# QZ1-boy/CDFO

Measured on AMD Instinct MI355X. Metric: x4 SR frames/sec, 7-frame 270x480->1080p, higher is better.
Workload: dtype fp16 MFMA, fp32 accumulate (1 pass inside Block_, 2 passes = fp16 hi+lo activations elsewhere, split-bf16 for the returned feature cache; 2-4e-4 max-abs vs the fp32 reference, bound 1e-3); 1 GPU; JCT-VC ClassB-shape synthetic clips: 8 clips/GPU x 7x1x270x480 luma (padded to 272x480) + MV/residual/partition/unfiltered priors -> 1080x1920, fresh path (pre_L1_fea=None), precision=fp16x2, Gumbel noise drawn per forward inside the mask kernel (the reference's default behaviour); clips_per_gpu=8, parallelism=batch-shard x1, weights=random init (seed 0), launch=eager

## Files before the change

cdfo_amd/_lib.py:

```python
from __future__ import annotations

import ctypes as C
import os

import torch

from . import switches

_HERE = os.path.dirname(os.path.abspath(__file__))
LIB_PATH = switches.get("CDFO_LIB_PATH") or os.path.join(_HERE, "lib", "libcdfo_hip.so")

_lib = None


class CdfoError(RuntimeError):
    pass


class ConvArgs(C.Structure):
    _fields_ = [
        ("src", C.c_void_p * 8), ("ld", C.c_int * 8), ("cs", C.c_int * 8), ("nsrc", C.c_int),
        ("B", C.c_int), ("H", C.c_int), ("W", C.c_int), ("Ho", C.c_int), ("Wo", C.c_int),
        ("ks", C.c_int), ("stride", C.c_int), ("pad", C.c_int),
        ("Cin", C.c_int), ("Cout", C.c_int), ("CoutP", C.c_int),
        ("w", C.c_void_p), ("w_bstride", C.c_longlong), ("bias", C.c_void_p),
        ("act", C.c_int),
        ("res1", C.c_void_p), ("ldr1", C.c_int),
        ("res2", C.c_void_p), ("ldr2", C.c_int),
        ("out", C.c_void_p), ("ldo", C.c_int), ("store_mode", C.c_int),
        ("prec", C.c_int),
        ("ln_gamma", C.c_void_p), ("ln_beta", C.c_void_p),
        ("tap_mask", C.c_void_p),
        ("src_f16", C.c_int), ("out_f16", C.c_int),
        ("out2_cp16", C.c_void_p),
        ("src_plane_wrap", C.c_int),
        ("res_up2", C.c_void_p), ("ldru", C.c_int),
        ("out2_lo", C.c_int),
        ("mask_out", C.c_void_p), ("flow", C.c_void_p), ("flow_bstride", C.c_longlong), ("off_mag", C.c_float),
        ("off_accumulate", C.c_int),
        ("res2_pixscale", C.c_void_p),
        ("src_halfsplit", C.c_int),
    ]


def lib() -> C.CDLL:
    global _lib
    if _lib is None:
        if not os.path.exists(LIB_PATH):
            raise CdfoError(
                f"{LIB_PATH} is missing: the HIP extension has not been built "
                "(run `python -m cdfo_amd.build`).  There is no CPU fallback for the product path.")
        switches.check_hip_environment()
        _lib = C.CDLL(LIB_PATH)
        for name, (restype, argtypes) in header_prototypes().items():
            fn = getattr(_lib, name)
            fn.restype = restype
            fn.argtypes = argtypes
    return _lib


HEADER_PATH = os.path.join(os.path.dirname(_HERE), "include", "cdfo_hip.h")


def header_prototypes(path: str = HEADER_PATH):
    import re
    text = open(path).read()
    text = re.sub(r"/\*.*?\*/", " ", text, flags=re.S)
    protos = {}
    for m in re.finditer(r"(const char\*|long long|int)\s+(cdfo_[a-z0-9_]+)\s*\(([^)]*)\)\s*;", text):
        ret, name, args = m.group(1), m.group(2), m.group(3).strip()
        at = []
        if args and args != "void":
            for a in args.split(","):
                a = " ".join(a.split())
                if "*" in a:
                    at.append(C.c_void_p)
                elif a.startswith("long long"):
                    at.append(C.c_longlong)
                elif a.startswith("float"):
                    at.append(C.c_float)
                elif a.startswith("int"):
                    at.append(C.c_int)
                else:
                    raise CdfoError(f"cannot map C type in prototype of {name}: {a!r}")
        protos[name] = (C.c_char_p if ret.startswith("const char") else C.c_longlong if ret == "long long" else C.c_int, at)
    return protos


def check(status: int, what: str) -> None:
    if status != 0:
        kind = {-1: "invalid argument", -2: "misaligned pointer/pitch"}.get(status, f"hipError_t {status}")
        raise CdfoError(f"{what} failed: {kind}")
```

cdfo_amd/csrc/conv1x1_bf16x3.hip:

```cpp
#include "common.h"

namespace {

constexpr int PXT = 128;
constexpr int PIXB = 80;
constexpr int A_CHUNK = PXT * PIXB;
constexpr int A_BYTES = 4 * A_CHUNK;
constexpr int W_HALF = 4 * 2 * 64 * 16;
constexpr int W_BYTES = 2 * W_HALF;
constexpr int EPI_RS = 68;
constexpr int EPI_BYTES = 4 * 32 * EPI_RS * 4;
constexpr int MAXCB = 4;

typedef __bf16 bf16x8_t __attribute__((ext_vector_type(8)));
typedef unsigned int u32x2 __attribute__((ext_vector_type(2)));

__device__ __forceinline__ unsigned pack_bf16(float a, float b) {
  const __bf16 ha = (__bf16)a, hb = (__bf16)b;
  return (unsigned)__builtin_bit_cast(unsigned short, ha) | ((unsigned)__builtin_bit_cast(unsigned short, hb) << 16);
}
__device__ __forceinline__ float bf16_round(float a) { return (float)(__bf16)a; }
__device__ __forceinline__ void split_store(unsigned char* dst_hi, int lo_delta, const f32x4 v) {
  u32x2 hi, lo;
  hi[0] = pack_bf16(v[0], v[1]);
// ... 86 lines not shown
        const bf16x8_t ah = *reinterpret_cast<const bf16x8_t*>(sA + c * A_CHUNK + a_off);
        const bf16x8_t al = *reinterpret_cast<const bf16x8_t*>(sA + c * A_CHUNK + a_off + 32);
#pragma unroll
        for (int ni = 0; ni < 2; ++ni) {
          const bf16x8_t bh = *reinterpret_cast<const bf16x8_t*>(sW + (c * 2 * 64 + ni * 32) * 16 + b_off);
          const bf16x8_t bl = *reinterpret_cast<const bf16x8_t*>(sW + W_HALF + (c * 2 * 64 + ni * 32) * 16 + b_off);
          acc[cb][ni] = __builtin_amdgcn_mfma_f32_32x32x16_bf16(al, bh, acc[cb][ni], 0, 0, 0);
          acc[cb][ni] = __builtin_amdgcn_mfma_f32_32x32x16_bf16(ah, bl, acc[cb][ni], 0, 0, 0);
          acc[cb][ni] = __builtin_amdgcn_mfma_f32_32x32x16_bf16(ah, bh, acc[cb][ni], 0, 0, 0);
        }
      }
    }
  }

  __syncthreads();
  float* wl = reinterpret_cast<float*>(smem) + wave * 32 * EPI_RS;
  const float slope = a.act == CDFO_ACT_NONE ? 1.f : (a.act == CDFO_ACT_LRELU ? 0.1f : 0.f);
  const int c4 = lane & 15, pr = lane >> 4;
  const bool plain = a.store_mode == CDFO_STORE_PLAIN;
  const int cq = a.Cout >> 2;
  typedef _Float16 c1_f16x8 __attribute__((ext_vector_type(8)));
  c1_f16x8 twh[TAPS ? 4 : 1], twl[TAPS ? 4 : 1];
  if (TAPS) {
#pragma unroll
    for (int s4 = 0; s4 < 4; ++s4)
#pragma unroll
      for (int j = 0; j < 8; ++j) {
        const float wv = r < 9 ? a.res2[(16 * s4 + 8 * h + j) * 9 + r] : 0.f;
        twh[s4][j] = (_Float16)wv;
        twl[s4][j] = (_Float16)(wv - (float)twh[s4][j]);
      }
  }
#pragma unroll
  for (int cb = 0; cb < NCB; ++cb) {
#pragma unroll
    for (int ni = 0; ni < 2; ++ni)
#pragma unroll
      for (int e = 0; e < 16; ++e) wl[((e & 3) + 8 * (e >> 2) + 4 * h) * EPI_RS + ni * 32 + r] = acc[cb][ni][e];
    __builtin_amdgcn_fence(__ATOMIC_RELEASE, "wavefront");
    __builtin_amdgcn_wave_barrier();
    __builtin_amdgcn_fence(__ATOMIC_ACQUIRE, "wavefront");
    if (TAPS) {
      f32x4 y[4][2];
      float amax = 0.f;
#pragma unroll
      for (int s4 = 0; s4 < 4; ++s4)
#pragma unroll
        for (int q = 0; q < 2; ++q) {
          const int ch = 16 * s4 + 8 * h + 4 * q;
          f32x4 t = *reinterpret_cast<const f32x4*>(wl + r * EPI_RS + ch);
          if (a.bias) t += *reinterpret_cast<const f32x4*>(a.bias + cb * 64 + ch);
#pragma unroll
          for (int k = 0; k < 4; ++k) {
            t[k] = fmaxf(t[k], 0.f) + slope * fminf(t[k], 0.f);
            amax = fmaxf(amax, fabsf(t[k]));
          }
          y[s4][q] = t;
        }
      amax = fmaxf(amax, __shfl_xor(amax, 32, 64));
      int ex = 0;
      if (amax > 0.f && amax < INFINITY) frexpf(amax, &ex);
      ex = ex < -100 ? -100 : (ex > 100 ? 100 : ex);
      const float sc = ldexpf(1.f, 14 - ex), inv = ldexpf(1.f, ex - 14);
      f32x16 tacc;
#pragma unroll
      for (int e = 0; e < 16; ++e) tacc[e] = 0.f;
#pragma unroll
      for (int s4 = 0; s4 < 4; ++s4) {
        c1_f16x8 yh, yl;
#pragma unroll
        for (int j = 0; j < 8; ++j) {
          const float v = y[s4][j >> 2][j & 3] * sc;
          yh[j] = (_Float16)v;
          yl[j] = (_Float16)(v - (float)yh[j]);
        }
        tacc = __builtin_amdgcn_mfma_f32_32x32x16_f16(twl[s4], yh, tacc, 0, 0, 0);
        tacc = __builtin_amdgcn_mfma_f32_32x32x16_f16(twh[s4], yl, tacc, 0, 0, 0);
        tacc = __builtin_amdgcn_mfma_f32_32x32x16_f16(twh[s4], yh, tacc, 0, 0, 0);
      }
      const long long pin = p0 + wave * 32 + r;
      if (pin < P) {
        const int oy = (int)(pin / a.W), ox = (int)(pin - (long long)oy * a.W);
        const long long opix = ((long long)b * 2 * a.H + 2 * oy + (cb >> 1)) * (2 * a.W) + 2 * ox + (cb & 1);
        float* op = a.out + opix * a.ldo;
        const f32x4 t4 = {tacc[0] * inv, tacc[1] * inv, tacc[2] * inv, tacc[3] * inv};
        if ((a.ldo & 3) == 0) *reinterpret_cast<f32x4*>(op + 4 * h) = t4;
        else { op[4 * h] = t4[0]; op[4 * h + 1] = t4[1]; op[4 * h + 2] = t4[2]; op[4 * h + 3] = t4[3]; }
        if (h == 0) op[8] = tacc[4] * inv;
      }
      __builtin_amdgcn_fence(__ATOMIC_RELEASE, "wavefront");
      __builtin_amdgcn_wave_barrier();
      continue;
    }
    const int n = cb * 64 + c4 * 4;
    const bool nok = n < a.Cout;
    f32x4 bias = {0.f, 0.f, 0.f, 0.f};
    if (a.bias && nok) bias = *reinterpret_cast<const f32x4*>(a.bias + n);
#pragma unroll
    for (int it = 0; it < 8; ++it) {
      const int i = it * 4 + pr;
      f32x4 t = *reinterpret_cast<const f32x4*>(wl + i * EPI_RS + c4 * 4) + bias;
#pragma unroll
      for (int k = 0; k < 4; ++k) t[k] = fmaxf(t[k], 0.f) + slope * fminf(t[k], 0.f);
      const long long pin = p0 + wave * 32 + i;
      if (!nok || pin >= P) continue;
      const long long pix = (long long)b * P + pin;
      if (plain) {
        if (a.res1) t += *reinterpret_cast<const f32x4*>(a.res1 + pix * a.ldr1 + n);
        if (a.res2) t += *reinterpret_cast<const f32x4*>(a.res2 + pix * a.ldr2 + n);
        *reinterpret_cast<f32x4*>(a.out + pix * a.ldo + n) = t;
      } else {
        const int sub = n / cq, cc = n - sub * cq;
        const int oy = (int)(pin / a.W), ox = (int)(pin - (long long)oy * a.W);
        const long long opix = ((long long)b * 2 * a.H + 2 * oy + (sub >> 1)) * (2 * a.W) + 2 * ox + (sub & 1);
        *reinterpret_cast<f32x4*>(a.out + opix * a.ldo + cc) = t;
      }
    }
    __builtin_amdgcn_fence(__ATOMIC_RELEASE, "wavefront");
    __builtin_amdgcn_wave_barrier();
  }
}

}

int cdfo_conv1x1_stream_try(const cdfo_conv_args& a, hipStream_t st);
extern "C" int cdfo_layernorm64_cp16hl(const float* in, int ldi, const float* gamma, const float* beta, int B, long long P,
                                       void* out, void* stream);

extern "C" int cdfo_conv1x1_bf16x3(const cdfo_conv_args* pa, void* stream) {
  const cdfo_conv_args& a = *pa;
  hipStream_t st = static_cast<hipStream_t>(stream);
  if (a.nsrc < 1 || a.nsrc > CDFO_MAXSRC || a.B <= 0 || a.ks != 1 || a.stride != 1 || a.pad != 0) return CDFO_EINVAL;
  if (a.act == CDFO_ACT_SIGMOID || a.tap_mask || a.src_f16 || a.out_f16 || a.res_up2 || a.src_plane_wrap) return CDFO_EINVAL;
  const bool ln_out = a.out2_cp16 != nullptr;
  const bool copy_out = ln_out && !a.ln_gamma && !a.ln_beta;
  if (ln_out && (a.Cout != 64 || a.CoutP != 64 || a.store_mode != CDFO_STORE_PLAIN || a.ldo < 64 || !aligned16(a.out2_cp16))) return CDFO_EINVAL;
  if (ln_out && !copy_out && (!a.ln_gamma || !a.ln_beta || !aligned16(a.ln_gamma) || !aligned16(a.ln_beta))) return CDFO_EINVAL;
  int csum = 0;
  for (int s = 0; s < a.nsrc; ++s) {
    if (a.cs[s] <= 0 || a.cs[s] % 64 || a.ld[s] % 4 || a.ld[s] < a.cs[s]) return CDFO_EINVAL;
    if (!aligned16(a.src[s])) return CDFO_EALIGN;
    csum += a.cs[s];
  }
  if (csum != a.Cin || a.CoutP % 64 || a.CoutP > 64 * MAXCB || a.CoutP < a.Cout || a.Cout <= 0 || a.Cout % 4) return CDFO_EINVAL;
  if (a.Ho != a.H || a.Wo != a.W) return CDFO_EINVAL;
  if (a.store_mode == CDFO_STORE_S2D || (a.store_mode == CDFO_STORE_SHUFFLE2 && (a.Cout % 16 || a.res1 || a.res2))) return CDFO_EINVAL;
  if (a.store_mode == CDFO_STORE_TAPS9 && (a.Cout != 256 || a.CoutP != 256 || a.res1 || !a.res2 || a.ldo < 9 || a.w_bstride)) return CDFO_EINVAL;
  const bool taps = a.store_mode == CDFO_STORE_TAPS9;
  if (!aligned16(a.w) || a.w_bstride % 4 || (!taps && a.ldo % 4) || !aligned16(a.out) || (a.bias && !aligned16(a.bias))) return CDFO_EALIGN;
  if ((a.res1 && (a.ldr1 % 4 || !aligned16(a.res1))) || (!taps && a.res2 && (a.ldr2 % 4 || !aligned16(a.res2)))) return CDFO_EALIGN;
  if (!ln_out && a.ln_gamma && !(a.nsrc == 1 && a.cs[0] == 64 && a.ln_beta && aligned16(a.ln_gamma) && aligned16(a.ln_beta))) return CDFO_EINVAL;
  const long long P = (long long)a.H * a.W;
  if (a.res2_pixscale && (!a.res2 || taps)) return CDFO_EINVAL;
  if (ln_out) {
    const int r = cdfo_conv1x1_stream_try(a, st);
    if (r == 1) return 0;
    if (r != 0) return r;
    if (a.res2_pixscale) return CDFO_EINVAL;
    cdfo_conv_args plain = a;
    plain.out2_cp16 = nullptr; plain.ln_gamma = nullptr; plain.ln_beta = nullptr;
    const int rc = cdfo_conv1x1_bf16x3(&plain, stream);
    if (rc) return rc;
    if (copy_out) return cdfo_to_cp16(a.out, a.ldo, a.B, P, 64, a.out2_cp16, stream);
    return cdfo_layernorm64_cp16hl(a.out, a.ldo, a.ln_gamma, a.ln_beta, a.B, P, a.out2_cp16, stream);
  }
  {
    static const bool use_stream = cdfo_switch("CDFO_CONV1X1_STREAM", 1) != 0;
    static const bool taps_stream = cdfo_switch("CDFO_TAPS_STREAM", 1) != 0;
    if (use_stream && (!taps || taps_stream)) {
      const int r = cdfo_conv1x1_stream_try(a, st);
      if (r == 1) return 0;
      if (r != 0) return r;
    }
  }
  if (a.res2_pixscale) return CDFO_EINVAL;
  dim3 grid((unsigned)((P + PXT - 1) / PXT), a.B);
  const double px = (double)a.B * P;
  CdfoProfScope prof(st, KID_CONV1, 2.0 * px * a.Cout * a.Cin, 4.0 * (px * a.Cout + px * a.Cin + (double)a.Cin * a.Cout));
  if (taps) {
    hipLaunchKernelGGL((conv1x1_bf16x3_kernel<4, true>), grid, dim3(256), 0, st, a);
    CDFO_LAUNCH_CHECK();
    return 0;
  }
  switch (a.CoutP / 64) {
    case 1: hipLaunchKernelGGL(conv1x1_bf16x3_kernel<1>, grid, dim3(256), 0, st, a); break;
    case 2: hipLaunchKernelGGL(conv1x1_bf16x3_kernel<2>, grid, dim3(256), 0, st, a); break;
    case 3: hipLaunchKernelGGL(conv1x1_bf16x3_kernel<3>, grid, dim3(256), 0, st, a); break;
    default: hipLaunchKernelGGL(conv1x1_bf16x3_kernel<4>, grid, dim3(256), 0, st, a); break;
  }
  CDFO_LAUNCH_CHECK();
  return 0;
}
```

cdfo_amd/csrc/conv1x1_stream.hip:

```cpp
#include "common.h"

namespace {

constexpr int ST_THREADS = 256;
constexpr int ST_STAGE = 8192;
constexpr int ST_MAXNS = 4;

typedef __bf16 bf16x8_t __attribute__((ext_vector_type(8)));
typedef int i32x4 __attribute__((ext_vector_type(4)));
typedef unsigned int u32x2 __attribute__((ext_vector_type(2)));

struct st_item { const float* base; int ld; int ch0; };

struct st_args {
  st_item act[CDFO_MAXSRC * 4];
  int nkb;
  st_item res[2];
  const float* res_scale;
  const float* w; long long w_bstride; const float* bias;
  int Cin, Cout, CoutP, act_fn;
  float* out; int ldo;
  int B; long long P;
  int tiles_per_image; long long tiles;
  int ns;
  _Float16* ln_hl; const float* ln_g; const float* ln_b;
  const float* w_last;
  int W;
};

__device__ __forceinline__ unsigned st_pack_bf16(float a, float b) {
  const __bf16 ha = (__bf16)a, hb = (__bf16)b;
  return (unsigned)__builtin_bit_cast(unsigned short, ha) | ((unsigned)__builtin_bit_cast(unsigned short, hb) << 16);
}
__device__ __forceinline__ float st_bf16_round(float a) { return (float)(__bf16)a; }

__device__ __forceinline__ void st_dma8(const unsigned (&voff)[8], i32x4 rsrc, unsigned lds) {
  unsigned keep;
  asm volatile(
      "s_nop 4\n\t"
      "s_mov_b32 %0, m0\n\t"
      "s_mov_b32 m0, %10\n\ts_nop 0\n\t"
      "buffer_load_dwordx4 %1, %9, 0 offen lds\n\t"
      "s_add_u32 m0, m0, 0x400\n\ts_nop 0\n\t"
      "buffer_load_dwordx4 %2, %9, 0 offen lds\n\t"
      "s_add_u32 m0, m0, 0x400\n\ts_nop 0\n\t"
      "buffer_load_dwordx4 %3, %9, 0 offen lds\n\t"
      "s_add_u32 m0, m0, 0x400\n\ts_nop 0\n\t"
      "buffer_load_dwordx4 %4, %9, 0 offen lds\n\t"
      "s_add_u32 m0, m0, 0x400\n\ts_nop 0\n\t"
      "buffer_load_dwordx4 %5, %9, 0 offen lds\n\t"
      "s_add_u32 m0, m0, 0x400\n\ts_nop 0\n\t"
      "buffer_load_dwordx4 %6, %9, 0 offen lds\n\t"
      "s_add_u32 m0, m0, 0x400\n\ts_nop 0\n\t"
      "buffer_load_dwordx4 %7, %9, 0 offen lds\n\t"
      "s_add_u32 m0, m0, 0x400\n\ts_nop 0\n\t"
      "buffer_load_dwordx4 %8, %9, 0 offen lds\n\t"
      "s_mov_b32 m0, %0"
      : "=&s"(keep)
      : "v"(voff[0]), "v"(voff[1]), "v"(voff[2]), "v"(voff[3]), "v"(voff[4]), "v"(voff[5]), "v"(voff[6]), "v"(voff[7]),
        "s"(rsrc), "s"(lds)
      : "memory", "scc");
}

__device__ __forceinline__ void st_dma1(unsigned voff, i32x4 rsrc, unsigned lds) {
  unsigned keep;
  asm volatile(
      "s_nop 4\n\t"
      "s_mov_b32 %0, m0\n\t"
      "s_mov_b32 m0, %3\n\ts_nop 0\n\t"
      "buffer_load_dword %1, %2, 0 offen lds\n\t"
      "s_mov_b32 m0, %0"
      : "=&s"(keep)
      : "v"(voff), "s"(rsrc), "s"(lds)
      : "memory", "scc");
}

__device__ __forceinline__ void st_split_pair_f16(float x, float y, unsigned& hi, unsigned& lo) {
  typedef _Float16 h2 __attribute__((ext_vector_type(2)));
  const h2 hv = {(_Float16)x, (_Float16)y};
  hi = __builtin_bit_cast(unsigned, hv);
  float rx, ry;
  asm("v_fma_mix_f32 %0, %1, 1.0, -%2 op_sel_hi:[0,0,1]" : "=v"(rx) : "v"(x), "v"(hi));
  asm("v_fma_mix_f32 %0, %1, 1.0, -%2 op_sel:[0,0,1] op_sel_hi:[0,0,1]" : "=v"(ry) : "v"(y), "v"(hi));
  const h2 lv = {(_Float16)rx, (_Float16)ry};
  lo = __builtin_bit_cast(unsigned, lv);
}

template <int NCB, bool TAPS = false>
__global__ __launch_bounds__(ST_THREADS) void conv1x1_stream_kernel(st_args a) {
  extern __shared__ __attribute__((aligned(16))) unsigned char smem[];
  const int tid = threadIdx.x, lane = tid & 63, h = lane >> 5, r = lane & 31;
  const int wave = __builtin_amdgcn_readfirstlane(tid >> 6);
  const int nkb = a.nkb, NS = a.ns;
  const int w_half = nkb * 4 * 2 * NCB * 64 * 16;
  unsigned char* sWh = smem;
  unsigned char* sWl = smem + w_half;
  float* sBias = reinterpret_cast<float*>(smem + 2 * w_half);
  const int ring_off = 2 * w_half + NCB * 64 * 4;
  unsigned char* ring = smem + ring_off + wave * NS * ST_STAGE;
  const unsigned ring_lds = (unsigned)(unsigned long long)(smem) + ring_off + wave * NS * ST_STAGE;
  const unsigned char* scale_slots = smem + ring_off + 4 * NS * ST_STAGE + wave * 512;
  const unsigned scale_lds = (unsigned)(unsigned long long)(smem) + ring_off + 4 * NS * ST_STAGE + wave * 512;

  auto chan_of_row = [](int n) { const int m = n & 31; return (n & ~31) + ((m >> 4) & 1) * 16 + ((m >> 2) & 1) * 8 + ((m >> 3) & 1) * 4 + (m & 3); };

  const long long t_lo = a.tiles * blockIdx.x / gridDim.x, t_hi = a.tiles * (blockIdx.x + 1) / gridDim.x;
  if (t_lo >= t_hi) return;
  const int nres = (a.res[0].base ? 1 : 0) + (a.res[1].base ? 1 : 0);
  const int items_per_tile = nkb + nres * NCB;
  const float slope = a.act_fn == CDFO_ACT_NONE ? 1.f : (a.act_fn == CDFO_ACT_LRELU ? 0.1f : 0.f);

  int d_px[8], d_part[8];
#pragma unroll
  for (int k = 0; k < 8; ++k) {
    const int s = 64 * k + lane, p = s >> 4;
    d_px[k] = p;
    d_part[k] = (s & 15) ^ (p & 15);
  }
  auto part_off = [&](int q) { return r * 256 + ((q ^ (r & 15)) << 4); };

  typedef _Float16 st_h8 __attribute__((ext_vector_type(8)));
  typedef unsigned st_u4 __attribute__((ext_vector_type(4)));
  st_h8 twh[TAPS ? 4 : 1], twl[TAPS ? 4 : 1];
  if (TAPS) {
#pragma unroll
    for (int s4 = 0; s4 < 4; ++s4)
#pragma unroll
      for (int j = 0; j < 8; ++j) {
        const float wv = r < 9 ? a.w_last[(16 * s4 + 8 * h + j) * 9 + r] : 0.f;
        twh[s4][j] = (_Float16)wv;
        twl[s4][j] = (_Float16)(wv - (float)twh[s4][j]);
      }
  }

  for (long long img_t0 = t_lo; img_t0 < t_hi;) {
    const int b = (int)(img_t0 / a.tiles_per_image);
    const long long img_end = (long long)(b + 1) * a.tiles_per_image;
    const long long seg_hi = img_end < t_hi ? img_end : t_hi;
    __syncthreads();
    {
      const float* wb = a.w + (long long)b * a.w_bstride;
      const int ngrp = (a.Cin >> 2) * NCB * 64;
      for (int i = tid; i < ngrp; i += ST_THREADS) {
        const int rowpos = i % (NCB * 64), kg = i / (NCB * 64);
        const int n = chan_of_row(rowpos);
        f32x4 wv = {0.f, 0.f, 0.f, 0.f};
        if (n < a.CoutP) wv = *reinterpret_cast<const f32x4*>(wb + ((long long)kg * a.CoutP + n) * 4);
        const int c = kg >> 2, hh = (kg >> 1) & 1, j0 = (kg & 1) * 4;
        u32x2 hi, lo;
        hi[0] = st_pack_bf16(wv[0], wv[1]); hi[1] = st_pack_bf16(wv[2], wv[3]);
        lo[0] = st_pack_bf16(wv[0] - st_bf16_round(wv[0]), wv[1] - st_bf16_round(wv[1]));
        lo[1] = st_pack_bf16(wv[2] - st_bf16_round(wv[2]), wv[3] - st_bf16_round(wv[3]));
        const int off = ((c * 2 + hh) * (NCB * 64) + rowpos) * 16 + j0 * 2;
        *reinterpret_cast<u32x2*>(sWh + off) = hi;
        *reinterpret_cast<u32x2*>(sWl + off) = lo;
      }
      for (int i = tid; i < NCB * 64; i += ST_THREADS) sBias[i] = (a.bias && i < a.Cout) ? a.bias[i] : 0.f;
    }
    __syncthreads();

    const long long n_items = (seg_hi - img_t0) * items_per_tile;
    long long issued = 0;
    auto issue = [&](long long it) {
      const long long tile = img_t0 + it / items_per_tile;
      const int k = (int)(it % items_per_tile);
      const long long p0 = (tile - (long long)b * a.tiles_per_image) * 128 + wave * 32;
      if (a.res_scale && k == 0) {
        const long long rows = a.P - p0;
        const unsigned long long pb = reinterpret_cast<unsigned long long>(a.res_scale + (long long)b * a.P + (rows > 0 ? p0 : 0));
        i32x4 rs;
        rs[0] = __builtin_amdgcn_readfirstlane((int)(unsigned)pb);
        rs[1] = __builtin_amdgcn_readfirstlane((int)(unsigned)(pb >> 32));
        rs[2] = __builtin_amdgcn_readfirstlane((int)(rows > 0 ? (rows < 32 ? rows : 32) * 4 : 0));
        rs[3] = 0x00020000;
        st_dma1((unsigned)r * 4, rs, __builtin_amdgcn_readfirstlane(scale_lds + (unsigned)(tile & 1) * 256));
      }
      st_item src;
      int chan0;
      if (k < nkb) { src = a.act[k]; chan0 = src.ch0; }
      else {
        const int j = k - nkb;
        src = a.res[j / NCB];
        chan0 = (j % NCB) * 64;
      }
      const long long rows_left = a.P - p0;
      const float* base = src.base + ((long long)b * a.P + (rows_left > 0 ? p0 : 0)) * src.ld + chan0;
      const unsigned long long pb = reinterpret_cast<unsigned long long>(base);
      i32x4 rsrc;
      rsrc[0] = __builtin_amdgcn_readfirstlane((int)(unsigned)pb);
      rsrc[1] = __builtin_amdgcn_readfirstlane((int)(unsigned)(pb >> 32));
      const long long bytes = rows_left > 0 ? (rows_left < 32 ? rows_left : 32) * (long long)src.ld * 4 : 0;
      rsrc[2] = __builtin_amdgcn_readfirstlane((int)bytes);
      rsrc[3] = 0x00020000;
      unsigned voff[8];
#pragma unroll
      for (int q = 0; q < 8; ++q) voff[q] = (unsigned)(d_px[q] * src.ld * 4 + d_part[q] * 16);
      st_dma8(voff, rsrc, __builtin_amdgcn_readfirstlane(ring_lds + (unsigned)(it % NS) * ST_STAGE));
    };
    for (; issued < NS - 1 && issued < n_items; ++issued) issue(issued);

    f32x16 acc[NCB][2];
    for (long long it = 0; it < n_items; ++it) {
      const int k = (int)(it % items_per_tile);
      const long long younger = TAPS ? 0 : issued - it - 1;
      if (younger >= 2) asm volatile("s_waitcnt vmcnt(16)" ::: "memory");
      else if (younger == 1) asm volatile("s_waitcnt vmcnt(8)" ::: "memory");
      else asm volatile("s_waitcnt vmcnt(0)" ::: "memory");
      const unsigned char* st = ring + (it % NS) * ST_STAGE;
      if (TAPS) {
        if (issued < n_items) { asm volatile("s_waitcnt lgkmcnt(0)" ::: "memory"); issue(issued); ++issued; }
      }
      if (k == 0) {
#pragma unroll
        for (int cb = 0; cb < NCB; ++cb)
#pragma unroll
          for (int ni = 0; ni < 2; ++ni)
#pragma unroll
            for (int e = 0; e < 16; ++e) acc[cb][ni][e] = 0.f;
      }
      if (k < nkb) {
#pragma unroll
        for (int c = 0; c < 4; ++c) {
          const f32x4 v0 = *reinterpret_cast<const f32x4*>(st + part_off(c * 4 + h * 2));
          const f32x4 v1 = *reinterpret_cast<const f32x4*>(st + part_off(c * 4 + h * 2 + 1));
          union { unsigned u[4]; bf16x8_t v; } ph, pl;
          ph.u[0] = st_pack_bf16(v0[0], v0[1]); ph.u[1] = st_pack_bf16(v0[2], v0[3]);
          ph.u[2] = st_pack_bf16(v1[0], v1[1]); ph.u[3] = st_pack_bf16(v1[2], v1[3]);
          pl.u[0] = st_pack_bf16(v0[0] - st_bf16_round(v0[0]), v0[1] - st_bf16_round(v0[1]));
          pl.u[1] = st_pack_bf16(v0[2] - st_bf16_round(v0[2]), v0[3] - st_bf16_round(v0[3]));
          pl.u[2] = st_pack_bf16(v1[0] - st_bf16_round(v1[0]), v1[1] - st_bf16_round(v1[1]));
          pl.u[3] = st_pack_bf16(v1[2] - st_bf16_round(v1[2]), v1[3] - st_bf16_round(v1[3]));
          const int wrow = ((k * 4 + c) * 2 + h) * (NCB * 64) + r;
#pragma unroll
          for (int cb = 0; cb < NCB; ++cb)
#pragma unroll
            for (int ni = 0; ni < 2; ++ni) {
              const bf16x8_t wh = *reinterpret_cast<const bf16x8_t*>(sWh + (wrow + cb * 64 + ni * 32) * 16);
              const bf16x8_t wl = *reinterpret_cast<const bf16x8_t*>(sWl + (wrow + cb * 64 + ni * 32) * 16);
              acc[cb][ni] = __builtin_amdgcn_mfma_f32_32x32x16_bf16(wh, pl.v, acc[cb][ni], 0, 0, 0);
              acc[cb][ni] = __builtin_amdgcn_mfma_f32_32x32x16_bf16(wl, ph.v, acc[cb][ni], 0, 0, 0);
              acc[cb][ni] = __builtin_amdgcn_mfma_f32_32x32x16_bf16(wh, ph.v, acc[cb][ni], 0, 0, 0);
            }
        }
        if (k == nkb - 1) {
#pragma unroll
          for (int cb = 0; cb < NCB; ++cb)
#pragma unroll
            for (int ni = 0; ni < 2; ++ni)
#pragma unroll
              for (int e = 0; e < 16; ++e) {
                const float t = acc[cb][ni][e] + sBias[cb * 64 + ni * 32 + (e >> 3) * 16 + h * 8 + (e & 7)];
                acc[cb][ni][e] = fmaxf(t, 0.f) + slope * fminf(t, 0.f);
              }
        }
      } else {
        const int cb = (k - nkb) % NCB;
        float sc = 1.f;
        if (a.res_scale && (k - nkb) / NCB == nres - 1)
          sc = *reinterpret_cast<const float*>(scale_slots + ((img_t0 + it / items_per_tile) & 1) * 256 + lane * 4);
#pragma unroll
        for (int cc = 0; cc < NCB; ++cc) {
          if (cc != cb) continue;
#pragma unroll
          for (int ni = 0; ni < 2; ++ni)
#pragma unroll
            for (int jj = 0; jj < 2; ++jj) {
              const int q = (ni * 32 + jj * 16 + h * 8) >> 2;
              const f32x4 r0 = *reinterpret_cast<const f32x4*>(st + part_off(q));
              const f32x4 r1 = *reinterpret_cast<const f32x4*>(st + part_off(q + 1));
#pragma unroll
              for (int e = 0; e < 4; ++e) { acc[cc][ni][8 * jj + e] = fmaf(sc, r0[e], acc[cc][ni][8 * jj + e]); acc[cc][ni][8 * jj + 4 + e] = fmaf(sc, r1[e], acc[cc][ni][8 * jj + 4 + e]); }
            }
        }
      }
      if (!TAPS && issued < n_items) { asm volatile("s_waitcnt lgkmcnt(0)" ::: "memory"); issue(issued); ++issued; }
      if (k == items_per_tile - 1) {
        const long long tile = img_t0 + it / items_per_tile;
        const long long pin = (tile - (long long)b * a.tiles_per_image) * 128 + wave * 32 + r;
        if (NCB == 1 && a.ln_hl && !a.ln_g) {
          typedef _Float16 st_f16x8 __attribute__((ext_vector_type(8)));
          if (pin < a.P) {
#pragma unroll
            for (int ni = 0; ni < 2; ++ni)
#pragma unroll
              for (int jj = 0; jj < 2; ++jj) {
                const int n = ni * 32 + jj * 16 + h * 8;
                st_f16x8 hv;
#pragma unroll
                for (int e = 0; e < 8; ++e) hv[e] = (_Float16)acc[0][ni][8 * jj + e];
                *reinterpret_cast<st_f16x8*>(a.ln_hl + (((long long)b * 4 + (n >> 4)) * a.P + pin) * 16 + h * 8) = hv;
              }
          }
        } else if (NCB == 1 && a.ln_hl) {
          typedef _Float16 st_f16x8 __attribute__((ext_vector_type(8)));
          float sm = 0.f;
#pragma unroll
          for (int ni = 0; ni < 2; ++ni)
#pragma unroll
            for (int e = 0; e < 16; ++e) sm += acc[0][ni][e];
          sm += __shfl_xor(sm, 32, 64);
          const float mu = sm * (1.f / 64.f);
          float sq = 0.f;
#pragma unroll
          for (int ni = 0; ni < 2; ++ni)
#pragma unroll
            for (int e = 0; e < 16; ++e) { const float d = acc[0][ni][e] - mu; sq = fmaf(d, d, sq); }
          sq += __shfl_xor(sq, 32, 64);
          const float rstd = 1.f / sqrtf(sq * (1.f / 64.f) + 1e-5f);
          if (pin < a.P) {
#pragma unroll
            for (int ni = 0; ni < 2; ++ni)
#pragma unroll
              for (int jj = 0; jj < 2; ++jj) {
                const int n = ni * 32 + jj * 16 + h * 8;
                const f32x4 g0 = *reinterpret_cast<const f32x4*>(a.ln_g + n), g1 = *reinterpret_cast<const f32x4*>(a.ln_g + n + 4);
                const f32x4 b0 = *reinterpret_cast<const f32x4*>(a.ln_b + n), b1 = *reinterpret_cast<const f32x4*>(a.ln_b + n + 4);
                st_f16x8 hi, lo;
#pragma unroll
                for (int e = 0; e < 8; ++e) {
                  const float y = (acc[0][ni][8 * jj + e] - mu) * rstd * (e < 4 ? g0[e & 3] : g1[e & 3]) + (e < 4 ? b0[e & 3] : b1[e & 3]);
                  hi[e] = (_Float16)y;
                  lo[e] = (_Float16)(y - (float)hi[e]);
                }
                _Float16* o16 = a.ln_hl + (((long long)b * 8 + (n >> 4)) * a.P + pin) * 16 + h * 8;
                *reinterpret_cast<st_f16x8*>(o16) = hi;
                *reinterpret_cast<st_f16x8*>(o16 + 4 * a.P * 16) = lo;
              }
          }
        }
        if (TAPS) {
          const int oy = (int)(pin / a.W), ox = (int)(pin - (long long)oy * a.W);
#pragma unroll
          for (int cb = 0; cb < NCB; ++cb) {
            float amax = 0.f;
#pragma unroll
            for (int ni = 0; ni < 2; ++ni)
#pragma unroll
              for (int e = 0; e < 16; ++e) amax = fmaxf(amax, fabsf(acc[cb][ni][e]));
            amax = fmaxf(amax, __shfl_xor(amax, 32, 64));
            int ex = 0;
            if (amax > 0.f && amax < INFINITY) frexpf(amax, &ex);
            ex = ex < -100 ? -100 : (ex > 100 ? 100 : ex);
            const float sc = ldexpf(1.f, 14 - ex), inv = ldexpf(1.f, ex - 14);
            f32x16 tacc;
#pragma unroll
            for (int e = 0; e < 16; ++e) tacc[e] = 0.f;
#pragma unroll
            for (int s4 = 0; s4 < 4; ++s4) {
              unsigned hh[4], ll[4];
#pragma unroll
              for (int j = 0; j < 4; ++j)
                st_split_pair_f16(acc[cb][s4 >> 1][8 * (s4 & 1) + 2 * j] * sc, acc[cb][s4 >> 1][8 * (s4 & 1) + 2 * j + 1] * sc, hh[j], ll[j]);
              const st_u4 hu = {hh[0], hh[1], hh[2], hh[3]}, lu = {ll[0], ll[1], ll[2], ll[3]};
              const st_h8 yh = __builtin_bit_cast(st_h8, hu), yl = __builtin_bit_cast(st_h8, lu);
              tacc = __builtin_amdgcn_mfma_f32_32x32x16_f16(twl[s4], yh, tacc, 0, 0, 0);
              tacc = __builtin_amdgcn_mfma_f32_32x32x16_f16(twh[s4], yl, tacc, 0, 0, 0);
              tacc = __builtin_amdgcn_mfma_f32_32x32x16_f16(twh[s4], yh, tacc, 0, 0, 0);
            }
            if (pin < a.P) {
              const long long opix = ((long long)b * 2 * (a.P / a.W) + 2 * oy + (cb >> 1)) * (2 * a.W) + 2 * ox + (cb & 1);
              float* op = a.out + opix * a.ldo;
              const f32x4 t4 = {tacc[0] * inv, tacc[1] * inv, tacc[2] * inv, tacc[3] * inv};
              *reinterpret_cast<f32x4*>(op + 4 * h) = t4;
              if (h == 0) op[8] = tacc[4] * inv;
            }
          }
        } else if (pin < a.P) {
          float* op = a.out + ((long long)b * a.P + pin) * a.ldo;
#pragma unroll
          for (int cb = 0; cb < NCB; ++cb)
#pragma unroll
            for (int ni = 0; ni < 2; ++ni)
#pragma unroll
              for (int jj = 0; jj < 2; ++jj) {
                const int n = cb * 64 + ni * 32 + jj * 16 + h * 8;
                if (n < a.Cout) {
                  f32x4 v0, v1;
#pragma unroll
                  for (int e = 0; e < 4; ++e) { v0[e] = acc[cb][ni][8 * jj + e]; v1[e] = acc[cb][ni][8 * jj + 4 + e]; }
                  *reinterpret_cast<f32x4*>(op + n) = v0;
                  *reinterpret_cast<f32x4*>(op + n + 4) = v1;
                }
              }
        }
      }
    }
    img_t0 = seg_hi;
  }
}

}

int cdfo_conv1x1_stream_try(const cdfo_conv_args& a, hipStream_t st) {
  const bool ln_out = a.out2_cp16 != nullptr;
  const bool taps = a.store_mode == CDFO_STORE_TAPS9;
  if (taps) {
    if (a.Cin != 64 || a.nsrc != 1 || a.ldo % 4 || a.ldo < 12 || a.ln_gamma || ln_out || (long long)a.ld[0] * 4 * 32 >= (1ll << 31)) return 0;
    st_args s{};
    s.act[0].base = a.src[0]; s.act[0].ld = a.ld[0]; s.act[0].ch0 = 0;
    s.nkb = 1;
    s.w = a.w; s.w_bstride = a.w_bstride; s.bias = a.bias;
    s.Cin = 64; s.Cout = 256; s.CoutP = 256; s.act_fn = a.act;
    s.out = a.out; s.ldo = a.ldo; s.B = a.B; s.P = (long long)a.H * a.W;
    s.w_last = a.res2; s.W = a.W;
    s.tiles_per_image = (int)((s.P + 127) / 128);
    s.tiles = (long long)a.B * s.tiles_per_image;
    s.ns = 2;
    const int w_bytes = 2 * 1 * 4 * 2 * 4 * 64 * 16 + 4 * 64 * 4;
    const int lds = w_bytes + 4 * s.ns * ST_STAGE;
    const int cus = cdfo_num_cus();
    if (cus <= 0) return CDFO_EINVAL;
    const int grid = (int)(s.tiles < cus ? s.tiles : cus);
    const double px = (double)a.B * s.P;
    CdfoProfScope prof(st, KID_CONV1, 2.0 * px * 256 * 64 + 2.0 * px * 4 * 9 * 64, 4.0 * (px * 64 + px * 4 * a.ldo + 64.0 * 256));
    static CdfoAttrOnce once;
    const hipError_t e = cdfo_set_max_lds(once, reinterpret_cast<const void*>(conv1x1_stream_kernel<4, true>), 160 * 1024 - 256);
    if (e != hipSuccess) return (int)e;
    hipLaunchKernelGGL((conv1x1_stream_kernel<4, true>), dim3(grid), dim3(ST_THREADS), lds, st, s);
    const hipError_t e2 = hipGetLastError();
    return e2 == hipSuccess ? 1 : (int)e2;
  }
  if (a.store_mode != CDFO_STORE_PLAIN || (a.ln_gamma && !ln_out) || a.CoutP % 64 || a.CoutP > 128 || a.Cout % 8) return 0;
  if (ln_out && (a.CoutP != 64 || a.Cout != 64)) return 0;
  const int ncb = a.CoutP / 64, nkb = a.Cin / 64;
  if (nkb < 1 || nkb > CDFO_MAXSRC * 4) return 0;
  const int w_bytes = 2 * nkb * 4 * 2 * ncb * 64 * 16 + ncb * 64 * 4;
  const int scale_bytes = (a.res2 && a.res2_pixscale) ? 4 * 512 : 0;
  int ns = (160 * 1024 - 256 - scale_bytes - w_bytes) / (4 * ST_STAGE);
  if (ns > ST_MAXNS) ns = ST_MAXNS;
  if (scale_bytes) {
    const int items_per_tile = nkb + ((a.res1 ? 1 : 0) + 1) * ncb;
    if (ns > items_per_tile + 2) ns = items_per_tile + 2;
  }
  if (ns < 3) return 0;
  const long long P = (long long)a.H * a.W;
  st_args s{};
  int k = 0;
  for (int i = 0; i < a.nsrc; ++i) {
    if ((long long)a.ld[i] * 4 * 32 >= (1ll << 31)) return 0;
    for (int c = 0; c < a.cs[i]; c += 64) { s.act[k].base = a.src[i]; s.act[k].ld = a.ld[i]; s.act[k].ch0 = c; ++k; }
  }
  if (k != nkb) return 0;
  s.nkb = nkb;
  int nr = 0;
  if (a.res1) { if (a.ldr1 < a.CoutP) return 0; s.res[nr].base = a.res1; s.res[nr].ld = a.ldr1; ++nr; }
  if (a.res2) { if (a.ldr2 < a.CoutP) return 0; s.res[nr].base = a.res2; s.res[nr].ld = a.ldr2; ++nr; }
  s.res_scale = a.res2 ? a.res2_pixscale : nullptr;
  s.w = a.w; s.w_bstride = a.w_bstride; s.bias = a.bias;
  s.Cin = a.Cin; s.Cout = a.Cout; s.CoutP = a.CoutP; s.act_fn = a.act;
  s.out = a.out; s.ldo = a.ldo; s.B = a.B; s.P = P;
  s.ln_hl = ln_out ? static_cast<_Float16*>(a.out2_cp16) : nullptr; s.ln_g = a.ln_gamma; s.ln_b = a.ln_beta;
  s.tiles_per_image = (int)((P + 127) / 128);
  s.tiles = (long long)a.B * s.tiles_per_image;
  s.ns = ns;
  const int cus = cdfo_num_cus();
  if (cus <= 0) return CDFO_EINVAL;
  const int grid = (int)(s.tiles < cus ? s.tiles : cus);
  const int lds = w_bytes + 4 * ns * ST_STAGE + scale_bytes;
  const double px = (double)a.B * P;
  CdfoProfScope prof(st, KID_CONV1, 2.0 * px * a.Cout * a.Cin, 4.0 * (px * a.Cout * (1 + nr) + px * a.Cin + (double)a.Cin * a.Cout));
  if (ncb == 1) {
    static CdfoAttrOnce once;
    const hipError_t e = cdfo_set_max_lds(once, reinterpret_cast<const void*>(conv1x1_stream_kernel<1>), 160 * 1024 - 256);
    if (e != hipSuccess) return (int)e;
    hipLaunchKernelGGL(conv1x1_stream_kernel<1>, dim3(grid), dim3(ST_THREADS), lds, st, s);
  } else {
    static CdfoAttrOnce once;
    const hipError_t e = cdfo_set_max_lds(once, reinterpret_cast<const void*>(conv1x1_stream_kernel<2>), 160 * 1024 - 256);
    if (e != hipSuccess) return (int)e;
    hipLaunchKernelGGL(conv1x1_stream_kernel<2>, dim3(grid), dim3(ST_THREADS), lds, st, s);
  }
  hipError_t e = hipGetLastError();
  return e == hipSuccess ? 1 : (int)e;
}
```

cdfo_amd/csrc/conv3x3_bf16.hip:

```cpp
#include "common.h"
#include "conv_epilogue.h"

constexpr int PIXB_F32SRC = 80;

namespace {

constexpr int TH = 8, TW = 32, IW = 34, NPIX = 34 * 10;
constexpr int W_HALF = 9 * 2 * 64 * 16;

enum { M_BF16X3 = CDFO_PREC_BF16X3, M_BF16 = CDFO_PREC_BF16, M_FP16X2 = CDFO_PREC_FP16X2, M_FP16IN = CDFO_PREC_FP16,
       M_FP16X1 = CDFO_PREC_FP16X1 };

typedef __bf16 bf16x8_t __attribute__((ext_vector_type(8)));
typedef _Float16 f16x8_t __attribute__((ext_vector_type(8)));
typedef unsigned int u32x2 __attribute__((ext_vector_type(2)));
typedef unsigned int u32x4 __attribute__((ext_vector_type(4)));

template <int MODE> struct Fmt;
template <> struct Fmt<M_BF16X3> { using frag = bf16x8_t; static constexpr bool ALO = true, WLO = true; };
template <> struct Fmt<M_BF16> { using frag = bf16x8_t; static constexpr bool ALO = false, WLO = false; };
template <> struct Fmt<M_FP16X2> { using frag = f16x8_t; static constexpr bool ALO = true, WLO = false; };
template <> struct Fmt<M_FP16IN> { using frag = f16x8_t; static constexpr bool ALO = false, WLO = false; };
template <> struct Fmt<M_FP16X1> { using frag = f16x8_t; static constexpr bool ALO = false, WLO = false; };

// ... 186 lines not shown
      hi[0] = pack16<F16>(v[0], v[1]);
      hi[1] = pack16<F16>(v[2], v[3]);
      *reinterpret_cast<u32x2*>(sA + a_lds[s]) = hi;
      if (F::ALO) {
        lo[0] = pack16<F16>(v[0] - round16<F16>(v[0]), v[1] - round16<F16>(v[1]));
        lo[1] = pack16<F16>(v[2] - round16<F16>(v[2]), v[3] - round16<F16>(v[3]));
        *reinterpret_cast<u32x2*>(sA + a_lds[s] + 32) = lo;
      }
    }
#pragma unroll
    for (int s = 0; s < NWS; ++s) {
      const int idx = tid + 256 * s;
      if (idx < NWU) *reinterpret_cast<u32x4*>(sW + idx * 16) = rw[s];
    }
  };

  frag_t fah[2][2], fal[2][2], fbh[2][2], fbl[2][2];
  auto load_frags = [&](int t, int par) {
    const int dy = t / 3, dx = t - dy * 3;
#pragma unroll
    for (int mi = 0; mi < 2; ++mi) {
      fah[par][mi] = *reinterpret_cast<const frag_t*>(sA + a_off[mi] + (dy * IW + dx) * PIXB);
      if (F::ALO) fal[par][mi] = *reinterpret_cast<const frag_t*>(sA + a_off[mi] + (dy * IW + dx) * PIXB + 32);
    }
#pragma unroll
    for (int ni = 0; ni < NT; ++ni) {
      fbh[par][ni] = *reinterpret_cast<const frag_t*>(sW + (t * 2 * 64 + ni * 32) * 16 + b_off);
      if (F::WLO) fbl[par][ni] = *reinterpret_cast<const frag_t*>(sW + W_HALF + (t * 2 * 64 + ni * 32) * 16 + b_off);
    }
  };
  auto mma_tap = [&](int par) {
    if (DBG & 1) {
#pragma unroll
      for (int mi = 0; mi < 2; ++mi)
#pragma unroll
        for (int ni = 0; ni < NT; ++ni) acc[mi][ni][0] += (float)fah[par][mi][0] * (float)fbh[par][ni][0];
      return;
    }
#pragma unroll
    for (int mi = 0; mi < 2; ++mi)
#pragma unroll
      for (int ni = 0; ni < NT; ++ni) {
        if (F::ALO) acc[mi][ni] = mma(fal[par][mi], fbh[par][ni], acc[mi][ni]);
        if (F::WLO) acc[mi][ni] = mma(fah[par][mi], fbl[par][ni], acc[mi][ni]);
        acc[mi][ni] = mma(fah[par][mi], fbh[par][ni], acc[mi][ni]);
      }
  };

  constexpr bool OFFMASK_OK = (MODE == M_BF16X3 || MODE == M_FP16X2 || MODE == M_FP16X1) && NT == 2 && DBG == 0;
  constexpr bool OFFMASK_EARLY = OFFMASK_OK && MODE == M_FP16X1;
  const bool offmask = OFFMASK_OK && a.store_mode == CDFO_STORE_OFFMASK;
  OffmaskLane<NT> om;

  issue_loads(0);
  write_lds();
  __syncthreads();
  const int nmain = (OFFMASK_EARLY && offmask) ? nchunks - 1 : nchunks;
  for (int c = 0; c < nmain; ++c) {
    if (WAVES_PER_SIMD <= 2 && c + 1 < nchunks && !(DBG & 2)) issue_loads(c + 1);
    if (a.tap_mask) {
      const unsigned tm = a.tap_mask[c];
#pragma unroll
      for (int t = 0; t < 9; ++t) {
        if (!((tm >> t) & 1u)) continue;
        load_frags(t, 0);
        mma_tap(0);
      }
    } else {
      if (WAVES_PER_SIMD <= 2) {
        load_frags(0, 0);
#pragma unroll
        for (int t = 0; t < 9; ++t) {
          if (t < 8) load_frags(t + 1, (t & 1) ^ 1);
          mma_tap(t & 1);
        }
      } else {
#pragma unroll 1
        for (int t = 0; t < 9; ++t) {
          load_frags(t, 0);
          mma_tap(0);
        }
      }
    }
    if (!(DBG & 16)) __syncthreads();
    if (c + 1 < nchunks) {
      if (WAVES_PER_SIMD > 2) issue_loads(c + 1);
      if (!(DBG & 4)) write_lds();
      if (!(DBG & 16)) __syncthreads();
    }
  }
  if (OFFMASK_EARLY && offmask) {
    offmask_prefetch<NT>(a, om, lane, b, oy0 + wave * 2, ox0, n0);
    load_frags(0, 0);
#pragma unroll
    for (int t = 0; t < 9; ++t) {
      if (t < 8) load_frags(t + 1, (t & 1) ^ 1);
      mma_tap(t & 1);
    }
    __syncthreads();
  }

  if (DBG & 8) {
    float t = 0.f;
#pragma unroll
    for (int mi = 0; mi < 2; ++mi)
#pragma unroll
      for (int ni = 0; ni < NT; ++ni)
#pragma unroll
        for (int e = 0; e < 16; ++e) t += acc[mi][ni][e];
    if (t == 123.456f) a.out[0] = t;
    return;
  }
  if (offmask) {
    if (!OFFMASK_EARLY) offmask_prefetch<NT>(a, om, lane, b, oy0 + wave * 2, ox0, n0);
    offmask_finish<NT>(a, om, acc, lane, oy0 + wave * 2, ox0);
    return;
  }
  float* wl = reinterpret_cast<float*>(smem) + wave * ConvEpi<NT>::WAVE_FLOATS;
#pragma unroll
  for (int mi = 0; mi < 2; ++mi) conv_tile_epilogue_row32<NT>(a, wl, acc[mi], lane, b, oy0 + wave * 2 + mi, ox0, n0);
}

template <bool F16>
__global__ void pack16_kernel(const float* __restrict__ w, unsigned short* __restrict__ p, int Cout, int Cin, int CoutP) {
  const long long half = (long long)(Cin / 16) * 18 * CoutP * 8;
  for (long long i = blockIdx.x * (long long)blockDim.x + threadIdx.x; i < half;
       i += (long long)gridDim.x * blockDim.x) {
    const int j = i & 7;
    long long rest = i >> 3;
    const int n = rest % CoutP; rest /= CoutP;
    const int hh = rest & 1; rest >>= 1;
    const int t = rest % 9;
    const int c = rest / 9;
    const int cin = c * 16 + hh * 8 + j;
    float v = 0.f;
    if (n < Cout) v = w[((long long)n * Cin + cin) * 9 + t];
    if (F16) {
      p[i] = __builtin_bit_cast(unsigned short, (_Float16)v);
    } else {
      const __bf16 hi = (__bf16)v;
      p[i] = __builtin_bit_cast(unsigned short, hi);
      p[half + i] = __builtin_bit_cast(unsigned short, (__bf16)(v - (float)hi));
    }
  }
}

}

extern "C" int cdfo_conv3x3_bf16(const cdfo_conv_args* pa, void* stream) {
  const cdfo_conv_args& a = *pa;
  hipStream_t st = static_cast<hipStream_t>(stream);
  if (a.nsrc < 1 || a.nsrc > CDFO_MAXSRC || a.B <= 0 || a.ks != 3 || a.stride != 1 || a.pad != 1) return CDFO_EINVAL;
  if (a.act == CDFO_ACT_SIGMOID) return CDFO_EINVAL;
  if (a.out2_cp16 || a.res_up2 || a.src_plane_wrap || a.res2_pixscale) return CDFO_EINVAL;
  int csum = 0;
  for (int s = 0; s < a.nsrc; ++s) {
    if (a.cs[s] <= 0 || a.cs[s] % 16 || a.ld[s] % 4 || a.ld[s] < a.cs[s]) return CDFO_EINVAL;
    if (!aligned16(a.src[s])) return CDFO_EALIGN;
    csum += a.cs[s];
  }
  if (csum != a.Cin || a.CoutP % 64 || a.CoutP < a.Cout || a.Cout <= 0 || a.Ho != a.H || a.Wo != a.W) return CDFO_EINVAL;
  const bool offmask = a.store_mode == CDFO_STORE_OFFMASK;
  if (offmask) {
    const int pr = a.prec & 255;
    if ((pr != CDFO_PREC_BF16X3 && pr != CDFO_PREC_FP16X2 && pr != CDFO_PREC_FP16X1) || (a.prec >> 8) || a.Cout % 3 || a.Cout <= 32 || a.Wo % 4 || a.act != CDFO_ACT_NONE ||
        a.res1 || a.res2 || a.out_f16 || a.tap_mask || !a.mask_out || !a.flow || a.flow_bstride % 4 ||
        (long long)a.Ho * a.Wo >= (1ll << 31))
      return CDFO_EINVAL;
    if (!aligned16(a.mask_out) || !aligned16(a.flow)) return CDFO_EALIGN;
  }
  if ((a.store_mode != CDFO_STORE_PLAIN && a.store_mode != CDFO_STORE_S2D && !offmask) || a.w_bstride != 0) return CDFO_EINVAL;
  if (a.store_mode == CDFO_STORE_S2D && ((a.Ho | a.Wo) & 1 || a.res1 || a.res2)) return CDFO_EINVAL;
  if (!aligned16(a.w) || a.Cout % 4 || a.ldo % 4 || !aligned16(a.out) || (a.bias && !aligned16(a.bias))) return CDFO_EALIGN;
  if ((a.res1 && (a.ldr1 % 4 || !aligned16(a.res1))) || (a.res2 && (a.ldr2 % 4 || !aligned16(a.res2)))) return CDFO_EALIGN;
  if ((long long)a.B * a.H * a.W >= (1ll << 31)) return CDFO_EINVAL;
  if (a.src_f16 != ((a.prec & 255) == CDFO_PREC_FP16) || (a.src_f16 && (a.nsrc != 1 || a.ld[0] % 8))) return CDFO_EINVAL;
  if (a.out_f16 && (a.res1 || a.res2 || a.store_mode == CDFO_STORE_SHUFFLE2)) return CDFO_EINVAL;
  dim3 grid(cdiv(cdiv(a.Wo, TW) * cdiv(a.Ho, TH) * a.B, 8) * 8 * (a.CoutP / 64));
  const double px = (double)a.B * a.Ho * a.Wo;
  CdfoProfScope prof(st, KID_CONV3_WIDE, 2.0 * px * a.Cout * a.Cin * 9,
                     4.0 * (px * a.Cout + px * a.Cin + 9.0 * a.Cin * a.Cout));
  const int dbg = a.prec >> 8, prec = a.prec & 255;
  if (dbg) {
#ifdef CDFO_DEV_ABLATIONS
    if (prec != CDFO_PREC_BF16X3) return CDFO_EINVAL;
#define CDFO_DBG_CASE(D) case D: hipLaunchKernelGGL((conv3x3_mma16_kernel<M_BF16X3, 2, D>), grid, dim3(256), 0, st, a); break;
    switch (dbg) {
      CDFO_DBG_CASE(1) CDFO_DBG_CASE(2) CDFO_DBG_CASE(3) CDFO_DBG_CASE(4) CDFO_DBG_CASE(7) CDFO_DBG_CASE(8)
      CDFO_DBG_CASE(15) CDFO_DBG_CASE(16) CDFO_DBG_CASE(31)
      default: return CDFO_EINVAL;
    }
#undef CDFO_DBG_CASE
#else
    return CDFO_EINVAL;
#endif
  } else if (prec == CDFO_PREC_BF16X3 && a.Cout <= 32 && a.CoutP == 64) {
    hipLaunchKernelGGL((conv3x3_mma16_kernel<M_BF16X3, 2, 0, 1>), grid, dim3(256), 0, st, a);
  } else if (prec == CDFO_PREC_FP16X2 && a.Cout <= 32 && a.CoutP == 64) {
    hipLaunchKernelGGL((conv3x3_mma16_kernel<M_FP16X2, 2, 0, 1>), grid, dim3(256), 0, st, a);
  } else if (prec == CDFO_PREC_BF16X3) {
    hipLaunchKernelGGL((conv3x3_mma16_kernel<M_BF16X3, 2, 0>), grid, dim3(256), 0, st, a);
  } else if (prec == CDFO_PREC_BF16) {
    hipLaunchKernelGGL((conv3x3_mma16_kernel<M_BF16, 2, 0>), grid, dim3(256), 0, st, a);
  } else if (prec == CDFO_PREC_FP16X2) {
    hipLaunchKernelGGL((conv3x3_mma16_kernel<M_FP16X2, 2, 0>), grid, dim3(256), 0, st, a);
  } else if (prec == CDFO_PREC_FP16) {
    hipLaunchKernelGGL((conv3x3_mma16_kernel<M_FP16IN, 2, 0>), grid, dim3(256), 0, st, a);
  } else if (prec == CDFO_PREC_FP16X1) {
    hipLaunchKernelGGL((conv3x3_mma16_kernel<M_FP16X1, 2, 0>), grid, dim3(256), 0, st, a);
  } else {
    return CDFO_EINVAL;
  }
  CDFO_LAUNCH_CHECK();
  return 0;
}

static int pack16_launch(const float* w, void* packed, int Cout, int Cin, bool f16, void* stream) {
  if (Cin % 16 || Cout <= 0) return CDFO_EINVAL;
  const int CoutP = (Cout + 63) / 64 * 64;
  const long long half = (long long)(Cin / 16) * 18 * CoutP * 8;
  const int blocks = (int)((half + 255) / 256 < 2048 ? (half + 255) / 256 : 2048);
  CdfoProfScope prof(static_cast<hipStream_t>(stream), KID_PACK, 0, 8.0 * half);
  if (f16)
    hipLaunchKernelGGL(pack16_kernel<true>, dim3(blocks), dim3(256), 0, static_cast<hipStream_t>(stream), w,
                       static_cast<unsigned short*>(packed), Cout, Cin, CoutP);
  else
    hipLaunchKernelGGL(pack16_kernel<false>, dim3(blocks), dim3(256), 0, static_cast<hipStream_t>(stream), w,
                       static_cast<unsigned short*>(packed), Cout, Cin, CoutP);
  CDFO_LAUNCH_CHECK();
  return 0;
}

extern "C" int cdfo_pack_conv3x3_bf16(const float* w_oihw, void* packed, int Cout, int Cin, void* stream) {
  return pack16_launch(w_oihw, packed, Cout, Cin, false, stream);
}
extern "C" int cdfo_pack_conv3x3_f16(const float* w_oihw, void* packed, int Cout, int Cin, void* stream) {
  return pack16_launch(w_oihw, packed, Cout, Cin, true, stream);
}
```

cdfo_amd/csrc/conv3x3_ring.hip:

```cpp
#include "common.h"

namespace {

constexpr int RG_THREADS = 512;
constexpr int RG_TH = 16, RG_IW = 34, RG_NPIX = 18 * 34;
constexpr int RG_ACT = 20 * 1024;
constexpr int RG_ET_ROWS = 10, RG_ET_COLS = 18;
constexpr int RG_ET_PIECES = 48;
template <bool SPARSE> struct RingLds {
  static constexpr int NS = SPARSE ? 3 : 4;
  static constexpr int WGT = (SPARSE ? 8 : 18) * 1024;
  static constexpr int STAGE = RG_ACT + WGT;
  static constexpr int ETILE = NS * STAGE;
  static constexpr int DUMP = ETILE + (SPARSE ? RG_ET_PIECES * 1024 : 0);
  static constexpr int BIAS = DUMP + 1024;
  static constexpr int WINTAB = BIAS + 4096;
  static constexpr int TOTAL = WINTAB + (SPARSE ? 1024 : 0);
};

typedef _Float16 f16x8_t __attribute__((ext_vector_type(8)));
typedef int i32x4 __attribute__((ext_vector_type(4)));

struct ring_extra {
  const void* src;
// ... 931 lines not shown

    if (DBG & 8) {
      float t = 0.f;
#pragma unroll
      for (int ni = 0; ni < 2; ++ni)
#pragma unroll
        for (int mi = 0; mi < CR; ++mi)
#pragma unroll
          for (int q = 0; q < 16; ++q) t += acc[ni][mi][q] + rva[ni & 1][mi & 1][0][q & 3];
      if (t == 123.456f) a.out[0] = t;
      continue;
    }
    auto epilogue_row = [&](int mi, const f32x4 (&rv)[2][2][2]) {
      const int oy = oyw + mi, X = ox0 + r;
      const bool ok = row_ok(mi);
      const long long pix = (long long)(b * H + oy) * W + X;
#pragma unroll
      for (int ni = 0; ni < 2; ++ni)
#pragma unroll
        for (int jj = 0; jj < 2; ++jj) {
          const int n = n0 + ni * 32 + jj * 16 + h * 8;
          const f32x4 b0 = *reinterpret_cast<const f32x4*>(smem + L::BIAS + n * 4);
          const f32x4 b1 = *reinterpret_cast<const f32x4*>(smem + L::BIAS + n * 4 + 16);
          f32x4 v0, v1;
#pragma unroll
          for (int k = 0; k < 4; ++k) {
            const float t0 = acc[ni][mi][8 * jj + k] + b0[k], t1 = acc[ni][mi][8 * jj + 4 + k] + b1[k];
            v0[k] = fmaxf(t0, slope * t0);
            v1[k] = fmaxf(t1, slope * t1);
          }
          v0 += rv[ni][jj][0];
          v1 += rv[ni][jj][1];
          if (!ok || n >= a.Cout) continue;
          if (a.res2 && !(DBG & 16)) {
            const float* p2 = a.res2 + pix * a.ldr2 + n;
            v0 += *reinterpret_cast<const f32x4*>(p2);
            v1 += *reinterpret_cast<const f32x4*>(p2 + 4);
          }
          if (a.res_up2) {
            const float ly = (oy & 1) ? 0.25f : 0.75f, lx = (X & 1) ? 0.25f : 0.75f;
            if (SPARSE) {
              const int li = ((oy + 1) >> 1) - (oy0 >> 1), lj = ((X + 1) >> 1) - (ox0 >> 1);
              const unsigned char* et = smem + L::ETILE;
              const int cq = (ni * 32 + jj * 16 + h * 8) >> 2;
#pragma unroll
              for (int hf = 0; hf < 2; ++hf) {
                auto tap = [&](int i, int j) {
                  const int px = i * RG_ET_COLS + j;
                  return *reinterpret_cast<const f32x4*>(et + px * 256 + (((cq + hf) ^ (px & 15)) << 4));
                };
                (hf ? v1 : v0) += (1.f - ly) * ((1.f - lx) * tap(li, lj) + lx * tap(li, lj + 1)) +
                                  ly * ((1.f - lx) * tap(li + 1, lj) + lx * tap(li + 1, lj + 1));
              }
            } else {
              const int Hd = H >> 1, Wd = W >> 1;
              const int Q = (oy + 1) >> 1, P = (X + 1) >> 1;
              const int ya = Q > 0 ? Q - 1 : 0, yb = Q < Hd ? Q : Hd - 1, xa = P > 0 ? P - 1 : 0, xb = P < Wd ? P : Wd - 1;
              const float* eb = a.res_up2 + (long long)b * Hd * Wd * a.ldru + n;
              const float* paa = eb + ((long long)ya * Wd + xa) * a.ldru;
              const float* pab = eb + ((long long)ya * Wd + xb) * a.ldru;
              const float* pba = eb + ((long long)yb * Wd + xa) * a.ldru;
              const float* pbb = eb + ((long long)yb * Wd + xb) * a.ldru;
#pragma unroll
              for (int hf = 0; hf < 2; ++hf) {
                const f32x4 eaa = *reinterpret_cast<const f32x4*>(paa + 4 * hf), eab = *reinterpret_cast<const f32x4*>(pab + 4 * hf);
                const f32x4 eba = *reinterpret_cast<const f32x4*>(pba + 4 * hf), ebb = *reinterpret_cast<const f32x4*>(pbb + 4 * hf);
                (hf ? v1 : v0) += (1.f - ly) * ((1.f - lx) * eaa + lx * eab) + ly * ((1.f - lx) * eba + lx * ebb);
              }
            }
          }
          f16x8_t hv;
#pragma unroll
          for (int k = 0; k < 4; ++k) { hv[k] = (_Float16)v0[k]; hv[4 + k] = (_Float16)v1[k]; }
          if (a.out_f16) {
            *reinterpret_cast<f16x8_t*>(reinterpret_cast<_Float16*>(a.out) + pix * a.ldo + n) = hv;
          } else {
            *reinterpret_cast<f32x4*>(a.out + pix * a.ldo + n) = v0;
            *reinterpret_cast<f32x4*>(a.out + pix * a.ldo + n + 4) = v1;
          }
          if (a.out2_cp16) {
            const int npl = a.out2_lo ? (a.Cout >> 3) : (a.Cout >> 4);
            _Float16* o2 = static_cast<_Float16*>(a.out2_cp16) + (((long long)b * npl + (n >> 4)) * H * W + (long long)oy * W + X) * 16 + h * 8;
            *reinterpret_cast<f16x8_t*>(o2) = hv;
            if (a.out2_lo) {
              f16x8_t lv;
#pragma unroll
              for (int k = 0; k < 4; ++k) { lv[k] = (_Float16)(v0[k] - (float)hv[k]); lv[4 + k] = (_Float16)(v1[k] - (float)hv[4 + k]); }
              *reinterpret_cast<f16x8_t*>(o2 + (long long)(a.Cout >> 4) * H * W * 16) = lv;
            }
          }
        }
    };
    unsigned long long te0 = 0, te1 = 0;
    if (DBG & 16) asm volatile("s_memtime %0" : "=s"(te0) : : "memory");
    load_res_row(1, rvb);
    epilogue_row(0, rva);
    load_res_row(2, rva);
    epilogue_row(1, rvb);
    load_res_row(3, rvb);
    epilogue_row(2, rva);
    epilogue_row(3, rvb);
    if (DBG & 16) {
      asm volatile("s_memtime %0" : "=s"(te1) : : "memory");
      asm volatile("s_waitcnt lgkmcnt(0)" ::: "memory");
      if (ord == RG_PROBE_UNIT + 1 && lane == 0) {
        unsigned long long* cb = reinterpret_cast<unsigned long long*>(const_cast<float*>(a.res2)) + ((long long)blockIdx.x * 8 + wave) * 40;
        cb[29] = te0;
        cb[39] = te1;
      }
    }
  }
}

int rg_num_cus() { return cdfo_num_cus(); }

bool rg_split() {
  static const bool v = cdfo_switch("CDFO_RING_SPLIT", 1) != 0;
  return v;
}

template <bool SPARSE, int DBG>
int rg_launch(const cdfo_conv_args& a, const ring_extra& e, int grid, hipStream_t st) {
  static CdfoAttrOnce once, once_split;
  if constexpr (SPARSE) {
    if (rg_split() && !(a.res_up2 && e.nc < 8)) {
      static const bool mf16 = cdfo_switch("CDFO_RING_MFMA16", 1) != 0;
      if (mf16 && !(DBG & (4 | 16))) {
        static CdfoAttrOnce once16;
        const hipError_t err = cdfo_set_max_lds(once16, reinterpret_cast<const void*>(conv3x3_ring_split_kernel<SPARSE, DBG, true>), RingLds<SPARSE>::TOTAL);
        if (err != hipSuccess) return (int)err;
        hipLaunchKernelGGL((conv3x3_ring_split_kernel<SPARSE, DBG, true>), dim3(grid), dim3(RG_THREADS), RingLds<SPARSE>::TOTAL, st, a, e);
        return 0;
      }
      const hipError_t err = cdfo_set_max_lds(once_split, reinterpret_cast<const void*>(conv3x3_ring_split_kernel<SPARSE, DBG>), RingLds<SPARSE>::TOTAL);
      if (err != hipSuccess) return (int)err;
      hipLaunchKernelGGL((conv3x3_ring_split_kernel<SPARSE, DBG>), dim3(grid), dim3(RG_THREADS), RingLds<SPARSE>::TOTAL, st, a, e);
      return 0;
    }
  }
  const hipError_t err = cdfo_set_max_lds(once, reinterpret_cast<const void*>(conv3x3_ring_kernel<SPARSE, DBG>), RingLds<SPARSE>::TOTAL);
  if (err != hipSuccess) return (int)err;
  hipLaunchKernelGGL((conv3x3_ring_kernel<SPARSE, DBG>), dim3(grid), dim3(RG_THREADS), RingLds<SPARSE>::TOTAL, st, a, e);
  return 0;
}

}

extern "C" int cdfo_conv3x3_ring(const cdfo_conv_args* pa, void* stream) {
  const cdfo_conv_args& a = *pa;
  hipStream_t st = static_cast<hipStream_t>(stream);
  if (a.nsrc != 1 || a.B <= 0 || a.ks != 3 || a.stride != 1 || a.pad != 1 || !a.src_f16) return CDFO_EINVAL;
  if (a.act == CDFO_ACT_SIGMOID || a.Cin <= 0 || a.Cin % 16 || a.cs[0] != a.Cin || a.ld[0] != 16) return CDFO_EINVAL;
  if (a.CoutP % 64 || a.CoutP > 1024 || a.CoutP < a.Cout || a.Cout <= 0 || a.Ho != a.H || a.Wo != a.W || a.w_bstride != 0) return CDFO_EINVAL;
  if (a.store_mode != CDFO_STORE_PLAIN || a.res2_pixscale) return CDFO_EINVAL;
  if (a.Cout % 8) return CDFO_EINVAL;
  if (a.out2_cp16 && (a.Cout % 16 || !aligned16(a.out2_cp16))) return CDFO_EINVAL;
  if (a.res_up2 && ((a.H | a.W) & 1 || a.ldru % 4 || a.ldru < a.Cout || !aligned16(a.res_up2))) return CDFO_EINVAL;
  if (!aligned16(a.src[0]) || !aligned16(a.w) || a.Cout % 4 || a.ldo % 4 || !aligned16(a.out) ||
      (a.bias && !aligned16(a.bias)))
    return CDFO_EALIGN;
  if ((a.res1 && (a.ldr1 % 4 || !aligned16(a.res1))) || (a.res2 && (a.ldr2 % 4 || !aligned16(a.res2)))) return CDFO_EALIGN;
  const int nc = a.Cin / 16;
  if ((long long)nc * a.H * a.W * 32 >= (1ll << 31) || (long long)a.B * a.H * a.W >= (1ll << 31)) return CDFO_EINVAL;
  const int taps = a.tap_mask ? 4 : 9;
  const long long w_bytes = (long long)nc * taps * 2 * a.CoutP * 16;
  if (w_bytes >= (1ll << 31)) return CDFO_EINVAL;
  const int cus = rg_num_cus();
  if (cus < 8) return CDFO_EINVAL;
  ring_extra e;
  e.src = a.src[0]; e.nc = nc; e.w = a.w; e.CoutP = a.CoutP; e.tap_mask = a.tap_mask; e.w_bytes = (int)w_bytes;
  e.plane_wrap = a.src_plane_wrap;
  e.halfsplit = a.src_halfsplit ? 1 : 0;
  static const int touch = cdfo_switch("CDFO_RING_TOUCH", 0);
  e.touch = (touch && a.res1 && (long long)a.H * a.W * a.ldr1 * 4 < (1ll << 31)) ? 1 : 0;
  e.src_planes = a.src_plane_wrap ? a.src_plane_wrap : nc;
  if (a.src_plane_wrap < 0 || a.src_plane_wrap > nc) return CDFO_EINVAL;
  const int grid = cus / 8 * 8;
  const double px = (double)a.B * a.Ho * a.Wo;
  CdfoProfScope prof(st, a.tap_mask ? KID_CONV3_RING4 : KID_CONV3_RING, 2.0 * px * a.Cout * a.Cin * taps,
                     2.0 * px * a.Cin + (a.out_f16 ? 2.0 : 4.0) * px * a.Cout + 2.0 * taps * a.Cin * a.Cout);
  int rc;
  switch (a.prec >> 8) {
    case 0: rc = a.tap_mask ? rg_launch<true, 0>(a, e, grid, st) : rg_launch<false, 0>(a, e, grid, st); break;
#ifdef CDFO_DEV_ABLATIONS
    case 1: rc = a.tap_mask ? rg_launch<true, 1>(a, e, grid, st) : rg_launch<false, 1>(a, e, grid, st); break;
    case 2: rc = a.tap_mask ? rg_launch<true, 2>(a, e, grid, st) : rg_launch<false, 2>(a, e, grid, st); break;
    case 4: rc = a.tap_mask ? rg_launch<true, 4>(a, e, grid, st) : rg_launch<false, 4>(a, e, grid, st); break;
    case 8: rc = a.tap_mask ? rg_launch<true, 8>(a, e, grid, st) : rg_launch<false, 8>(a, e, grid, st); break;
    case 9: rc = a.tap_mask ? rg_launch<true, 9>(a, e, grid, st) : rg_launch<false, 9>(a, e, grid, st); break;
    case 10: rc = a.tap_mask ? rg_launch<true, 10>(a, e, grid, st) : rg_launch<false, 10>(a, e, grid, st); break;
    case 16: rc = a.tap_mask ? rg_launch<true, 16>(a, e, grid, st) : rg_launch<false, 16>(a, e, grid, st); break;
#endif
    default: return CDFO_EINVAL;
  }
  if (rc) return rc;
  CDFO_LAUNCH_CHECK();
  return 0;
}
```

cdfo_amd/csrc/conv_igemm.hip:

```cpp
#include "common.h"
#include "conv_epilogue.h"

namespace {

constexpr int TW = 16;

template <int KS, int S, int TH, int NT, int KC>
struct Geo {
  static constexpr int AST = KC + 4;
  static constexpr int MT = TH / 8;
  static constexpr int BN = 32 * NT;
  static constexpr int IH = (TH - 1) * S + KS;
  static constexpr int IW = (TW - 1) * S + KS;
  static constexpr int NPIX = IH * IW;
  static constexpr int A_FLOATS = ((NPIX * AST + 3) / 4) * 4;
  static constexpr int W_FLOATS = KS * KS * (KC / 4) * BN * 4;
  static constexpr int MAIN_BYTES = (A_FLOATS + W_FLOATS) * 4;
  static constexpr int LDS_BYTES = MAIN_BYTES > ConvEpi<NT>::BLOCK_BYTES ? MAIN_BYTES : ConvEpi<NT>::BLOCK_BYTES;
};

template <int KS, int S, int TH, int NT, int KC>
__global__ __launch_bounds__(256) void conv_igemm_f32(cdfo_conv_args a) {
  using G = Geo<KS, S, TH, NT, KC>;
  constexpr int MT = G::MT, BN = G::BN, IW = G::IW, NPIX = G::NPIX, T = KS * KS, KG = KC / 4, AST = G::AST;
// ... 19 lines not shown
  for (int mi = 0; mi < MT; ++mi)
#pragma unroll
    for (int ni = 0; ni < NT; ++ni)
#pragma unroll
      for (int e = 0; e < 16; ++e) acc[mi][ni][e] = 0.f;

  int a_off[MT];
#pragma unroll
  for (int mi = 0; mi < MT; ++mi) {
    const int m = wave * MT + mi;
    a_off[mi] = (((2 * m + (r >> 4)) * S) * IW + (r & 15) * S) * AST + 4 * h;
  }
  const int b_off = (h * BN + r) * 4;

  const int nchunks = a.Cin / KC;
  int s_idx = 0, s_base = 0;
  for (int c = 0; c < nchunks; ++c) {
    const int ch0 = c * KC;
    while (ch0 >= s_base + a.cs[s_idx]) { s_base += a.cs[s_idx]; ++s_idx; }
    const float* src = a.src[s_idx];
    const int ld = a.ld[s_idx];
    const int coff = ch0 - s_base;
    __syncthreads();
    if constexpr (KS == 1 && KC == 64) {
      constexpr int NL = NPIX * KG / 256;
      static_assert(NPIX * KG % 256 == 0, "tile must divide evenly");
      f32x4 v[NL];
      bool inside[NL];
#pragma unroll
      for (int s = 0; s < NL; ++s) {
        const int idx = tid + 256 * s;
        const int p = idx / KG, q = idx - p * KG;
        const int iy = p / IW, ix = p - iy * IW;
        const int gy = iy0 + iy, gx = ix0 + ix;
        inside[s] = gy >= 0 && gy < a.H && gx >= 0 && gx < a.W;
        const long long pix = inside[s] ? ((long long)(b * a.H + gy) * a.W + gx) : 0ll;
        v[s] = *reinterpret_cast<const f32x4*>(src + pix * ld + coff + q * 4);
      }
      const bool do_ln = a.ln_gamma != nullptr;
#pragma unroll
      for (int s = 0; s < NL; ++s) {
        const int idx = tid + 256 * s;
        const int p = idx / KG, q = idx - p * KG;
        f32x4 t = v[s];
        if (do_ln) {
          float sm = (t[0] + t[1]) + (t[2] + t[3]);
#pragma unroll
          for (int o = 8; o > 0; o >>= 1) sm += __shfl_xor(sm, o, 64);
          const f32x4 d = t - sm * (1.f / 64.f);
          float sq = (d[0] * d[0] + d[1] * d[1]) + (d[2] * d[2] + d[3] * d[3]);
#pragma unroll
          for (int o = 8; o > 0; o >>= 1) sq += __shfl_xor(sq, o, 64);
          const float rstd = 1.f / sqrtf(sq * (1.f / 64.f) + 1e-5f);
          t = d * rstd * *reinterpret_cast<const f32x4*>(a.ln_gamma + q * 4) +
              *reinterpret_cast<const f32x4*>(a.ln_beta + q * 4);
        }
        if (!inside[s]) t = f32x4{0.f, 0.f, 0.f, 0.f};
        *reinterpret_cast<f32x4*>(sA + p * AST + q * 4) = t;
      }
    } else {
      for (int idx = tid; idx < NPIX * KG; idx += 256) {
        const int p = idx / KG, q = idx - p * KG;
        const int iy = p / IW, ix = p - iy * IW;
        const int gy = iy0 + iy, gx = ix0 + ix;
        f32x4 v = {0.f, 0.f, 0.f, 0.f};
        if (gy >= 0 && gy < a.H && gx >= 0 && gx < a.W)
          v = *reinterpret_cast<const f32x4*>(src + ((long long)(b * a.H + gy) * a.W + gx) * ld + coff + q * 4);
        *reinterpret_cast<f32x4*>(sA + p * AST + q * 4) = v;
      }
    }
    for (int idx = tid; idx < T * KG * BN; idx += 256) {
      const int n = idx % BN, tk = idx / BN;
      const int kg = tk % KG, t = tk / KG;
      const f32x4 v = *reinterpret_cast<const f32x4*>(
          wbase + ((long long)(t * cin4 + (ch0 >> 2) + kg) * a.CoutP + n0 + n) * 4);
      *reinterpret_cast<f32x4*>(sW + idx * 4) = v;
    }
    __syncthreads();
#pragma unroll
    for (int t = 0; t < T; ++t) {
      const int dy = t / KS, dx = t - dy * KS;
#pragma unroll
      for (int j = 0; j < KC / 8; ++j) {
        f32x4 av[MT], bv[NT];
#pragma unroll
        for (int mi = 0; mi < MT; ++mi)
          av[mi] = *reinterpret_cast<const f32x4*>(sA + a_off[mi] + (dy * IW + dx) * AST + 8 * j);
#pragma unroll
        for (int ni = 0; ni < NT; ++ni)
          bv[ni] = *reinterpret_cast<const f32x4*>(sW + ((t * KG + 2 * j) * BN + ni * 32) * 4 + b_off);
#pragma unroll
        for (int e = 0; e < 4; ++e)
#pragma unroll
          for (int mi = 0; mi < MT; ++mi)
#pragma unroll
            for (int ni = 0; ni < NT; ++ni)
              acc[mi][ni] = __builtin_amdgcn_mfma_f32_32x32x2f32(av[mi][e], bv[ni][e], acc[mi][ni], 0, 0, 0);
      }
    }
  }

  __syncthreads();
  float* wl = smem + wave * ConvEpi<NT>::WAVE_FLOATS;
#pragma unroll
  for (int mi = 0; mi < MT; ++mi)
    conv_tile_epilogue<NT>(a, wl, acc[mi], lane, b, oy0 + 2 * (wave * MT + mi), ox0, n0);
}

__global__ void pack_weight_kernel(const float* __restrict__ w, float* __restrict__ p, int Cout, int Cin, int ks,
                                   int CoutP, int shuffle2, int transposed) {
  const int T = ks * ks;
  const long long total = (long long)T * Cin * CoutP;
  for (long long i = blockIdx.x * (long long)blockDim.x + threadIdx.x; i < total;
       i += (long long)gridDim.x * blockDim.x) {
    const int e = i & 3;
    long long rest = i >> 2;
    const int n = rest % CoutP; rest /= CoutP;
    const int c4 = rest % (Cin / 4);
    const int t = rest / (Cin / 4);
    const int cin = c4 * 4 + e;
    float v = 0.f;
    if (n < Cout) {
      int o = n;
      if (shuffle2) { const int cq = Cout / 4; o = (n % cq) * 4 + n / cq; }
      if (!transposed) v = w[((long long)o * Cin + cin) * T + t];
      else v = w[((long long)cin * Cout + o) * T + (T - 1 - t)];
    }
    p[i] = v;
  }
}

template <int KS, int S, int TH, int NT, int KC>
int launch(const cdfo_conv_args& a, hipStream_t st) {
  using G = Geo<KS, S, TH, NT, KC>;
  static CdfoAttrOnce once;
  const hipError_t ea = cdfo_set_max_lds(once, reinterpret_cast<const void*>(&conv_igemm_f32<KS, S, TH, NT, KC>), G::LDS_BYTES);
  if (ea != hipSuccess) return (int)ea;
  dim3 grid(cdiv(cdiv(a.Wo, TW) * cdiv(a.Ho, TH) * a.B, 8) * 8 * (a.CoutP / G::BN));
  const int kid = KS == 1 ? KID_CONV1 : (S == 2 ? KID_CONV3_S2 : (NT == 2 ? KID_CONV3_WIDE : KID_CONV3_NARROW));
  const double px = (double)a.B * a.Ho * a.Wo;
  CdfoProfScope prof(st, kid, 2.0 * px * a.Cout * a.Cin * KS * KS,
                     4.0 * (px * a.Cout + (double)a.B * a.H * a.W * a.Cin + (double)KS * KS * a.Cin * a.Cout));
  hipLaunchKernelGGL((conv_igemm_f32<KS, S, TH, NT, KC>), grid, dim3(256), G::LDS_BYTES, st, a);
  CDFO_LAUNCH_CHECK();
  return 0;
}

}

extern "C" int cdfo_conv_igemm(const cdfo_conv_args* pa, void* stream) {
  const cdfo_conv_args& a = *pa;
  hipStream_t st = static_cast<hipStream_t>(stream);
  if (a.nsrc < 1 || a.nsrc > CDFO_MAXSRC || a.B <= 0 || a.H <= 0 || a.W <= 0) return CDFO_EINVAL;
  if (a.act == CDFO_ACT_SIGMOID || a.out2_cp16 || a.res_up2 || a.src_plane_wrap || a.res2_pixscale) return CDFO_EINVAL;
  int csum = 0;
  for (int s = 0; s < a.nsrc; ++s) {
    if (a.cs[s] <= 0 || a.cs[s] % 16 || a.ld[s] % 4 || a.ld[s] < a.cs[s]) return CDFO_EINVAL;
    if (!aligned16(a.src[s])) return CDFO_EALIGN;
    csum += a.cs[s];
  }
  if (csum != a.Cin || a.CoutP % 32 || a.CoutP < a.Cout || a.Cout <= 0) return CDFO_EINVAL;
  if (!aligned16(a.w) || a.w_bstride % 4) return CDFO_EALIGN;
  if (a.Ho != (a.H + 2 * a.pad - a.ks) / a.stride + 1 || a.Wo != (a.W + 2 * a.pad - a.ks) / a.stride + 1)
    return CDFO_EINVAL;
  if (a.store_mode == CDFO_STORE_SHUFFLE2 && (a.Cout % 16 || a.res1 || a.res2)) return CDFO_EINVAL;
  if (a.Cout % 4 || a.ldo % 4 || !aligned16(a.out) || (a.bias && !aligned16(a.bias))) return CDFO_EALIGN;
  if ((a.res1 && (a.ldr1 % 4 || !aligned16(a.res1))) || (a.res2 && (a.ldr2 % 4 || !aligned16(a.res2)))) return CDFO_EALIGN;
  if (a.prec != CDFO_PREC_F32 || a.tap_mask || a.src_f16 || a.out_f16) return CDFO_EINVAL;
  if (a.store_mode == CDFO_STORE_S2D && ((a.Ho | a.Wo) & 1 || a.res1 || a.res2)) return CDFO_EINVAL;
  const bool wide = (a.CoutP % 64) == 0;
  bool k64 = a.ks == 1 && a.stride == 1 && wide;
  for (int s = 0; s < a.nsrc; ++s) k64 = k64 && (a.cs[s] % 64 == 0);
  if (a.ln_gamma && !(k64 && a.nsrc == 1 && a.cs[0] == 64 && a.ln_beta)) return CDFO_EINVAL;
  if (a.ln_gamma && (!aligned16(a.ln_gamma) || !aligned16(a.ln_beta))) return CDFO_EALIGN;
  if (k64) return launch<1, 1, 8, 2, 64>(a, st);
  if (a.ks == 3 && a.stride == 1) return wide ? launch<3, 1, 16, 2, 16>(a, st) : launch<3, 1, 16, 1, 16>(a, st);
  if (a.ks == 1 && a.stride == 1) return wide ? launch<1, 1, 16, 2, 16>(a, st) : launch<1, 1, 16, 1, 16>(a, st);
  if (a.ks == 3 && a.stride == 2) return wide ? launch<3, 2, 8, 2, 16>(a, st) : launch<3, 2, 8, 1, 16>(a, st);
  return CDFO_EINVAL;
}

extern "C" int cdfo_pack_conv_weight(const float* w, float* packed, int Cout, int Cin, int ks, int shuffle2,
                                     int transposed, void* stream) {
  if (Cin % 4 || Cout <= 0 || ks <= 0) return CDFO_EINVAL;
  const int CoutP = (Cout + 31) / 32 * 32;
  const long long total = (long long)ks * ks * Cin * CoutP;
  const int blocks = (int)((total + 255) / 256 < 2048 ? (total + 255) / 256 : 2048);
  CdfoProfScope prof(static_cast<hipStream_t>(stream), KID_PACK, 0, 8.0 * total);
  hipLaunchKernelGGL(pack_weight_kernel, dim3(blocks), dim3(256), 0, static_cast<hipStream_t>(stream), w, packed, Cout,
                     Cin, ks, CoutP, shuffle2, transposed);
  CDFO_LAUNCH_CHECK();
  return 0;
}
```

cdfo_amd/cvsr_v8.py:

```python
from __future__ import annotations

import threading

import contextlib
import math
from typing import Dict, List, Optional, Sequence

import torch
import torch.nn as nn

from . import kernels as K
from . import switches

NF, NFRAMES = 64, 7


def _param_spec():
    sp = []

    def conv(key, co, ci, kh, kw=None, bias=True, init="default"):
        kw = kw or kh
        sp.append((key + ".weight", (co, ci, kh, kw), ci * kh * kw, init))
        if bias:
            sp.append((key + ".bias", (co,), ci * kh * kw, "zero" if init == "kaiming0.1" else "bias"))

    conv("conv_first", 64, 1, 3)
    conv("conv_second", 64, 1, 3)
    p = "transformer_feature_extraction.path1."
    for n in ("norm1", "norm2"):
        sp.append((p + n + ".body.weight", (64,), None, "ones"))
        sp.append((p + n + ".body.bias", (64,), None, "zero"))
    sp.append((p + "attn.temperature", (8, 1, 1), None, "ones"))
    conv(p + "attn.qkv", 192, 64, 1, bias=False)
    conv(p + "attn.qkv_dwconv", 192, 1, 3, bias=False)
    conv(p + "attn.project_out", 64, 64, 1, bias=False)
    conv(p + "conv", 64, 64, 3)
    u = p + "side_to_feaoneUDSA.body."
    conv(u + "0", 16, 64, 3)
    conv(u + "2", 16, 16, 3)
    conv(u + "4", 16, 16, 3)
    conv(u + "6.spatial", 1, 2, 7)
    conv(u + "7", 16, 16, 3)
    conv(u + "9", 16, 16, 3)
    conv(u + "11", 64, 16, 3)
    conv("conv_expand_fea_r", 64, 128, 3)
    conv("conv_expand_ufs", 64, 1, 3)
    conv("conv_expand_rms", 64, 1, 3)
    conv("tsa_fusion", 64, 448, 1)
    for g in range(7):
        gp = f"recon_trunk.body.{g}."
        conv(gp + "conv", 64, 64, 3)
        for b in range(3):
            bp = gp + f"body.{b}."
            conv(bp + "body.0", 256, 64, 3, init="kaiming0.1")
            conv(bp + "body.2", 64, 256, 3, init="kaiming0.1")
            conv(bp + "down.0", 64, 64, 1, init="kaiming0.1")
            conv(bp + "up.0", 64, 64, 1, init="kaiming0.1")
    conv("upconv1", 256, 64, 1)
    conv("upconv2", 256, 64, 1)
    conv("conv_last", 1, 64, 3)
    a = "MV_deform_align."
    sp.append((a + "temperature", (4, 1, 1), None, "ones"))
    conv(a + "conv_du.0", 4, 64, 1)
    conv(a + "conv_du.2", 64, 4, 1)
    conv(a + "project_out", 64, 64, 1, bias=False)
    conv(a + "fusion_in.0", 64, 128, 1)
    conv(a + "fusion_in.2", 64, 64, 1)
    conv(a + "fusion_out.0", 64, 128, 1, bias=False)
    conv(a + "CALayer.conv_du.0", 64, 64, 1)
    conv(a + "CALayer.conv_du.2", 64, 64, 1)
    for rb in ("ResidualBlock.", "ResidualBlock1."):
        conv(a + rb + "conv1", 64, 64, 3, init="kaiming0.1")
        conv(a + rb + "conv2", 64, 64, 3, init="kaiming0.1")
    r = "RDAB."
    conv(r + "input_conv", 128, 64, 1)
    conv(r + "conv_du_re.0", 64, 64, 1)
    conv(r + "conv_du_re.2", 64, 64, 3)
    conv(r + "conv_du_re2.0", 64, 64, 1)
    conv(r + "fuse", 64, 128, 1)
    conv(r + "directW1_conv", 1, 1, 1, 9)
    conv(r + "directH1_conv", 1, 1, 9, 1)
    return sp


class _Holder(nn.Module):
    """Parameter container: reproduces the reference's module tree names without its Python forward code."""


def _register(root: nn.Module, key: str, param: nn.Parameter):
    parts = key.split(".")
    m = root
    for name in parts[:-1]:
        if name not in m._modules:
            m.add_module(name, _Holder())
        m = m._modules[name]
    m.register_parameter(parts[-1], param)


class CVSR_V8(nn.Module):
    def __init__(self, nf=64, nframes=7, fea_ext_RBs=7, SCGs=4, istraining=False):
        super().__init__()
        if nf != 64 or nframes != 7:
            raise ValueError("the HIP path is specialised for nf=64, nframes=7 (the only configuration the reference runs)")
        self.nf, self.center, self.istraining, self.stride = nf, nframes // 2, istraining, 4
        self.gumbel_uniform: Optional[Sequence[torch.Tensor]] = None
        self._precision = "fp16x2"
        self.neighbour_streams = 0
        self.udsa_n16 = switches.get("CDFO_UDSA_N16")
        self.udsa_side_stream = switches.get("CDFO_UDSA_STREAM")
        self.attn_pv_single = not switches.get("CDFO_ATTN_PV3")
        self.neighbour_group = 0
        self.overlap_new_frame = switches.get("CDFO_OVERLAP_NEW")
        self.new_frame_alone = switches.get("CDFO_NEW_ALONE")
        self.trunk_side_stream = switches.get("CDFO_TRUNK_SIDE")
        self.wino_halfsplit = switches.get("CDFO_WINO_HS")
        self.fe_weight_lo = True
        self.fea_r_single_pass = switches.get("CDFO_FEA_R_1PASS")
        for key, shape, fan_in, init in _param_spec():
            t = torch.empty(shape)
            if init == "default":
                nn.init.kaiming_uniform_(t, a=math.sqrt(5))
            elif init == "kaiming0.1":
                nn.init.kaiming_normal_(t, a=0, mode="fan_in")
                t.mul_(0.1)
            elif init == "bias":
                bound = 1.0 / math.sqrt(fan_in)
                nn.init.uniform_(t, -bound, bound)
            elif init == "ones":
                t.fill_(1.0)
            else:
                t.zero_()
            _register(self, key, nn.Parameter(t))
        self.debug_taps: Optional[dict] = None
        self.capture_noise: Optional[list] = None
        self._noise_seed = 0
        self._noise_key: Optional[torch.Tensor] = None
        self.range_guard = True
        self.last_range: Optional[dict] = None
        self._probe = None
        self._warned_range = False
        self._packed: Optional[dict] = None
        self._packed_sig = None

    def _signature(self):
        return tuple((p.data_ptr(), p._version) for p in self.parameters())

    def _weights(self) -> dict:
        sig = self._signature()
        if self._packed is not None and sig == self._packed_sig:
            return self._packed
        sd = {k: v.detach() for k, v in self.named_parameters()}
        for k, v in sd.items():
            if not v.is_cuda:
                raise NotImplementedError("CVSR_V8 (HIP): parameters must live on the GPU; call .cuda() / .to(device)")
            if v.dtype != torch.float32:
                raise NotImplementedError("CVSR_V8 (HIP): fp32 parameters expected")
        w: Dict[str, object] = {}

        def pc(key, **kw):
            w[key] = K.pack_conv(sd[key + ".weight"], sd.get(key + ".bias"), **kw)

        p = "transformer_feature_extraction.path1."
        for key in (p + "attn.qkv", p + "conv", p + "side_to_feaoneUDSA.body.0", p + "side_to_feaoneUDSA.body.11",
                    "conv_expand_fea_r", "tsa_fusion", "MV_deform_align.fusion_out.0",
                    "MV_deform_align.ResidualBlock.conv1", "MV_deform_align.ResidualBlock.conv2",
                    "MV_deform_align.ResidualBlock1.conv1", "MV_deform_align.ResidualBlock1.conv2",
                    "RDAB.input_conv", "RDAB.conv_du_re.0", "RDAB.conv_du_re.2", "RDAB.fuse"):
            pc(key)
        for g in range(7):
            pc(f"recon_trunk.body.{g}.conv")
            w[f"recon_trunk.body.{g}.conv_hl2"] = K.pack_conv_hilo(sd[f"recon_trunk.body.{g}.conv.weight"],
                                                                   sd[f"recon_trunk.body.{g}.conv.bias"], weight_lo=False)
            for b in range(3):
                for leaf in ("body.0", "body.2", "down.0", "up.0"):
                    pc(f"recon_trunk.body.{g}.body.{b}.{leaf}")
        masks = []
        for ph in range(4):
            pa, pb = ph >> 1, ph & 1
            m = 0
            for dy in range(3):
                for dx in range(3):
                    if 0 <= 2 * dy + pa - 1 <= 3 and 0 <= 2 * dx + pb - 1 <= 3:
                        m |= 1 << (dy * 3 + dx)
            masks += [m] * 16
        tap_mask = torch.tensor(masks, dtype=torch.int32, device=sd["conv_first.weight"].device)
        for g in range(7):
            for b in range(3):
                bp = f"recon_trunk.body.{g}.body.{b}."
                w3, b2 = sd[bp + "body.2.weight"], sd[bp + "body.2.bias"]
                wdn, bdn = sd[bp + "down.0.weight"][:, :, 0, 0], sd[bp + "down.0.bias"]
                w4 = w3.new_zeros(64, 256, 4, 4)
                for pa in range(2):
                    for pb in range(2):
                        w4[:, :, pa:pa + 3, pb:pb + 3] += 0.25 * w3
                wp = w3.new_zeros(64, 4, 256, 3, 3)
                for ph in range(4):
                    pa, pb = ph >> 1, ph & 1
                    for dy in range(3):
                        for dx in range(3):
                            u, v = 2 * dy + pa - 1, 2 * dx + pb - 1
                            if 0 <= u <= 3 and 0 <= v <= 3:
                                wp[:, ph, :, dy, dx] = w4[:, :, u, v]
                wf = torch.einsum("po,ocyx->pcyx", wdn, wp.view(64, 1024, 3, 3)).contiguous()
                fused = K.pack_conv(wf, wdn @ b2 + bdn)
                fused.tap_mask = tap_mask
                w[bp + "down_fused"] = fused
                wup, bup = sd[bp + "up.0.weight"][:, :, 0, 0], sd[bp + "up.0.bias"]
                w[bp + "body.2_up"] = K.pack_conv(torch.einsum("po,ocyx->pcyx", wup, w3).contiguous(), wup @ b2 + bup)
                w[bp + "pro"] = K.pack_block_prologue(sd[bp + "up.0.weight"], sd[bp + "up.0.bias"],
                                                      sd[bp + "down.0.weight"], sd[bp + "down.0.bias"])
        fe = "transformer_feature_extraction.path1."
        wlo = bool(getattr(self, "fe_weight_lo", True))
        w[fe + "conv_hl"] = K.pack_conv_hilo(sd[fe + "conv.weight"], sd[fe + "conv.bias"], wlo)
        w[fe + "side_to_feaoneUDSA.body.11_hl"] = K.pack_conv_hilo(sd[fe + "side_to_feaoneUDSA.body.11.weight"],
                                                                   sd[fe + "side_to_feaoneUDSA.body.11.bias"], wlo)
        w[fe + "qkv_dw"] = K.pack_qkv_dw(sd[fe + "attn.qkv.weight"], sd[fe + "norm1.body.weight"], sd[fe + "norm1.body.bias"])
        w["rms_du0"] = K.compose_stem_1x1(sd["conv_expand_rms.weight"], sd["conv_expand_rms.bias"], sd["RDAB.conv_du_re.0.weight"],
                                          sd["RDAB.conv_du_re.0.bias"])
        w["RDAB.conv_du_re.2_s2d"] = K.pack_conv_s2p2_s2d(sd["RDAB.conv_du_re.2.weight"], sd["RDAB.conv_du_re.2.bias"])
        w[fe + "side_to_feaoneUDSA.body.0_n16"] = K.pack_conv_n16(sd[fe + "side_to_feaoneUDSA.body.0.weight"])
        w["udsa_head"] = K.pack_udsa_head(sd[fe + "side_to_feaoneUDSA.body.0.weight"], sd[fe + "side_to_feaoneUDSA.body.0.bias"],
                                          sd["conv_second.weight"], sd["conv_second.bias"])
        pc("upconv1", shuffle2=True)
        pc("upconv2", shuffle2=True)
        w["raw"] = {k: v.contiguous() for k, v in sd.items()}
        self._packed, self._packed_sig = w, sig
        return w

    PRECISIONS = {"f32": K.PREC_F32, "bf16x3": K.PREC_BF16X3, "bf16": K.PREC_BF16, "fp16x2": K.PREC_FP16X2}

    def _conv(self, *args, exact=False, inner=False, **kw):
        prec = self.PRECISIONS[self.precision]
        if exact and prec == K.PREC_FP16X2:
            prec = K.PREC_BF16X3
        elif inner and prec == K.PREC_FP16X2:
            prec = K.PREC_FP16X1
        return K.conv(*args, prec=prec, **kw)

    def _udsa(self, w, x2, res, head=None):
        raw = w["raw"]
        u = "transformer_feature_extraction.path1.side_to_feaoneUDSA.body."
        if head is not None:
            t = head
        elif self.precision != "f32" and self.udsa_n16:
            t = K.conv3x3_n16(x2, w[u + "0_n16"], raw[u + "0.bias"], K.ACT_LRELU)
        else:
            t = self._conv(x2, w[u + "0"], pad=1, act=K.ACT_LRELU, exact=True)
        t = K.small_conv16(t, raw[u + "2.weight"], raw[u + "2.bias"], 2, 2, act=K.ACT_LRELU)
        t = K.small_conv16(t, raw[u + "4.weight"], raw[u + "4.bias"], 2, 2, act=K.ACT_LRELU)
        t = K.spatial_gate16(t, raw[u + "6.spatial.weight"], raw[u + "6.spatial.bias"])
        t = K.small_conv16(t, raw[u + "7.weight"], raw[u + "7.bias"], 2, 2, 0, True, K.ACT_LRELU)
        if self.precision == "fp16x2":
            t = K.small_conv16(t, raw[u + "9.weight"], raw[u + "9.bias"], 2, 2, 1, True, K.ACT_LRELU, out_hl=True)
            return K.conv_ring(t, w[u + "11_hl"], act=K.ACT_LRELU, res1=res, plane_wrap=2)
        t = K.small_conv16(t, raw[u + "9.weight"], raw[u + "9.bias"], 2, 2, 1, True, K.ACT_LRELU)
        return self._conv(t, w[u + "11"], pad=1, act=K.ACT_LRELU, res1=res, exact=True)

    def _feature_extraction(self, w, x1, prior, P, Bn):
        raw = w["raw"]
        p = "transformer_feature_extraction.path1."
        x2 = None
        main = torch.cuda.current_stream(x1.device)
        side = self._trunk_side(x1.device) if self.udsa_side_stream else None
        for rnd in range(3):
            with (torch.cuda.stream(side) if side is not None else contextlib.nullcontext()):
                if side is not None and rnd == 0:
                    side.wait_stream(main)
                if rnd == 0:
                    x2 = self._udsa(w, None, x1, head=K.udsa_head(prior, P, Bn, self.H, self.W, w["udsa_head"]))
                else:
                    x2 = self._udsa(w, x2, x2)
                if side is not None:
                    x2.record_stream(main)
            if self.precision == "f32":
                qkv = self._conv(x1, w[p + "attn.qkv"], ln=(raw[p + "norm1.body.weight"], raw[p + "norm1.body.bias"]))
                qkv = K.dwconv3x3(qkv, raw[p + "attn.qkv_dwconv.weight"])
            else:
                v, part, n = K.qkv_dw(x1, w[p + "qkv_dw"], raw[p + "attn.qkv_dwconv.weight"], gram=True)
                fold = K.mdta_fold(part, n, raw[p + "attn.temperature"], raw[p + "attn.project_out.weight"])
                if self.precision == "fp16x2":
                    x1, ln = self._conv(v, fold, res1=x1, ln_out=(raw[p + "norm2.body.weight"], raw[p + "norm2.body.bias"]))
                else:
                    x1 = self._conv(v, fold, res1=x1)
            if self.precision == "f32":
                part, n = K.gram_partial(qkv[..., 0:64], qkv[..., 64:128], 8)
                fold = K.mdta_fold(part, n, raw[p + "attn.temperature"], raw[p + "attn.project_out.weight"])
                x1 = self._conv(qkv[..., 128:192], fold, res1=x1)
            if side is not None:
                main.wait_stream(side)
            if self.precision == "fp16x2":
                x1 = K.conv_ring(ln, w[p + "conv_hl"], res1=x1, res2=x2, plane_wrap=8)
            else:
                ln = K.layernorm64(x1, raw[p + "norm2.body.weight"], raw[p + "norm2.body.bias"])
                x1 = self._conv(ln, w[p + "conv"], pad=1, res1=x1, res2=x2, exact=True)
        return x1

    def _rdab(self, w, du0, x, noises):
        raw = w["raw"]
        GB, H, W, _ = x.shape
        G = len(noises)
        B = GB // G
        t = self._conv(du0, w["RDAB.conv_du_re.2_s2d"], pad=1, act=K.ACT_RELU, exact=True)
        part, n = K.chan_sum_partial(t)
        vmax = K.vec_mlp(part, n, t.shape[1] * t.shape[2], raw["RDAB.conv_du_re2.0.weight"],
                         raw["RDAB.conv_du_re2.0.bias"], 64, K.ACT_RELU)
        xq = self._conv(x, w["RDAB.input_conv"])
        sq, vrow, qwin = (K.empty_act(GB, H, W, 64, x.device) for _ in range(3))
        for g, noise in enumerate(noises):
            sl = slice(g * B, (g + 1) * B)
            outs = (sq[sl], vrow[sl], qwin[sl])
            if isinstance(noise, tuple):
                _, seed, draw, capture = noise
                K.rdab_prep_rng(xq[sl], vmax[sl], seed, draw, raw["RDAB.directW1_conv.weight"], raw["RDAB.directW1_conv.bias"],
                                noise_out=capture, outs=outs)
            else:
                K.rdab_prep(xq[sl], vmax[sl], noise, raw["RDAB.directW1_conv.weight"], raw["RDAB.directW1_conv.bias"], outs=outs)
        cat = K.empty_act(GB, H, W, 128, x.device)
        am = 20 if self.precision == "fp16x2" and self.attn_pv_single else 0
        rowo = K.seq_attn(sq, vrow, am)
        qc = K.colconv9(sq, raw["RDAB.directH1_conv.weight"], raw["RDAB.directH1_conv.bias"])
        K.seq_attn(qc, rowo, am + 1, out=cat[..., 0:64])
        K.seq_attn(qwin, xq[..., 64:128], am + 2, out=cat[..., 64:128])
        return self._conv(cat, w["RDAB.fuse"], res1=x)

    def _align(self, w, xc, extra, pred, mvs, mv_bstride, out):
        raw = w["raw"]
        a = "MV_deform_align."
        GB, H, W, _ = xc.shape
        B = GB // len(mvs)
        warped = K.empty_act(GB, H, W, NF, xc.device)
        for g, mv in enumerate(mvs):
            K.flow_warp(extra[g * B:(g + 1) * B], mv, mv_bstride, out=warped[g * B:(g + 1) * B])
        kf = self._conv([warped, pred], w[a + "fusion_out.0"], act=K.ACT_RELU)
        gp, ng = K.gram_partial(xc, kf, 16)
        sw, ns = K.chan_sum_partial(warped)
        sp, _ = K.chan_sum_partial(pred)
        fold = K.align_fold(gp, ng, sw, sp, ns, H * W, raw[a + "temperature"], raw[a + "conv_du.0.weight"],
                            raw[a + "conv_du.0.bias"], raw[a + "conv_du.2.weight"], raw[a + "conv_du.2.bias"],
                            raw[a + "project_out.weight"], raw[a + "fusion_out.0.weight"])
        o = self._conv([warped, pred, xc], fold, act=K.ACT_RELU)
        part, n = K.chan_sum_partial(o)
        gate = K.vec_mlp(part, n, H * W, raw[a + "CALayer.conv_du.0.weight"], raw[a + "CALayer.conv_du.0.bias"], 64,
                         K.ACT_RELU, raw[a + "CALayer.conv_du.2.weight"], raw[a + "CALayer.conv_du.2.bias"], 64,
                         K.ACT_SIGMOID)
        rb = [w[a + n] for n in ("ResidualBlock.conv1", "ResidualBlock.conv2", "ResidualBlock1.conv1", "ResidualBlock1.conv2")]
        fast16 = self.precision == "fp16x2" and H % 2 == 0 and all(c.wh is not None for c in rb)
        if fast16:
            o, o16 = K.scale_channels(o, gate, want_cp16=True)
        else:
            o = K.scale_channels(o, gate)
        if fast16:
            n16 = torch.empty_like(o16)
            o = K.conv3x3_ws_res(K.conv3x3_ws(o16, rb[0], act=K.ACT_RELU), rb[1], res1=o, out2_cp16=n16)
            return K.conv3x3_ws_res(K.conv3x3_ws(n16, rb[2], act=K.ACT_RELU), rb[3], res1=o, res2=xc, out=out)
        r = self._conv(o, rb[0], pad=1, act=K.ACT_RELU)
        o = self._conv(r, rb[1], pad=1, res1=o)
        r = self._conv(o, rb[2], pad=1, act=K.ACT_RELU)
        return self._conv(r, rb[3], pad=1, res1=o, res2=xc, out=out)

    def _block(self, w, p, x, x16=None, want16=False, want_hl=False):
        b0, b2, dn, up = w[p + "body.0"], w[p + "body.2"], w[p + "down.0"], w[p + "up.0"]
        t16 = self.precision == "fp16x2"
        if t16 and x.shape[1] % 4 == 0 and b0.wh is not None:
            c1 = lambda src, **kw: K.conv3x3_body0(src, b0, act=K.ACT_LRELU, **kw)
            up2 = (b0.ww is not None and K.wino_up2_enabled() and x.shape[1] % 2 == 0 and x.shape[2] % 2 == 0
                   and x.shape[1] * x.shape[2] * 8 * b0.Cout < (1 << 31))
            if x16 is None:
                u16, d16, x16 = K.block_prologue(x, w[p + "pro"], want_x16=True, lowres_up=up2)
            else:
                u16, d16 = K.block_prologue(x, w[p + "pro"], lowres_up=up2)
            hs = up2 and self.wino_halfsplit
            c2 = (lambda src: K.conv3x3_wino_up2(src, b0, act=K.ACT_LRELU, halfsplit=hs)) if up2 else (lambda src: c1(src, s2d=True))
            side = self._trunk_side(x.device) if self.trunk_side_stream else None
            if side is not None:
                main = torch.cuda.current_stream(x.device)
                side.wait_stream(main)
                with torch.cuda.stream(side):
                    d = K.conv_ring(c1(d16), w[p + "body.2_up"])
                out = K.conv_ring(c1(x16), b2, res1=x)
                t = c2(u16)
                main.wait_stream(side)
                d.record_stream(main)
            else:
                out = K.conv_ring(c1(x16), b2, res1=x)
                d = K.conv_ring(c1(d16), w[p + "body.2_up"])
                t = c2(u16)
            y16 = torch.empty_like(x16) if want16 else None
            if want_hl:
                y16 = torch.empty((x16.shape[0], 8) + tuple(x16.shape[2:]), dtype=torch.float16, device=x16.device)
            y = K.conv_ring(t, w[p + "down_fused"], res1=out, res_up2=d, out2_cp16=y16, out2_hl=want_hl, src_halfsplit=hs)
            return (y, y16) if (want16 or want_hl) else y
        out = self._conv(self._conv(x, b0, pad=1, act=K.ACT_LRELU, out_f16=t16, inner=True), b2, pad=1, res1=x)
        d = self._conv(K.resample2(x, up=False), dn)
        d = self._conv(self._conv(d, b0, pad=1, act=K.ACT_LRELU, out_f16=t16, inner=True), b2, pad=1)
        K.resample2(self._conv(d, up), up=True, out=out, accumulate=True)
        u = K.resample2(self._conv(x, up), up=True, out_f16=t16)
        t = self._conv(u, b0, pad=1, act=K.ACT_LRELU, s2d=True, out_f16=t16, inner=True)
        y = self._conv(t, w[p + "down_fused"], pad=1, res1=out)
        return (y, None) if want16 else y

    def _trunk_side(self, device):
        cache = self.__dict__.setdefault("_trunk_side_streams", {})
        st = cache.get(device)
        if st is None:
            st = cache[device] = torch.cuda.Stream(device)
        return st

    def _trunk(self, w, fused):
        y = fused
        for g in range(7):
            r, r16 = y, None
            fast = self.precision == "fp16x2" and y.shape[1] % 4 == 0 and w[f"recon_trunk.body.{g}.body.0.body.0"].wh is not None
            for b in range(3):
                if b < 2:
                    r, r16 = self._block(w, f"recon_trunk.body.{g}.body.{b}.", r, r16, want16=True)
                elif fast:
                    r, r16 = self._block(w, f"recon_trunk.body.{g}.body.{b}.", r, r16, want_hl=True)
                else:
                    r, r16 = self._block(w, f"recon_trunk.body.{g}.body.{b}.", r, r16), None
            if fast:
                y = K.conv_ring(r16, w[f"recon_trunk.body.{g}.conv_hl2"], res1=y, res2=fused if g == 6 else None)
            else:
                y = self._conv(r, w[f"recon_trunk.body.{g}.conv"], pad=1, res1=y, res2=fused if g == 6 else None)
        return y

    _tls = threading.local()

    @property
    def precision(self) -> str:
        ov = getattr(CVSR_V8._tls, "override", None)
        if ov is not None and ov[0] is self:
            return ov[1]
        return self._precision

    @precision.setter
    def precision(self, value: str):
        if value not in self.PRECISIONS:
            raise ValueError(f"precision must be one of {sorted(self.PRECISIONS)}, got {value!r}")
        self._precision = value

    def _resolve_noise(self, x, gumbel_uniform):
        noise = gumbel_uniform if gumbel_uniform is not None else self.gumbel_uniform
        if noise is None:
            if torch.cuda.is_current_stream_capturing():
                if self._noise_key is None or self._noise_key.device != x.device:
                    raise RuntimeError("CVSR_V8 (HIP): call model.refresh_noise_key(device) before capturing a forward "
                                       "that draws its own Gumbel noise")
                self._noise_seed = self._noise_key
            else:
                self._noise_seed = K.next_noise_seed(x.device)
        return noise

    def forward(self, x, mvs0, mvs1, pms, rms, ufs, pre_L1_fea=None, gumbel_uniform=None):
        if not x.is_cuda:
            raise NotImplementedError("CVSR_V8 (HIP): CPU tensors are not supported; there is no CPU fallback")
        with K.on_device(x):
            training = torch.is_grad_enabled() and any(p.requires_grad for p in self.parameters())
            if training and torch.cuda.is_current_stream_capturing():
                raise RuntimeError("CVSR_V8 (HIP): the autograd path cannot be captured into a HIP graph (its mask kernel takes the "
                                   "Philox key as a launch argument); capture inference forwards under torch.no_grad()")
            noise = self._resolve_noise(x, gumbel_uniform)
            if training:
                if pre_L1_fea is not None:
                    raise NotImplementedError("CVSR_V8 (HIP): the cached-feature path is an inference path; training uses fresh clips")
                for prm in self.parameters():
                    if not prm.is_cuda or prm.dtype != torch.float32:
                        raise NotImplementedError("CVSR_V8 (HIP): fp32 parameters on the GPU expected")
                from .cvsr_v8_train import forward_train
                return forward_train(self, x, mvs0, mvs1, pms, rms, ufs, noise)
            guard = self.precision == "fp16x2" and self.range_guard
            if not guard:
                return self._forward(x, mvs0, mvs1, pms, rms, ufs, pre_L1_fea, noise)
            capturing = torch.cuda.is_current_stream_capturing()
            if capturing:
                probe = self.__dict__.get("_graph_probe")
                if probe is None:
                    raise RuntimeError("CVSR_V8 (HIP): the fp16 range guard reads probes back and cannot be captured by hand; use "
                                       "model.capture(), whose graph carries the two probes and whose replay() reads them back")
                probe.zero_()
            else:
                probe = torch.zeros(4, dtype=torch.int32, device=x.device)
            self._probe = probe
            try:
                res = self._forward(x, mvs0, mvs1, pms, rms, ufs, pre_L1_fea, noise)
            finally:
                self._probe = None
            if capturing:
                return res
            pinned = self.__dict__.setdefault("_guard_pinned", {})
            if x.device not in pinned:
                pinned[x.device] = torch.zeros(4, dtype=torch.int32).pin_memory()
            host = pinned[x.device]
            host.copy_(probe, non_blocking=True)
            ev = torch.cuda.Event()
# ... 220 lines not shown
```

cdfo_amd/kernels.py:

```python
from __future__ import annotations

import contextlib
import ctypes as C
from dataclasses import dataclass
from typing import Optional, Sequence

import torch

from . import _lib, switches
from ._lib import CdfoError, ConvArgs, check

ACT_NONE, ACT_LRELU, ACT_RELU, ACT_SIGMOID = 0, 1, 2, 3
PREC_F32, PREC_BF16X3, PREC_BF16, PREC_FP16X2, PREC_FP16, PREC_FP16X1 = 0, 1, 2, 3, 4, 5


def _stream() -> C.c_void_p:
    return C.c_void_p(torch.cuda.current_stream().cuda_stream)


def on_device(t: torch.Tensor):
    if not t.is_cuda:
        raise NotImplementedError("the HIP path needs device tensors (there is no CPU fallback)")
    return torch.cuda.device(t.device)


def _p(t: Optional[torch.Tensor]) -> Optional[int]:
    return None if t is None else t.data_ptr()


def _chk_act(t: torch.Tensor, name: str = "tensor", dtype=torch.float32):
    if not t.is_cuda:
        raise NotImplementedError(f"{name}: the HIP path needs device tensors (no CPU fallback)")
    if t.device.index != torch.cuda.current_device():
        raise CdfoError(f"{name} lives on {t.device} but the current device is cuda:{torch.cuda.current_device()}: "
                        "enter kernels.on_device(tensor) (the module forwards do) before calling the wrappers")
    if t.dtype != dtype or t.dim() != 4 or t.stride(3) != 1:
        raise ValueError(f"{name}: expected fp32 [B,H,W,C] with contiguous channels, got {t.dtype} {tuple(t.shape)} "
                         f"strides {t.stride()}")
    B, H, W, Cc = t.shape
    ld = t.stride(2)
    if (W > 1 and t.stride(1) != W * ld) or (B > 1 and t.stride(0) != H * W * ld):
        raise ValueError(f"{name}: rows/images must be densely packed at pitch ld={ld}, strides {t.stride()}")
    return B, H, W, Cc, ld


def empty_act(B: int, H: int, W: int, Cc: int, device) -> torch.Tensor:
    return torch.empty((B, H, W, Cc), dtype=torch.float32, device=device)


def nchw_to_nhwc(x: torch.Tensor, out: Optional[torch.Tensor] = None) -> torch.Tensor:
    B, Cc, H, W = x.shape
    x = x.contiguous()
    if out is None:
        out = empty_act(B, H, W, Cc, x.device)
    _, _, _, _, ldo = _chk_act(out, "out")
    check(_lib.lib().cdfo_nchw_to_nhwc(C.c_void_p(x.data_ptr()), C.c_void_p(out.data_ptr()), B, Cc, H, W, ldo,
                                       _stream()), "cdfo_nchw_to_nhwc")
    return out


def nhwc_to_nchw(x: torch.Tensor) -> torch.Tensor:
    B, H, W, Cc, ld = _chk_act(x, "x")
    out = torch.empty((B, Cc, H, W), dtype=torch.float32, device=x.device)
    check(_lib.lib().cdfo_nhwc_to_nchw(C.c_void_p(x.data_ptr()), ld, C.c_void_p(out.data_ptr()), B, Cc, H, W,
                                       _stream()), "cdfo_nhwc_to_nchw")
    return out


def range_probe(x: torch.Tensor, slots: torch.Tensor) -> None:
    if not x.is_contiguous() or x.dtype != torch.float32 or x.numel() % 4:
        raise ValueError("range_probe: dense fp32 tensor with a multiple of 4 elements expected")
    check(_lib.lib().cdfo_range_probe(C.c_void_p(x.data_ptr()), C.c_longlong(x.numel()), C.c_void_p(slots.data_ptr()),
                                      _stream()), "cdfo_range_probe")


@dataclass
class PackedConv:
    w: torch.Tensor
    bias: Optional[torch.Tensor]
    Cout: int
    Cin: int
    ks: int
    CoutP: int
    shuffle2: bool = False
    w_bstride: int = 0
    wq: Optional[torch.Tensor] = None
    tap_mask: Optional[torch.Tensor] = None
    wh: Optional[torch.Tensor] = None
    CoutP16: int = 0
    wh_sparse: Optional[torch.Tensor] = None
    ww: Optional[torch.Tensor] = None


def pack_conv(weight: torch.Tensor, bias: Optional[torch.Tensor], shuffle2: bool = False,
              transposed: bool = False) -> PackedConv:
    w = weight.detach().contiguous().float()
    if transposed:
        Cin, Cout, ks, _ = w.shape
    else:
        Cout, Cin, ks, _ = w.shape
    CoutP = (Cout + 31) // 32 * 32
    packed = torch.empty(ks * ks * Cin * CoutP, dtype=torch.float32, device=w.device)
    check(_lib.lib().cdfo_pack_conv_weight(C.c_void_p(w.data_ptr()), C.c_void_p(packed.data_ptr()), Cout, Cin, ks,
                                           int(shuffle2), int(transposed), _stream()), "cdfo_pack_conv_weight")
    b = None
    if bias is not None:
        b = bias.detach().contiguous().float()
        if shuffle2:
            cq = Cout // 4
            b = b.view(cq, 4).t().contiguous().view(-1)
    pc = PackedConv(packed, b, Cout, Cin, ks, CoutP, shuffle2)
    if ks == 3 and not transposed and not shuffle2 and Cout % 4 == 0 and Cin % 16 == 0:
        cp16 = (Cout + 63) // 64 * 64
        pc.CoutP16 = cp16
        wq = torch.empty(2 * (Cin // 16) * 18 * cp16 * 8, dtype=torch.bfloat16, device=w.device)
        check(_lib.lib().cdfo_pack_conv3x3_bf16(C.c_void_p(w.data_ptr()), C.c_void_p(wq.data_ptr()), Cout, Cin,
                                                _stream()), "cdfo_pack_conv3x3_bf16")
        pc.wq = wq
        wh = torch.empty((Cin // 16) * 18 * cp16 * 8, dtype=torch.float16, device=w.device)
        check(_lib.lib().cdfo_pack_conv3x3_f16(C.c_void_p(w.data_ptr()), C.c_void_p(wh.data_ptr()), Cout, Cin, _stream()),
              "cdfo_pack_conv3x3_f16")
        pc.wh = wh
        if Cin == 64 and Cout % 128 == 0:
            ww = torch.empty(Cout * 64 * 12, dtype=torch.float16, device=w.device)
            check(_lib.lib().cdfo_pack_conv3x3_wino(C.c_void_p(w.data_ptr()), C.c_void_p(ww.data_ptr()), Cout, _stream()),
                  "cdfo_pack_conv3x3_wino")
            pc.ww = ww
    return pc


def conv(srcs: Sequence[torch.Tensor], pc: PackedConv, *, stride: int = 1, pad: int = 0, act: int = ACT_NONE,
         res1: Optional[torch.Tensor] = None, res2: Optional[torch.Tensor] = None,
         out: Optional[torch.Tensor] = None, prec: int = PREC_F32,
         ln: Optional[tuple] = None, s2d: bool = False, out_f16: bool = False, ln_out: Optional[tuple] = None,
         res2_scale: Optional[torch.Tensor] = None, cp16_out: bool = False):
    if isinstance(srcs, torch.Tensor):
        srcs = [srcs]
    a = ConvArgs()
    B = H = W = None
    cin = 0
    src_f16 = srcs[0].dtype == torch.float16
    if src_f16:
        prec = PREC_FP16
    elif prec == PREC_FP16:
        raise ValueError("PREC_FP16 needs an fp16 source tensor")
    odt = torch.float16 if out_f16 else torch.float32
    for i, s in enumerate(srcs):
        b_, h_, w_, c_, ld_ = _chk_act(s, f"src{i}", torch.float16 if src_f16 else torch.float32)
        if B is None:
            B, H, W = b_, h_, w_
        elif (B, H, W) != (b_, h_, w_):
            raise ValueError("conv sources disagree on B/H/W")
        a.src[i] = s.data_ptr()
        a.ld[i] = ld_
        a.cs[i] = c_
        cin += c_
    if cin != pc.Cin:
        raise ValueError(f"conv: sources have {cin} channels, weight expects {pc.Cin}")
    a.nsrc = len(srcs)
    Ho = (H + 2 * pad - pc.ks) // stride + 1
    Wo = (W + 2 * pad - pc.ks) // stride + 1
    a.B, a.H, a.W, a.Ho, a.Wo = B, H, W, Ho, Wo
    a.ks, a.stride, a.pad = pc.ks, stride, pad
    a.Cin, a.Cout, a.CoutP = pc.Cin, pc.Cout, pc.CoutP
    a.w = pc.w.data_ptr()
    a.w_bstride = pc.w_bstride
    a.bias = _p(pc.bias)
    a.act = act
    if pc.shuffle2:
        if out is None:
            out = empty_act(B, 2 * Ho, 2 * Wo, pc.Cout // 4, srcs[0].device)
        a.store_mode = 1
    elif s2d:
        if out is None:
            out = torch.empty((B, Ho // 2, Wo // 2, 4 * pc.Cout), dtype=odt, device=srcs[0].device)
        a.store_mode = 2
    else:
        if out is None:
            out = torch.empty((B, Ho, Wo, pc.Cout), dtype=odt, device=srcs[0].device)
        a.store_mode = 0
    _, _, _, _, a.ldo = _chk_act(out, "out", odt)
    a.src_f16, a.out_f16 = int(src_f16), int(out_f16)
    a.out = out.data_ptr()
    for nm, r in (("res1", res1), ("res2", res2)):
        if r is not None:
            rb, rh, rw, rc, rld = _chk_act(r, nm)
            if (rb, rh, rw) != (B, Ho, Wo) or rc < pc.Cout:
                raise ValueError(f"{nm} shape {tuple(r.shape)} does not match the conv output")
            setattr(a, nm, r.data_ptr())
            setattr(a, "ldr" + nm[-1], rld)
    if res2_scale is not None:
        if res2 is None or tuple(res2_scale.shape) != (B, Ho, Wo) or not res2_scale.is_contiguous() or res2_scale.dtype != torch.float32:
            raise ValueError("conv: res2_scale must be a contiguous fp32 [B,H,W] plane next to res2")
        a.res2_pixscale = res2_scale.data_ptr()
    if (prec != PREC_F32 and pc.wq is not None and stride == 1 and pad == 1 and pc.w_bstride == 0):
        a.prec = prec
        a.CoutP = pc.CoutP16
        a.w = (pc.wh if prec in (PREC_FP16X2, PREC_FP16, PREC_FP16X1) else pc.wq).data_ptr()
        a.tap_mask = _p(pc.tap_mask)
        check(_lib.lib().cdfo_conv3x3_bf16(C.byref(a), _stream()), "cdfo_conv3x3_bf16")
        return out
    if src_f16 or out_f16:
        raise ValueError("fp16 tensors are only supported by the 16-bit MFMA 3x3 kernel")
    a.prec = 0
    if ln is not None:
        a.ln_gamma, a.ln_beta = ln[0].data_ptr(), ln[1].data_ptr()
    if (prec != PREC_F32 and pc.ks == 1 and stride == 1 and pad == 0 and pc.CoutP % 64 == 0 and pc.CoutP <= 256
            and all(s.shape[3] % 64 == 0 for s in srcs)):
        if cp16_out:
            if ln_out is not None or ln is not None or pc.Cout != 64 or pc.CoutP != 64:
                raise ValueError("conv: cp16_out needs a plain 64-channel 1x1 convolution")
            copy = torch.empty((B, 4, Ho, Wo, 16), dtype=torch.float16, device=out.device)
            a.out2_cp16 = copy.data_ptr()
            check(_lib.lib().cdfo_conv1x1_bf16x3(C.byref(a), _stream()), "cdfo_conv1x1_bf16x3")
            return out, copy
        planes = None
        if ln_out is not None and pc.Cout == 64 and pc.CoutP == 64 and ln is None:
            planes = torch.empty((B, 8, Ho, Wo, 16), dtype=torch.float16, device=out.device)
            a.out2_cp16, a.ln_gamma, a.ln_beta = planes.data_ptr(), ln_out[0].data_ptr(), ln_out[1].data_ptr()
        check(_lib.lib().cdfo_conv1x1_bf16x3(C.byref(a), _stream()), "cdfo_conv1x1_bf16x3")
        if ln_out is not None:
            return out, (planes if planes is not None else layernorm64_hl(out, ln_out[0], ln_out[1]))
        return out
    check(_lib.lib().cdfo_conv_igemm(C.byref(a), _stream()), "cdfo_conv_igemm")
    if ln_out is not None:
        return out, layernorm64_hl(out, ln_out[0], ln_out[1])
    if cp16_out:
        return out, to_cp16(out)
    return out


def _vp(t):
    return C.c_void_p(None if t is None else t.data_ptr())


@contextlib.contextmanager
def cu_limit(n: int):
    prev = _lib.lib().cdfo_set_cu_limit(int(n))
    try:
        yield
    finally:
        _lib.lib().cdfo_set_cu_limit(prev)


def conv_offset_mask(src: torch.Tensor, pc: PackedConv, offset: torch.Tensor, mask: torch.Tensor, flow: torch.Tensor, mag: float,
                     accumulate: bool, prec: int) -> None:
    B, H, W, Cc, ld = _chk_act(src)
    third = pc.Cout // 3
    if (pc.ks != 3 or Cc != pc.Cin or pc.Cout % 3 or pc.wq is None or W % 4 or prec not in (PREC_BF16X3, PREC_FP16X2, PREC_FP16X1)
            or tuple(offset.shape) != (B, 2 * third, H, W) or tuple(mask.shape) != (B, third, H, W) or tuple(flow.shape) != (B, 2, H, W)
            or not (offset.is_contiguous() and mask.is_contiguous() and flow.is_contiguous())
            or any(t.dtype != torch.float32 for t in (offset, mask, flow))):
        raise ValueError("conv_offset_mask: unsupported configuration")
    a = ConvArgs()
    a.src[0], a.ld[0], a.cs[0], a.nsrc = src.data_ptr(), ld, Cc, 1
    a.B, a.H, a.W, a.Ho, a.Wo = B, H, W, H, W
    a.ks, a.stride, a.pad = 3, 1, 1
    a.Cin, a.Cout, a.CoutP = pc.Cin, pc.Cout, pc.CoutP16
    a.w = (pc.wh if prec in (PREC_FP16X2, PREC_FP16X1) else pc.wq).data_ptr()
    a.bias = _p(pc.bias)
    a.act, a.prec, a.store_mode = ACT_NONE, prec, 4
    a.out, a.ldo = offset.data_ptr(), 4
    a.mask_out, a.flow, a.flow_bstride = mask.data_ptr(), flow.data_ptr(), 2 * H * W
    a.off_mag, a.off_accumulate = float(mag), int(accumulate)
    check(_lib.lib().cdfo_conv3x3_bf16(C.byref(a), _stream()), "cdfo_conv3x3_bf16 (offset / mask epilogue)")


def pack_conv_n16(weight: torch.Tensor) -> torch.Tensor:
    if tuple(weight.shape) != (16, 64, 3, 3):
        raise ValueError("pack_conv_n16: a [16, 64, 3, 3] weight expected")
    w = weight.detach().float().permute(2, 3, 1, 0).reshape(9, 2, 4, 8, 16).permute(0, 1, 2, 4, 3).reshape(18, 64, 8)
    hi = w.to(torch.bfloat16)
    lo = (w - hi.float()).to(torch.bfloat16)
    return torch.stack([hi, lo], 1).contiguous()


def conv3x3_n16(x: torch.Tensor, w_packed: torch.Tensor, bias: Optional[torch.Tensor], act: int = ACT_NONE) -> torch.Tensor:
    B, H, W, Cc, ld = _chk_act(x)
    if Cc != 64 or w_packed.dtype != torch.bfloat16 or w_packed.numel() != 18 * 2 * 64 * 8:
        raise ValueError("conv3x3_n16: 64 input channels and a pack_conv_n16 weight image expected")
    out = empty_act(B, H, W, 16, x.device)
    check(_lib.lib().cdfo_conv3x3_c64_n16(_vp(x), ld, B, H, W, _vp(w_packed), _vp(bias), act, _vp(out), 16, _stream()),
          "cdfo_conv3x3_c64_n16")
    return out


def to_cp16(x: torch.Tensor) -> torch.Tensor:
    B, H, W, Cc, ld = _chk_act(x)
    out = torch.empty((B, Cc // 16, H, W, 16), dtype=torch.float16, device=x.device)
    check(_lib.lib().cdfo_to_cp16(_vp(x), ld, B, C.c_longlong(H * W), Cc, _vp(out), _stream()), "cdfo_to_cp16")
    return out


def conv3x3_ws(src: torch.Tensor, pc: PackedConv, *, act: int = ACT_NONE, s2d: bool = False,
               out: Optional[torch.Tensor] = None, dbg: int = 0, clk: Optional[torch.Tensor] = None) -> torch.Tensor:
    if not src.is_cuda:
        raise NotImplementedError("conv3x3_ws: the HIP path needs device tensors (no CPU fallback)")
    if src.dtype != torch.float16 or src.dim() != 5 or src.shape[1] != 4 or src.shape[4] != 16 or not src.is_contiguous():
        raise ValueError(f"conv3x3_ws: expected a contiguous fp16 [B,4,H,W,16] source, got {src.dtype} {tuple(src.shape)}")
    if pc.wh is None or pc.Cin != 64 or pc.ks != 3 or pc.Cout % 64:
        raise ValueError("conv3x3_ws: needs a 3x3 weight with 64 input channels and Cout % 64 == 0")
    B, _, H, W, _ = src.shape
    shape = (B, pc.Cout // 4, H // 2, W // 2, 16) if s2d else (B, pc.Cout // 16, H, W, 16)
    if out is None:
        out = torch.empty(shape, dtype=torch.float16, device=src.device)
    elif out.shape != shape or out.dtype != torch.float16 or not out.is_contiguous():
        raise ValueError(f"conv3x3_ws: out must be a contiguous fp16 tensor of shape {shape}")
    per_img = 4 * H * W * 32
    step = max(1, min(B, ((1 << 31) - 1) // per_img))
    if per_img >= (1 << 31):
        raise ValueError(f"conv3x3_ws: one {H}x{W} image exceeds the 2 GiB source limit of a launch")
    for b0 in range(0, B, step):
        nb = min(step, B - b0)
        check(_lib.lib().cdfo_conv3x3_c64_ws(_vp(src[b0:b0 + nb]), nb, H, W, _vp(pc.wh), pc.CoutP16, _vp(pc.bias), pc.Cout,
                                             act, _vp(out[b0:b0 + nb]), 2 if s2d else 0, dbg, _vp(clk), _stream()),
              "cdfo_conv3x3_c64_ws")
    return out


def wino_enabled() -> bool:
    return switches.get("CDFO_WINO")


def halfsplit_to_rows(t: torch.Tensor) -> torch.Tensor:
    B, P, H, W, _ = t.shape
    return t.reshape(B, P, H, 2, W, 8).permute(0, 1, 2, 4, 3, 5).reshape(B, P, H, W, 16)


def conv3x3_wino(src: torch.Tensor, pc: PackedConv, *, act: int = ACT_NONE, s2d: bool = False,
                 out: Optional[torch.Tensor] = None, dbg: int = 0, halfsplit: bool = False, clk: Optional[torch.Tensor] = None) -> torch.Tensor:
    if not src.is_cuda:
        raise NotImplementedError("conv3x3_wino: the HIP path needs device tensors (no CPU fallback)")
    if src.dtype != torch.float16 or src.dim() != 5 or src.shape[1] != 4 or src.shape[4] != 16 or not src.is_contiguous():
        raise ValueError(f"conv3x3_wino: expected a contiguous fp16 [B,4,H,W,16] source, got {src.dtype} {tuple(src.shape)}")
    if pc.ww is None:
        raise ValueError("conv3x3_wino: needs a 3x3 weight with 64 input channels and Cout % 128 == 0")
    B, _, H, W, _ = src.shape
    shape = (B, pc.Cout // 4, H // 2, W // 2, 16) if s2d else (B, pc.Cout // 16, H, W, 16)
    if out is None:
        out = torch.empty(shape, dtype=torch.float16, device=src.device)
    elif out.shape != shape or out.dtype != torch.float16 or not out.is_contiguous():
        raise ValueError(f"conv3x3_wino: out must be a contiguous fp16 tensor of shape {shape}")
    if halfsplit and not s2d:
        raise ValueError("conv3x3_wino: half-split rows exist for the space-to-depth store only")
    mode = (5 if halfsplit else 2) if s2d else 0
    if dbg:
        check(_lib.lib().cdfo_conv3x3_c64_wino_dbg(_vp(src), B, H, W, _vp(pc.ww), _vp(pc.bias), pc.Cout, act, _vp(out), mode,
                                                   dbg, _vp(clk), _stream()), "cdfo_conv3x3_c64_wino_dbg")
        return out
    check(_lib.lib().cdfo_conv3x3_c64_wino(_vp(src), B, H, W, _vp(pc.ww), _vp(pc.bias), pc.Cout, act, _vp(out), mode,
                                           _stream()), "cdfo_conv3x3_c64_wino")
    return out


def wino_up2_enabled() -> bool:
    return wino_enabled() and switches.get("CDFO_WINO_UP2")


def conv3x3_wino_up2(src_lr: torch.Tensor, pc: PackedConv, *, act: int = ACT_NONE, halfsplit: bool = False) -> torch.Tensor:
    if not src_lr.is_cuda:
        raise NotImplementedError("conv3x3_wino_up2: the HIP path needs device tensors (no CPU fallback)")
    if src_lr.dtype != torch.float16 or src_lr.dim() != 5 or src_lr.shape[1] != 4 or src_lr.shape[4] != 16 or not src_lr.is_contiguous():
        raise ValueError(f"conv3x3_wino_up2: expected a contiguous fp16 [B,4,h,w,16] source, got {src_lr.dtype} {tuple(src_lr.shape)}")
    B, _, h, w, _ = src_lr.shape
    if pc.ww is None or h % 2 or w % 2:
        raise ValueError("conv3x3_wino_up2: needs a Winograd weight image (Cout % 128 == 0) and even low-resolution sizes")
    out = torch.empty((B, pc.Cout // 4, h, w, 16), dtype=torch.float16, device=src_lr.device)
    check(_lib.lib().cdfo_conv3x3_c64_wino_up2(_vp(src_lr), B, 2 * h, 2 * w, _vp(pc.ww), _vp(pc.bias), pc.Cout, act, _vp(out),
                                               5 if halfsplit else 2, _stream()), "cdfo_conv3x3_c64_wino_up2")
    return out


def conv3x3_body0(src: torch.Tensor, pc: PackedConv, *, act: int = ACT_NONE, s2d: bool = False) -> torch.Tensor:
    _, _, H, W, _ = src.shape
    if pc.ww is not None and wino_enabled() and W % 2 == 0 and (not s2d or H % 2 == 0) and H * W * 2 * pc.Cout < (1 << 31):
        return conv3x3_wino(src, pc, act=act, s2d=s2d)
    return conv3x3_ws(src, pc, act=act, s2d=s2d)


def conv_offset_mask_ws_fits(B: int, H: int, W: int, third: int) -> bool:
    return 4 * H * W * 32 * B < (1 << 31) and H * W * 2 * third * 4 < (1 << 31)


def conv_offset_mask_ws(src: torch.Tensor, pc: PackedConv, offset: torch.Tensor, mask: torch.Tensor, flow: torch.Tensor, mag: float,
                        accumulate: bool) -> None:
    if src.dtype != torch.float16 or src.dim() != 5 or src.shape[1] != 4 or src.shape[4] != 16 or not src.is_contiguous():
        raise ValueError(f"conv_offset_mask_ws: expected a contiguous fp16 [B,4,H,W,16] source, got {src.dtype} {tuple(src.shape)}")
    B, _, H, W, _ = src.shape
# ... 317 lines not shown

def scale_channels(x: torch.Tensor, gate: torch.Tensor, want_cp16: bool = False):
    B, H, W, Cc, ld = _chk_act(x)
    out = empty_act(B, H, W, Cc, x.device)
    o16 = torch.empty((B, Cc // 16, H, W, 16), dtype=torch.float16, device=x.device) if want_cp16 else None
    check(_lib.lib().cdfo_scale_channels(_vp(x), ld, _vp(gate), B, C.c_longlong(H * W), Cc, _vp(out), Cc, _vp(o16),
                                         _stream()), "cdfo_scale_channels")
    return (out, o16) if want_cp16 else out


def upconv_last(x: torch.Tensor, pc: PackedConv, w_last: torch.Tensor, b_last: torch.Tensor, xc: torch.Tensor,
                xc_bstride: int) -> torch.Tensor:
    B, H2, W2, Cc, ld = _chk_act(x)
    if not pc.shuffle2 or pc.Cout != 256 or pc.Cin != Cc or pc.ks != 1:
        raise ValueError("upconv_last: needs the pixel-shuffle packing of a 1x1 conv with 256 outputs")
    taps = torch.empty((B, 2 * H2, 2 * W2, 12), dtype=torch.float32, device=x.device)
    a = ConvArgs()
    a.src[0], a.ld[0], a.cs[0], a.nsrc = x.data_ptr(), ld, Cc, 1
    a.B, a.H, a.W, a.Ho, a.Wo = B, H2, W2, H2, W2
    a.ks, a.stride, a.pad = 1, 1, 0
    a.Cin, a.Cout, a.CoutP = pc.Cin, pc.Cout, pc.CoutP
    a.w, a.bias, a.act = pc.w.data_ptr(), _p(pc.bias), ACT_LRELU
    a.res2 = w_last.detach().contiguous().float().data_ptr()
    a.out, a.ldo, a.store_mode = taps.data_ptr(), 12, 3
    check(_lib.lib().cdfo_conv1x1_bf16x3(C.byref(a), _stream()), "cdfo_conv1x1_bf16x3 (tap sums)")
    out = torch.empty((B, 1, 2 * H2, 2 * W2), dtype=torch.float32, device=x.device)
    check(_lib.lib().cdfo_conv_last_taps(_vp(taps), 12, _vp(b_last), _vp(xc), C.c_longlong(xc_bstride), B, 2 * H2, 2 * W2,
                                         _vp(out), _stream()), "cdfo_conv_last_taps")
    return out


def conv_last(x: torch.Tensor, w: torch.Tensor, bias: torch.Tensor, xc: torch.Tensor, xc_bstride: int) -> torch.Tensor:
    B, Hh, Wh, Cc, ld = _chk_act(x)
    assert Cc == 64
    out = torch.empty((B, 1, Hh, Wh), dtype=torch.float32, device=x.device)
    check(_lib.lib().cdfo_conv_last(_vp(x), ld, _vp(w), _vp(bias), _vp(xc), C.c_longlong(xc_bstride), B, Hh, Wh,
                                    _vp(out), _stream()), "cdfo_conv_last")
    return out


def small_conv16(x: torch.Tensor, w: torch.Tensor, bias: torch.Tensor, stride: int, pad: int, out_pad: int = 0,
                 transposed: bool = False, act: int = ACT_NONE, out_hl: bool = False) -> torch.Tensor:
    B, H, W, Cc, ld = _chk_act(x)
    assert Cc == 16
    if transposed:
        Ho, Wo = (H - 1) * stride - 2 * pad + 3 + out_pad, (W - 1) * stride - 2 * pad + 3 + out_pad
    else:
        Ho, Wo = (H + 2 * pad - 3) // stride + 1, (W + 2 * pad - 3) // stride + 1
    if out_hl:
        hl = torch.empty((B, 2, Ho, Wo, 16), dtype=torch.float16, device=x.device)
        check(_lib.lib().cdfo_small_conv16_hl(_vp(x), ld, _vp(w), _vp(bias), B, H, W, stride, pad, out_pad, int(transposed), act,
                                              _vp(hl), _stream()), "cdfo_small_conv16_hl")
        return hl
    out = empty_act(B, Ho, Wo, 16, x.device)
    check(_lib.lib().cdfo_small_conv16(_vp(x), ld, _vp(w), _vp(bias), B, H, W, stride, pad, out_pad, int(transposed),
                                       act, _vp(out), 16, _stream()), "cdfo_small_conv16")
    return out


def spatial_gate16(x: torch.Tensor, w: torch.Tensor, bias: torch.Tensor) -> torch.Tensor:
    B, H, W, Cc, ld = _chk_act(x)
    assert Cc == 16
    out = empty_act(B, H, W, 16, x.device)
    check(_lib.lib().cdfo_spatial_gate16(_vp(x), ld, _vp(w), _vp(bias), B, H, W, _vp(out), 16, _stream()),
          "cdfo_spatial_gate16")
    return out


def chan_pool(x: torch.Tensor) -> torch.Tensor:
    B, H, W, Cc, ld = _chk_act(x)
    out = torch.empty((B, H, W, 2), dtype=torch.float32, device=x.device)
    check(_lib.lib().cdfo_chan_pool(_vp(x), ld, C.c_longlong(B * H * W), Cc, _vp(out), _stream()), "cdfo_chan_pool")
    return out


def gate_map_cumulative(pooled: torch.Tensor, cum: Optional[torch.Tensor], w: torch.Tensor, bias: torch.Tensor) -> torch.Tensor:
    B, H, W, two = pooled.shape
    if two != 2 or not pooled.is_contiguous() or (cum is not None and (tuple(cum.shape) != (B, H, W) or not cum.is_contiguous())):
        raise ValueError("gate_map_cumulative: pooled [B,H,W,2] and cum [B,H,W] expected")
    out = torch.empty((B, H, W), dtype=torch.float32, device=pooled.device)
    check(_lib.lib().cdfo_gate_map_cumulative(_vp(pooled), _vp(cum), _vp(w), _vp(bias), B, H, W, int(w.shape[-1]), _vp(out), _stream()),
          "cdfo_gate_map_cumulative")
    return out


def spatial_gate(x: torch.Tensor, w: torch.Tensor, bias: torch.Tensor) -> torch.Tensor:
    B, H, W, Cc, ld = _chk_act(x)
    out = empty_act(B, H, W, Cc, x.device)
    gate = torch.empty((B, H, W), dtype=torch.float32, device=x.device)
    check(_lib.lib().cdfo_spatial_gate(_vp(x), ld, _vp(chan_pool(x)), _vp(w), _vp(bias), B, H, W, Cc, int(w.shape[-1]),
                                       _vp(gate), _vp(out), Cc, _stream()), "cdfo_spatial_gate")
    return out


def rdab_mix(xf: torch.Tensor, xc: torch.Tensor, w3: torch.Tensor, b3: torch.Tensor, vmax: torch.Tensor,
             noise: torch.Tensor) -> torch.Tensor:
    B, H, W, Cc, ld = _chk_act(xf)
    if tuple(noise.shape) != (B, 64, H, W) or not noise.is_contiguous() or noise.dtype != torch.float32:
        raise ValueError(f"rdab_mix: noise must be a contiguous fp32 [B,64,H,W] tensor, got {tuple(noise.shape)}")
    if tuple(vmax.shape) != (B, 64) or tuple(w3.shape) != (1, 2, 3, 3):
        raise ValueError("rdab_mix: vmax must be [B,64] and the spatial weight [1,2,3,3]")
    out = empty_act(B, H, W, 64, xf.device)
    check(_lib.lib().cdfo_rdab_mix(_vp(xf), ld, _vp(chan_pool(xc)), _vp(w3), _vp(b3), _vp(vmax), _vp(noise), B, H, W,
                                   _vp(out), 64, _stream()), "cdfo_rdab_mix")
    return out


def shrink_planes(t: torch.Tensor, level: int) -> torch.Tensor:
    B, Cc, H, W = t.shape
    if t.stride(3) != 1 or t.stride(2) != W or t.stride(1) != H * W:
        t = t.contiguous()
    out = torch.empty((B, Cc, H >> level, W >> level), dtype=torch.float32, device=t.device)
    check(_lib.lib().cdfo_shrink_planes(_vp(t), C.c_longlong(t.stride(0)), Cc, B, H, W, level, _vp(out), _stream()),
          "cdfo_shrink_planes")
    return out


def lincomb(a: torch.Tensor, ca: float, b: Optional[torch.Tensor] = None, cb: float = 0.0,
            c: Optional[torch.Tensor] = None, cc: float = 0.0, out: Optional[torch.Tensor] = None) -> torch.Tensor:
    for t in (a, b, c, out):
        if t is not None and (not t.is_contiguous() or t.dtype != torch.float32 or t.shape != a.shape):
            raise ValueError("lincomb: contiguous fp32 tensors of one shape expected")
    if out is None:
        out = torch.empty_like(a)
    check(_lib.lib().cdfo_lincomb(_vp(out), _vp(a), float(ca), _vp(b), float(cb), _vp(c), float(cc),
                                  C.c_longlong(a.numel()), _stream()), "cdfo_lincomb")
    return out


def nchunks_for(P: int) -> int:
    return max(1, min(128, P // 1024))


def chan_sum_partial(x: torch.Tensor):
    B, H, W, Cc, ld = _chk_act(x)
    assert Cc == 64
    n = nchunks_for(H * W)
    part = torch.empty((B, n, 64), dtype=torch.float32, device=x.device)
    check(_lib.lib().cdfo_chan_sum_partial(_vp(x), ld, B, C.c_longlong(H * W), n, _vp(part), _stream()),
          "cdfo_chan_sum_partial")
    return part, n


def gram_partial(q: torch.Tensor, k: torch.Tensor, ch_per_head: int):
    B, H, W, Cc, ldq = _chk_act(q, "q")
    _, _, _, _, ldk = _chk_act(k, "k")
    n = nchunks_for(H * W)
    part = torch.empty((B, n, 64 * (ch_per_head + 2)), dtype=torch.float32, device=q.device)
    check(_lib.lib().cdfo_gram_partial(_vp(q), ldq, _vp(k), ldk, B, C.c_longlong(H * W), ch_per_head, n, _vp(part),
                                       _stream()), "cdfo_gram_partial")
    return part, n


def mdta_fold(part: torch.Tensor, n: int, temperature: torch.Tensor, proj_w: torch.Tensor) -> PackedConv:
    B = part.shape[0]
    wout = torch.empty((B, 4096), dtype=torch.float32, device=part.device)
    check(_lib.lib().cdfo_mdta_fold(_vp(part), n, _vp(temperature), _vp(proj_w), B, _vp(wout), _stream()),
          "cdfo_mdta_fold")
    return PackedConv(wout, None, 64, 64, 1, 64, False, 4096)


_FOLD_CIN = {}


def fold_scale_inputs(fold: PackedConv, gate: torch.Tensor) -> PackedConv:
    if fold.Cin != 64 or fold.Cout != 64 or fold.ks != 1 or fold.w_bstride != 4096 or tuple(gate.shape) != (fold.w.shape[0], 64):
        raise ValueError("fold_scale_inputs: a mdta_fold result and a [B, 64] gate expected")
    cin = _FOLD_CIN.get(gate.device)
    if cin is None:
        i = torch.arange(4096, device=gate.device)
        cin = (i // 1024) * 16 + ((i // 256) % 4) * 4 + i % 4
        if not (gate.is_cuda and torch.cuda.is_current_stream_capturing()):
            _FOLD_CIN[gate.device] = cin
    return PackedConv(fold.w * gate[:, cin], None, 64, 64, 1, 64, False, 4096)


def align_fold(gpart, ng, sw, sp, ns, P, temperature, du0_w, du0_b, du2_w, du2_b, proj_w, fusion_w) -> PackedConv:
    B = gpart.shape[0]
    wout = torch.empty((B, 192 * 64), dtype=torch.float32, device=gpart.device)
    check(_lib.lib().cdfo_align_fold(_vp(gpart), ng, _vp(sw), _vp(sp), ns, C.c_longlong(P), _vp(temperature),
                                     _vp(du0_w), _vp(du0_b), _vp(du2_w), _vp(du2_b), _vp(proj_w), _vp(fusion_w), B,
                                     _vp(wout), _stream()), "cdfo_align_fold")
    return PackedConv(wout, None, 64, 192, 1, 64, False, 192 * 64)


def vec_mlp(part: torch.Tensor, n: int, P: int, w1, b1, c1: int, act1: int, w2=None, b2=None, c2: int = 0,
            act2: int = ACT_NONE) -> torch.Tensor:
    B = part.shape[0]
    out = torch.empty((B, c2 if w2 is not None else c1), dtype=torch.float32, device=part.device)
    check(_lib.lib().cdfo_vec_mlp(_vp(part), n, C.c_longlong(P), _vp(w1), _vp(b1), c1, act1, _vp(w2), _vp(b2), c2, act2,
                                  B, _vp(out), _stream()), "cdfo_vec_mlp")
    return out


def _prep_outs(outs, B, H, W, device):
    if outs is None:
        return empty_act(B, H, W, 64, device), empty_act(B, H, W, 64, device), empty_act(B, H, W, 64, device)
    for t in outs:
        if tuple(t.shape) != (B, H, W, 64) or not t.is_contiguous() or t.dtype != torch.float32:
            raise ValueError("rdab_prep: outs must be three dense fp32 [B,H,W,64] tensors")
    return outs


def rdab_prep(xq: torch.Tensor, vmax: torch.Tensor, noise: torch.Tensor, wW: torch.Tensor, bW: torch.Tensor, outs=None):
    B, H, W, Cc, ld = _chk_act(xq)
    assert Cc == 128 and noise.is_contiguous() and tuple(noise.shape) == (B, 64, H, W)
    sq, vrow, qwin = _prep_outs(outs, B, H, W, xq.device)
    check(_lib.lib().cdfo_rdab_prep(_vp(xq), ld, _vp(vmax), _vp(noise), _vp(wW), _vp(bW), B, C.c_longlong(H * W),
                                    _vp(sq), 64, _vp(vrow), 64, _vp(qwin), 64, _stream()), "cdfo_rdab_prep")
    return sq, vrow, qwin


def rdab_prep_rng(xq: torch.Tensor, vmax: torch.Tensor, seed: int, draw: int, wW: torch.Tensor, bW: torch.Tensor,
                  noise_out: Optional[torch.Tensor] = None, outs=None):
    B, H, W, Cc, ld = _chk_act(xq)
    assert Cc == 128
    if noise_out is not None and (tuple(noise_out.shape) != (B, 64, H, W) or not noise_out.is_contiguous()
                                  or noise_out.dtype != torch.float32):
        raise ValueError("rdab_prep_rng: noise_out must be a contiguous fp32 [B,64,H,W] tensor")
    sq, vrow, qwin = _prep_outs(outs, B, H, W, xq.device)
    if isinstance(seed, torch.Tensor):
        if seed.dtype != torch.int64 or seed.numel() != 1 or seed.device != xq.device:
            raise ValueError("rdab_prep_rng: a device-side key must be an int64[1] tensor on the operands' device")
        check(_lib.lib().cdfo_rdab_prep_rng_dev(_vp(xq), ld, _vp(vmax), _vp(seed), draw, _vp(noise_out), _vp(wW), _vp(bW), B,
                                                C.c_longlong(H * W), _vp(sq), 64, _vp(vrow), 64, _vp(qwin), 64, _stream()),
              "cdfo_rdab_prep_rng_dev")
        return sq, vrow, qwin
    check(_lib.lib().cdfo_rdab_prep_rng(_vp(xq), ld, _vp(vmax), C.c_longlong(seed & 0x7FFFFFFFFFFFFFFF), draw, _vp(noise_out),
                                        _vp(wW), _vp(bW), B, C.c_longlong(H * W), _vp(sq), 64, _vp(vrow), 64, _vp(qwin), 64,
                                        _stream()), "cdfo_rdab_prep_rng")
    return sq, vrow, qwin


_seed_counter = 0


def next_noise_seed(device) -> int:
    global _seed_counter
    if torch.cuda.is_current_stream_capturing():
        base, off = int(torch.initial_seed()), 4 * _seed_counter
        _seed_counter += 1
    else:
        g = torch.cuda.default_generators[device.index if device.index is not None else torch.cuda.current_device()]
        base, off = int(g.initial_seed()), int(g.get_offset())
        g.set_offset(off + 4)
    return (base * 0x9E3779B97F4A7C15 + off * 0xD1B54A32D192ED03 + 0x632BE59BD9B4E019) & 0x7FFFFFFFFFFFFFFF


def colconv9(x: torch.Tensor, wH: torch.Tensor, bH: torch.Tensor) -> torch.Tensor:
    B, H, W, Cc, ld = _chk_act(x)
    out = empty_act(B, H, W, 64, x.device)
    check(_lib.lib().cdfo_colconv9(_vp(x), ld, _vp(wH), _vp(bH), B, H, W, _vp(out), 64, _stream()), "cdfo_colconv9")
    return out


def seq_attn(q: torch.Tensor, v: torch.Tensor, mode: int, out: Optional[torch.Tensor] = None) -> torch.Tensor:
    B, H, W, Cc, ldq = _chk_act(q, "q")
    _, _, _, _, ldv = _chk_act(v, "v")
    if out is None:
        out = empty_act(B, H, W, 64, q.device)
    _, _, _, _, ldo = _chk_act(out, "out")
    check(_lib.lib().cdfo_seq_attn(_vp(q), ldq, _vp(v), ldv, _vp(out), ldo, B, H, W, mode, _stream()), "cdfo_seq_attn")
    return out
```

cdfo_amd/switches.py:

```python
from __future__ import annotations

import functools
import os
from typing import NamedTuple, Optional, Tuple, Union

ONOFF, INT, PATH = "on/off", "int", "path"


class Switch(NamedTuple):
    name: str
    default: Union[int, None]
    kind: str
    layer: str
    meaning: str
    values: Optional[Tuple[int, ...]] = None


TABLE = (
    Switch("CDFO_LIB_PATH", None, PATH, "python", "another build of libcdfo_hip.so (A/B builds, the developer library cdfo_amd/lib/dev/)"),
    Switch("CDFO_DCN_EXACT", 0, ONOFF, "python", "1: the DCN forward always on its exact-fp32 kernel (cdfo_amd.dcn.EXACT_FP32)"),
    Switch("CDFO_TRAIN_EXACT", 0, ONOFF, "python", "1: the training path's convolutions on exact-fp32 MFMA (cdfo_amd.autograd.CONV_PREC = PREC_F32)"),
    Switch("CDFO_WINO", 1, ONOFF, "python", "0: Block_.body[0] stays on the direct weights-stationary kernel instead of the Winograd F(2,3) one"),
    Switch("CDFO_WINO_UP2", 1, ONOFF, "python", "0: Block_'s x2 branch on a materialised double-resolution source instead of the interpolating Winograd form"),
    Switch("CDFO_WINO_HS", 0, ONOFF, "python", "1: the x2 branch's 256-channel intermediate in half-split rows (model.wino_halfsplit; measured: no gain in the forward, 105.2 vs 105.3 ms)"),
    Switch("CDFO_UDSA_N16", 1, ONOFF, "python", "0: the prior U-net's first layer off the 16-channel kernel (model.udsa_n16)"),
    Switch("CDFO_UDSA_STREAM", 1, ONOFF, "python", "0: the prior U-net on the caller's stream instead of a side stream (model.udsa_side_stream)"),
    Switch("CDFO_ATTN_PV3", 0, ONOFF, "python", "1: all three fp16 passes in the attentions' second product instead of one (model.attn_pv_single = False)"),
    Switch("CDFO_OVERLAP_NEW", 1, ONOFF, "python", "0: streaming, frames 0-2 start behind the new frame's feature extraction, not beside it (model.overlap_new_frame)"),
    Switch("CDFO_NEW_ALONE", 1, ONOFF, "python", "0: streaming, the new frame's neighbour pipeline is not a group of its own (model.new_frame_alone)"),
    Switch("CDFO_TRUNK_SIDE", 1, ONOFF, "python", "0: Block_'s half-resolution branch on the caller's stream instead of a side stream (model.trunk_side_stream)"),
    Switch("CDFO_FEA_R_1PASS", 0, ONOFF, "python", "1: conv_expand_fea_r with activations rounded once to fp16 (model.fea_r_single_pass)"),
    Switch("CDFO_V7_FEAR_1PASS", 1, ONOFF, "python", "0: CVSR_V7's conv_expand_fea_r on fp16 hi + lo activations, two passes (model.fea_r_single_pass)"),
    Switch("CDFO_V7_FUSE_ASSEMBLY", 1, ONOFF, "python", "0: MVDualAttAlignment assembles offsets / masks in a kernel of its own (fuse_assembly)"),
    Switch("CDFO_V7_HEAD_1PASS", 1, ONOFF, "python", "0: MVDualAttAlignment's offset head on two-pass activations (head_one_pass)"),
    Switch("CDFO_V7_OFF0_1PASS", 1, ONOFF, "python", "0: MVDualAttAlignment's conv_offset[0] on two-pass activations (off0_one_pass)"),
    Switch("CDFO_V7_WS_HEAD", 1, ONOFF, "python", "0: MVDualAttAlignment's offset head off the weights-stationary kernel (ws_head)"),
    Switch("CDFO_WS_RING", 1, ONOFF, "hip", "0: Block_.body[0] on the private-halo kernel of rounds 1-2 instead of the ring-fed wave-specialised one"),
    Switch("CDFO_WS_MFMA16", 1, ONOFF, "hip", "0: the ring-fed weights-stationary kernel on v_mfma_f32_32x32x16_f16 instead of 16x16x32"),
    Switch("CDFO_WS_WAVES", 12, INT, "hip", "8: two instead of three waves per SIMD in the private-halo weights-stationary kernel", (8, 12)),
    Switch("CDFO_RING_SPLIT", 1, ONOFF, "hip", "0: the four-tap ring convolution on the eight-identical-waves kernel"),
    Switch("CDFO_RING_MFMA16", 1, ONOFF, "hip", "0: the wave-specialised ring kernel's consumers on 32x32x16"),
    Switch("CDFO_RING_TOUCH", 0, ONOFF, "hip", "1: producer-side touches of the tile's residual lines ahead of the epilogue (measured useless, off)"),
    Switch("CDFO_CONV1X1_STREAM", 1, ONOFF, "hip", "0: 1x1 convolutions on the one-tile-per-workgroup kernel instead of the persistent streaming one"),
    Switch("CDFO_TAPS_STREAM", 1, ONOFF, "hip", "0: the CDFO_STORE_TAPS9 1x1 convolution off the persistent streaming kernel"),
    Switch("CDFO_ATTN_NW", 0, INT, "hip", "4 | 8: force the attention workgroup width (0: chosen per shape)", (0, 4, 8)),
    Switch("CDFO_ATTN_XCD", 1, INT, "hip", "0: attention workgroups of one sequence spread over the XCDs as in round 2"),
    Switch("CDFO_DCN_WIN", 1, INT, "hip", "0: the DCN forward on the round-2 gather kernel instead of the window-sampled one"),
    Switch("CDFO_DCN_DBG", 0, INT, "hip", "developer library only (-DCDFO_DEV_ABLATIONS): ablation code of the window-sampled DCN kernel, wrong results"),
)
_ROWS = {s.name: s for s in TABLE}


def _parse(sw: Switch, raw: Optional[str]):
    if sw.kind == PATH:
        return raw or None
    if raw is None:
        return bool(sw.default) if sw.kind == ONOFF else sw.default
    if sw.kind == ONOFF and raw in ("0", "1"):
        return raw == "1"
    if sw.kind == INT and raw.lstrip("-").isdigit() and (sw.values is None or int(raw) in sw.values):
        return int(raw)
    allowed = "0 or 1" if sw.kind == ONOFF else ("one of %s" % (sw.values,) if sw.values else "an integer")
    raise ValueError(f"{sw.name}={raw!r}: expected {allowed} (cdfo_amd/switches.py)")


@functools.lru_cache(maxsize=None)
def get(name: str):
    sw = _ROWS[name]
    if sw.layer != "python":
        raise KeyError(f"{name} is read by the HIP library, not by Python")
    return _parse(sw, os.environ.get(name))


def check_hip_environment() -> None:
    for sw in TABLE:
        if sw.layer == "hip":
            _parse(sw, os.environ.get(sw.name))
```

include/cdfo_hip.h:

```cpp
#ifndef CDFO_HIP_H
#define CDFO_HIP_H

#ifdef __cplusplus
extern "C" {
#endif

#define CDFO_EINVAL (-1)
#define CDFO_EALIGN (-2)
#define CDFO_MAXSRC 8

enum { CDFO_ACT_NONE = 0, CDFO_ACT_LRELU = 1, CDFO_ACT_RELU = 2, CDFO_ACT_SIGMOID = 3 };
enum { CDFO_STORE_PLAIN = 0, CDFO_STORE_SHUFFLE2 = 1, CDFO_STORE_S2D = 2, CDFO_STORE_TAPS9 = 3, CDFO_STORE_OFFMASK = 4,
       CDFO_STORE_S2D_HS = 5  };
enum { CDFO_DTYPE_F32 = 0, CDFO_DTYPE_F16 = 1, CDFO_DTYPE_F64 = 2 };
enum { CDFO_PREC_F32 = 0, CDFO_PREC_BF16X3 = 1, CDFO_PREC_BF16 = 2, CDFO_PREC_FP16X2 = 3, CDFO_PREC_FP16 = 4, CDFO_PREC_FP16X1 = 5 };

int cdfo_abi_version(void);
const char* cdfo_build_info(void);
int cdfo_set_cu_limit(int n);

typedef struct {
  const float* src[CDFO_MAXSRC]; int ld[CDFO_MAXSRC]; int cs[CDFO_MAXSRC]; int nsrc;
  int B, H, W, Ho, Wo;
  int ks, stride, pad;
  int Cin, Cout, CoutP;
  const float* w; long long w_bstride; const float* bias;
  int act;
  const float* res1; int ldr1;
  const float* res2; int ldr2;
  float* out; int ldo; int store_mode;
  int prec;
  const float* ln_gamma; const float* ln_beta;
  const unsigned* tap_mask;
  int src_f16;
  int out_f16;
  void* out2_cp16;
  int src_plane_wrap;
  const float* res_up2; int ldru;
  int out2_lo;
  float* mask_out; const float* flow; long long flow_bstride; float off_mag; int off_accumulate;
  const float* res2_pixscale;
  int src_halfsplit;
} cdfo_conv_args;
int cdfo_sizeof_conv_args(void);
int cdfo_conv_igemm(const cdfo_conv_args* a, void* stream);

int cdfo_pack_conv_weight(const float* w_oihw, float* packed, int Cout, int Cin, int ks, int shuffle2,
                          int transposed, void* stream);

int cdfo_conv3x3_bf16(const cdfo_conv_args* a, void* stream);
int cdfo_pack_conv3x3_bf16(const float* w_oihw, void* packed, int Cout, int Cin, void* stream);
int cdfo_pack_conv3x3_f16(const float* w_oihw, void* packed, int Cout, int Cin, void* stream);

int cdfo_conv3x3_c64_ws(const void* src_cp16, int B, int H, int W, const void* w_f16, int CoutP, const float* bias,
                        int Cout, int act, void* out_cp16, int store_mode, int dbg, void* clk_probe, void* stream);
int cdfo_conv3x3_c64_wino(const void* src_cp16, int B, int H, int W, const void* w_wino, const float* bias, int Cout, int act,
                          void* out_cp16, int store_mode, void* stream);
int cdfo_pack_conv3x3_wino(const float* w_oihw, void* packed, int Cout, void* stream);
int cdfo_conv3x3_c64_wino_up2(const void* src_lr_cp16, int B, int H, int W, const void* w_wino, const float* bias, int Cout, int act,
                              void* out_cp16, int store_mode, void* stream);
int cdfo_conv3x3_c64_wino_dbg(const void* src_cp16, int B, int H, int W, const void* w_wino, const float* bias, int Cout, int act,
                              void* out_cp16, int store_mode, int dbg, void* clk_probe, void* stream);
int cdfo_conv3x3_c64_ws_offmask(const void* src_cp16, int B, int H, int W, const void* w_f16, int CoutP, const float* bias, int Cout,
                                float* offset, float* mask, const float* flow, long long flow_bstride, float mag, int accumulate,
                                void* stream);

int cdfo_conv3x3_c64_ws_res(const void* src_cp16, int B, int H, int W, const void* w_f16, int CoutP, const float* bias,
                            int Cout, int act, float* out, int ldo, const float* res1, int ldr1, const float* res2,
                            int ldr2, void* out2_cp16, void* stream);
int cdfo_conv3x3_ring(const cdfo_conv_args* a, void* stream);
int cdfo_to_cp16(const float* in, int ldi, int B, long long P, int C, void* out_cp16, void* stream);

int cdfo_conv1x1_bf16x3(const cdfo_conv_args* a, void* stream);

int cdfo_conv_last_taps(const float* taps, int ldt, const float* bias, const float* xc, long long xc_bstride, int B, int Hh,
                        int Wh, float* out, void* stream);
int cdfo_nchw_to_nhwc(const float* in, float* out, int B, int C, int H, int W, int ldo, void* stream);
int cdfo_nhwc_to_nchw(const float* in, int ldi, float* out, int B, int C, int H, int W, void* stream);
int cdfo_swap_outer(const float* in, float* out, int B, int N, long long block, void* stream);
int cdfo_range_probe(const float* x, long long n, void* slots2, void* stream);

int cdfo_stem_conv(const float* img, long long img_bstride, const float* w, const float* bias, int B, int H, int W,
                   int act, float* out, int ldo, const float* add, int lda, float* out2, int ldo2, void* stream);
int cdfo_stem_conv2(const float* img, long long img_bstride, const float* wA, const float* bA, const float* add, int lda,
                    float* outA, int ldoA, const float* wB, const float* bB, int actB, float* outB, int ldoB, int s2dB, int B,
                    int H, int W, void* stream);
int cdfo_layernorm64(const float* in, int ldi, const float* gamma, const float* beta, long long npix, float* out,
                     int ldo, void* stream);
int cdfo_layernorm64_cp16hl(const float* in, int ldi, const float* gamma, const float* beta, int B, long long P, void* out,
                            void* stream);
int cdfo_dwconv3x3(const float* in, int ldi, const float* w, int B, int H, int W, int C, float* out, int ldo,
                   void* stream);
int cdfo_flow_warp(const float* in, int ldi, const float* mv, long long mv_bstride, int B, int H, int W, int C,
                   float* out, int ldo, void* stream);
int cdfo_resample2(const float* in, int ldi, int B, int H, int W, int C, float* out, int ldo, int up, int accumulate,
                   int out_f16, void* stream);
int cdfo_scale_channels(const float* in, int ldi, const float* gate, int B, long long P, int C, float* out, int ldo,
                        void* out_cp16, void* stream);
int cdfo_conv_last(const float* in, int ldi, const float* w, const float* bias, const float* xc, long long xc_bstride,
                   int B, int Hh, int Wh, float* out, void* stream);

int cdfo_small_conv16(const float* in, int ldi, const float* w, const float* bias, int B, int H, int W, int stride,
                      int pad, int out_pad, int transposed, int act, float* out, int ldo, void* stream);
int cdfo_small_conv16_hl(const float* in, int ldi, const float* w, const float* bias, int B, int H, int W, int stride,
                         int pad, int out_pad, int transposed, int act, void* out_hl, void* stream);
int cdfo_udsa_head(const float* img, long long img_bstride, const float* wc, const float* bt, const float* b0, int B, int H,
                   int W, float* out, int ldo, void* stream);
int cdfo_spatial_gate16(const float* in, int ldi, const float* w, const float* bias, int B, int H, int W, float* out,
                        int ldo, void* stream);

int cdfo_chan_sum_partial(const float* in, int ldi, int B, long long P, int nchunk, float* partial, void* stream);
int cdfo_gram_partial(const float* q, int ldq, const float* k, int ldk, int B, long long P, int ch_per_head, int nchunk,
                      float* partial, void* stream);
int cdfo_mdta_fold(const float* partial, int nchunk, const float* temperature, const float* proj_w, int B, float* wout,
                   void* stream);
int cdfo_align_fold(const float* gram_partial, int nchunk_g, const float* sum_warp, const float* sum_pred, int nchunk_s,
                    long long P, const float* temperature, const float* du0_w, const float* du0_b, const float* du2_w,
                    const float* du2_b, const float* proj_w, const float* fusion_w, int B, float* wout, void* stream);
int cdfo_vec_mlp(const float* sum_partial, int nchunk, long long P, const float* w1, const float* b1, int c1, int act1,
                 const float* w2, const float* b2, int c2, int act2, int B, float* out, void* stream);

int cdfo_rdab_prep(const float* xq, int ldx, const float* vmax, const float* noise, const float* wW, const float* bW,
                   int B, long long P, float* sq, int lds_, float* vrow, int ldv, float* qwin, int ldw, void* stream);
int cdfo_rdab_prep_rng(const float* xq, int ldx, const float* vmax, long long seed, int draw, float* noise_out,
                       const float* wW, const float* bW, int B, long long P, float* sq, int lds_, float* vrow, int ldv,
                       float* qwin, int ldw, void* stream);
int cdfo_rdab_prep_rng_dev(const float* xq, int ldx, const float* vmax, const void* seed_dev, int draw, float* noise_out,
                           const float* wW, const float* bW, int B, long long P, float* sq, int lds_, float* vrow, int ldv,
                           float* qwin, int ldw, void* stream);
int cdfo_colconv9(const float* in, int ldi, const float* wH, const float* bH, int B, int H, int W, float* out, int ldo,
                  void* stream);
int cdfo_metric_partials(const float* a, const float* b, int N, int H, int W, int crop, float scale, int clamp, int round8,
                         int metric, double* partial, int partial_cap, int* nblocks_out, void* stream);
int cdfo_block_prologue(const float* x, int ldx, int B, int H, int W, const void* w_bf16, const float* bias128, void* u16,
                        void* d16, void* x16, void* stream);
int cdfo_block_prologue2(const float* x, int ldx, int B, int H, int W, const void* w_bf16, const float* bias128, void* u16, void* t16,
                         void* d16, void* x16, void* stream);
int cdfo_qkv_dw_gram_slots(int B, int H, int W);
int cdfo_qkv_dw(const float* x, int ldx, int B, int H, int W, const void* w_bf16, const float* bias, const float* dw_w,
                float eps, float* out, int ldo, float* gram, int gram_slots, void* stream);
int cdfo_seq_attn(const float* q, int ldq, const float* v, int ldv, float* out, int ldo, int B, int H, int W, int mode,
                  void* stream);

long long cdfo_dcn_workspace_bytes(int B, int C, int H, int W, int Co, int kh, int kw, int groups, int deformable_groups);
int cdfo_dcn_forward(const float* in, const float* offset, const float* mask, const float* weight, const float* bias,
                     float* out, int B, int C, int H, int W, int Co, int kh, int kw, int sh, int sw, int ph, int pw,
                     int dh, int dw, int groups, int deformable_groups, void* workspace, long long workspace_bytes,
                     void* stream);

int cdfo_dcn_backward(const float* in, const float* offset, const float* mask, const float* weight,
                      const float* grad_out, float* grad_in, float* grad_offset, float* grad_mask, float* grad_weight,
                      float* grad_bias, int B, int C, int H, int W, int Co, int kh, int kw, int sh, int sw, int ph,
                      int pw, int dh, int dw, int groups, int deformable_groups, float scale, void* stream);
long long cdfo_dcn_backward_workspace_bytes(int B, int C, int H, int W, int Co, int kh, int kw, int sh, int sw, int ph,
                                            int pw, int dh, int dw, int groups, int deformable_groups);
int cdfo_dcn_backward_ws(const float* in, const float* offset, const float* mask, const float* weight,
                         const float* grad_out, float* grad_in, float* grad_offset, float* grad_mask, float* grad_weight,
                         float* grad_bias, int B, int C, int H, int W, int Co, int kh, int kw, int sh, int sw, int ph,
                         int pw, int dh, int dw, int groups, int deformable_groups, float scale, void* workspace,
                         long long workspace_bytes, void* stream);

long long cdfo_dcn_workspace_bytes_dt(int dtype, int backward, int B, int C, int H, int W, int Co, int kh, int kw, int sh,
                                      int sw, int ph, int pw, int dh, int dw, int groups, int deformable_groups);
int cdfo_dcn_forward_dt(int dtype, const void* in, const void* offset, const void* mask, const void* weight,
                        const void* bias, void* out, int B, int C, int H, int W, int Co, int kh, int kw, int sh, int sw,
                        int ph, int pw, int dh, int dw, int groups, int deformable_groups, void* workspace,
                        long long workspace_bytes, void* stream);
int cdfo_dcn_backward_dt(int dtype, const void* in, const void* offset, const void* mask, const void* weight,
                         const void* grad_out, void* grad_in, void* grad_offset, void* grad_mask, void* grad_weight,
                         void* grad_bias, int B, int C, int H, int W, int Co, int kh, int kw, int sh, int sw, int ph, int pw,
                         int dh, int dw, int groups, int deformable_groups, float scale, void* workspace,
                         long long workspace_bytes, void* stream);

long long cdfo_conv_wgrad_slab_floats(int A, int Bc, int ks, int nsplit);
int cdfo_conv_wgrad(const float* S, int lds_, int A, const float* L, int ldl, int Bc, int N, int Hs, int Ws, int Hl, int Wl,
                    int ks, int stride, int pad, int nsplit, float* slab, float* dw, int Btot, int b_off, void* stream);
int cdfo_conv_wgrad_prec(const float* S, int lds_, int A, const float* L, int ldl, int Bc, int N, int Hs, int Ws, int Hl, int Wl,
                         int ks, int stride, int pad, int nsplit, float* slab, float* dw, int Btot, int b_off, int prec,
                         void* stream);
int cdfo_coldot(const float* a, int lda, const float* b, int ldb, int nimg, long long P, int C, int nchunk, float scale,
                float* part, float* out, void* stream);
int cdfo_ew(const float* a, int lda, const float* b, int ldb, long long rows, int C, int mode, int aux, float scale, long long P,
            float* out, int ldo, void* stream);
int cdfo_layernorm64_bwd(const float* x, int ldx, const float* g, int ldg, const float* gamma, long long npix, float* dx,
                         int ldo, float* part, int nblk, void* stream);
int cdfo_dwconv3x3_wgrad(const float* x, int ldx, const float* g, int ldg, int B, int H, int W, int C, float* part, int nblk,
                         void* stream);
int cdfo_spatial_gate16_bwd(const float* t, int ldt, const float* g, int ldg, const float* w, const float* bias, int B, int H,
                            int W, float* scratch, float* dt, int ldo, float* dw99, void* stream);
int cdfo_gumbel_mask(const float* vmax, const float* noise, long long seed, int draw, float* noise_out, int B, long long P,
                     float* mask, int ldm, void* stream);
int cdfo_chanconv9(const float* in, int ldi, const float* w9, const float* bias, int flip, long long npix, float* out, int ldo,
                   void* stream);
int cdfo_corr9(const float* in, int ldi, const float* g, int ldg, int axis, int B, int H, int W, float* part, int nblk,
               void* stream);
int cdfo_seq_attn_bwd(const float* q, int ldq, const float* v, int ldv, const float* o, int ldo, const float* g, int ldg,
                      float* dq, int lddq, float* dv, int lddv, int B, int H, int W, int mode, void* stream);
int cdfo_flow_warp_bwd(const float* g, int ldg, const float* mv, long long mv_bstride, int B, int H, int W, int C, float* dx,
                       int ldo, void* stream);
int cdfo_resample2_bwd(const float* g, int ldg, int B, int H, int W, int C, int up, float* din, int ldo, void* stream);

int cdfo_chan_pool(const float* x, int ld, long long npix, int C, float* out, void* stream);
int cdfo_gate_map_cumulative(const float* pooled, const float* cum_in, const float* w, const float* bias, int B, int H, int W, int ks,
                             float* cum_out, void* stream);
int cdfo_spatial_gate(const float* x, int ld, const float* pooled, const float* w, const float* bias, int B, int H, int W,
                      int C, int ks, float* gate_scratch, float* out, int ldo, void* stream);
int cdfo_rdab_mix(const float* xf, int ld, const float* pooled, const float* w3, const float* b3, const float* vmax,
                  const float* noise, int B, int H, int W, float* out, int ldo, void* stream);
int cdfo_shrink_planes(const float* src, long long src_bstride, int planes, int B, int H, int W, int level, float* dst,
                       void* stream);
int cdfo_lincomb(float* out, const float* a, float ca, const float* b, float cb, const float* c, float cc, long long n,
                 void* stream);

int cdfo_conv2d_nchw(const float* in, const float* w, const float* bias, int B, int C, int H, int W, int Co, int kh,
                     int kw, int stride, int pad, int act, float* out, void* stream);
int cdfo_maxpool_nchw(const float* in, int BC, int H, int W, int k, int stride, float* out, void* stream);
int cdfo_resize_bilinear_nchw(const float* in, int BC, int H, int W, int Ho, int Wo, int accumulate, float* out,
                              void* stream);
int cdfo_avgpool_nchw(const float* in, int BC, long long P, float* out, void* stream);
int cdfo_ew_nchw(const float* a, const float* b, const float* x, const float* y, long long n, long long P, int mode,
                 float* out, void* stream);
int cdfo_mv_offset_mask(const float* o1, const float* o2, int ld, const float* flow, long long flow_bstride, int B,
                        long long P, int third, float mag, float* offset, float* mask, void* stream);

int cdfo_conv3x3_c64_n16(const float* x, int ldx, int B, int H, int W, const void* w_packed, const float* bias, int act, float* out,
                         int ldo, void* stream);

int cdfo_conv2d_nchw_bwd(const float* in, const float* w, const float* gout, int B, int C, int H, int W, int Co, int kh, int kw,
                         int stride, int pad, float* gin, float* gw, float* gbias, void* stream);
int cdfo_maxpool_nchw_bwd(const float* in, const float* gout, int BC, int H, int W, int k, int stride, int* idx_scratch, float* gin,
                          void* stream);
int cdfo_resize_bilinear_nchw_bwd(const float* gout, int BC, int H, int W, int Ho, int Wo, float* gin, void* stream);
int cdfo_ew_nchw_bwd(const float* g, const float* y, const float* a, const float* x, const float* yv, long long n, long long P,
                     int mode, float* out, void* stream);
int cdfo_gate_nchw_bwd_y(const float* g, const float* a, const float* x, int BC, long long P, float* gy, void* stream);
int cdfo_mv_offset_mask_bwd(const float* o1, const float* o2, int ld, const float* goff, const float* gmask, int B, long long P,
                            int third, float mag, float* g1, float* g2, void* stream);

int cdfo_chan_pool_bwd(const float* x, int ld, const float* dpooled, long long npix, float* dx, int ldo, void* stream);
int cdfo_mul_plane(const float* x, int ld, const float* plane, long long npix, float* out, int ldo, void* stream);
int cdfo_dot_plane(const float* a, int lda, const float* b, int ldb, long long npix, float* out, void* stream);
int cdfo_gumbel_softmax(const float* v, const float* u, int B, long long P, float* out, int ldo, void* stream);
int cdfo_softmax64_bwd(const float* r, int ldr, const float* dm, int ldm, long long npix, float* dz, int ldo, void* stream);

int cdfo_prof_begin(int max_records);
int cdfo_prof_end(int* launches, double* ms, double* flops, double* bytes, int nkid);
int cdfo_prof_kid_count(void);

#ifdef __cplusplus
}
#endif
#endif
```

Before: 77.72 frames/s.

## Fuse DualAttAlignment statistics into the streaming 1x1 conv kernels

Adds a fused align_stats kernel that computes the key 1x1 conv, the Gram matrix, squared norms and the channel sums of both inputs in a single streaming pass, with per-workgroup slot partials. It also adds a channel-sum epilogue to the streaming 1x1 conv so the CALayer pooling no longer needs a separate pass over the output. Together these replace several launches and full-tensor rereads with one pass, at the cost of more complex kernels, extra LDS reductions and zero-initialised partial buffers. Both paths are gated by a new switch that defaults to on.

```diff
diff --git a/cdfo_amd/_lib.py b/cdfo_amd/_lib.py
--- a/cdfo_amd/_lib.py
+++ b/cdfo_amd/_lib.py
@@ -40,6 +40,7 @@
         ("off_accumulate", C.c_int),
         ("res2_pixscale", C.c_void_p),
         ("src_halfsplit", C.c_int),
+        ("chan_sum_out", C.c_void_p), ("chan_sum_slots", C.c_int),
     ]
 
 
diff --git a/cdfo_amd/csrc/conv1x1_bf16x3.hip b/cdfo_amd/csrc/conv1x1_bf16x3.hip
--- a/cdfo_amd/csrc/conv1x1_bf16x3.hip
+++ b/cdfo_amd/csrc/conv1x1_bf16x3.hip
@@ -262,6 +262,20 @@
   if (!ln_out && a.ln_gamma && !(a.nsrc == 1 && a.cs[0] == 64 && a.ln_beta && aligned16(a.ln_gamma) && aligned16(a.ln_beta))) return CDFO_EINVAL;
   const long long P = (long long)a.H * a.W;
   if (a.res2_pixscale && (!a.res2 || taps)) return CDFO_EINVAL;
+  if (a.chan_sum_out) {
+    if (a.Cout != 64 || a.CoutP != 64 || a.store_mode != CDFO_STORE_PLAIN || a.chan_sum_slots <= 0 || !aligned16(a.chan_sum_out)) return CDFO_EINVAL;
+    static const bool use_stream = cdfo_switch("CDFO_CONV1X1_STREAM", 1) != 0;
+    if (use_stream && !ln_out) {
+      const int r = cdfo_conv1x1_stream_try(a, st);
+      if (r == 1) return 0;
+      if (r != 0) return r;
+    }
+    cdfo_conv_args plain = a;
+    plain.chan_sum_out = nullptr; plain.chan_sum_slots = 0;
+    const int rc = cdfo_conv1x1_bf16x3(&plain, stream);
+    if (rc) return rc;
+    return cdfo_chan_sum_partial(a.out, a.ldo, a.B, P, a.chan_sum_slots, a.chan_sum_out, stream);
+  }
   if (ln_out) {
     const int r = cdfo_conv1x1_stream_try(a, st);
     if (r == 1) return 0;
diff --git a/cdfo_amd/csrc/conv1x1_stream.hip b/cdfo_amd/csrc/conv1x1_stream.hip
--- a/cdfo_amd/csrc/conv1x1_stream.hip
+++ b/cdfo_amd/csrc/conv1x1_stream.hip
@@ -26,7 +26,19 @@
   _Float16* ln_hl; const float* ln_g; const float* ln_b;
   const float* w_last;
   int W;
+  float* csum; int csum_slots;
 };
+
+__host__ __device__ inline long long st_owner(long long t, long long tiles, int grid) { return ((t + 1) * grid + tiles - 1) / tiles - 1; }
+inline int st_slots(int B, int tiles_per_image, int grid) {
+  const long long tiles = (long long)B * tiles_per_image;
+  int n = 1;
+  for (int b = 0; b < B; ++b) {
+    const int m = (int)(st_owner((long long)(b + 1) * tiles_per_image - 1, tiles, grid) - st_owner((long long)b * tiles_per_image, tiles, grid)) + 1;
+    n = m > n ? m : n;
+  }
+  return n;
+}
 
 __device__ __forceinline__ unsigned st_pack_bf16(float a, float b) {
   const __bf16 ha = (__bf16)a, hb = (__bf16)b;
@@ -86,7 +98,7 @@
   lo = __builtin_bit_cast(unsigned, lv);
 }
 
-template <int NCB, bool TAPS = false>
+template <int NCB, bool TAPS = false, bool CSUM = false>
 __global__ __launch_bounds__(ST_THREADS) void conv1x1_stream_kernel(st_args a) {
   extern __shared__ __attribute__((aligned(16))) unsigned char smem[];
   const int tid = threadIdx.x, lane = tid & 63, h = lane >> 5, r = lane & 31;
@@ -200,6 +212,9 @@
     for (; issued < NS - 1 && issued < n_items; ++issued) issue(issued);
 
     f32x16 acc[NCB][2];
+    float cs[CSUM ? 32 : 1];
+#pragma unroll
+    for (int e = 0; e < (CSUM ? 32 : 1); ++e) cs[e] = 0.f;
     for (long long it = 0; it < n_items; ++it) {
       const int k = (int)(it % items_per_tile);
       const long long younger = TAPS ? 0 : issued - it - 1;
@@ -366,6 +381,12 @@
             }
           }
         } else if (pin < a.P) {
+          if (CSUM) {
+#pragma unroll
+            for (int ni = 0; ni < 2; ++ni)
+#pragma unroll
+              for (int e = 0; e < 16; ++e) cs[ni * 16 + e] += acc[0][ni][e];
+          }
           float* op = a.out + ((long long)b * a.P + pin) * a.ldo;
 #pragma unroll
           for (int cb = 0; cb < NCB; ++cb)
@@ -385,10 +406,302 @@
         }
       }
     }
+    if (CSUM) {
+      float* red = reinterpret_cast<float*>(ring);
+#pragma unroll
+      for (int ni = 0; ni < 2; ++ni)
+#pragma unroll
+        for (int jj = 0; jj < 2; ++jj) {
+          const int n = ni * 32 + jj * 16 + h * 8;
+          const f32x4 v0 = {cs[ni * 16 + 8 * jj], cs[ni * 16 + 8 * jj + 1], cs[ni * 16 + 8 * jj + 2], cs[ni * 16 + 8 * jj + 3]};
+          const f32x4 v1 = {cs[ni * 16 + 8 * jj + 4], cs[ni * 16 + 8 * jj + 5], cs[ni * 16 + 8 * jj + 6], cs[ni * 16 + 8 * jj + 7]};
+          *reinterpret_cast<f32x4*>(red + r * 64 + n) = v0;
+          *reinterpret_cast<f32x4*>(red + r * 64 + n + 4) = v1;
+        }
+      __syncthreads();
+      const int slot = (int)(blockIdx.x - st_owner((long long)b * a.tiles_per_image, a.tiles, gridDim.x));
+      if (tid < 64 && slot >= 0 && slot < a.csum_slots) {
+        float sw[4];
+#pragma unroll
+        for (int wv = 0; wv < 4; ++wv) {
+          const float* rw = reinterpret_cast<const float*>(smem + ring_off + wv * NS * ST_STAGE);
+          float t = 0.f;
+          for (int rr = 0; rr < 32; ++rr) t += rw[rr * 64 + tid];
+          sw[wv] = t;
+        }
+        a.csum[((long long)b * a.csum_slots + slot) * 64 + tid] = (sw[0] + sw[1]) + (sw[2] + sw[3]);
+      }
+    }
     img_t0 = seg_hi;
   }
 }
 
+struct sg_args {
+  st_item src[3];
+  const float* w; const float* bias; int act_fn;
+  long long P; int tiles_per_image; long long tiles;
+  float* gram; float* sum0; float* sum1; int slots;
+};
+
+constexpr int SG_NS = 3;
+
+template <int CH>
+__global__ __launch_bounds__(ST_THREADS) void align_gram_partial_kernel(sg_args a) {
+  extern __shared__ __attribute__((aligned(16))) unsigned char smem[];
+  constexpr int NS = SG_NS, NKB = 2, IPT = 3, GS = CH + 2;
+  const int tid = threadIdx.x, lane = tid & 63, h = lane >> 5, r = lane & 31;
+  const int wave = __builtin_amdgcn_readfirstlane(tid >> 6);
+  constexpr int w_half = NKB * 4 * 2 * 64 * 16;
+  unsigned char* sWh = smem;
+  unsigned char* sWl = smem + w_half;
+  float* sBias = reinterpret_cast<float*>(smem + 2 * w_half);
+  constexpr int ring_off = 2 * w_half + 64 * 4;
+  unsigned char* ring = smem + ring_off + wave * NS * ST_STAGE;
+  const unsigned ring_lds = (unsigned)(unsigned long long)(smem) + ring_off + wave * NS * ST_STAGE;
+  auto chan_of_row = [](int n) { const int m = n & 31; return (n & ~31) + ((m >> 4) & 1) * 16 + ((m >> 2) & 1) * 8 + ((m >> 3) & 1) * 4 + (m & 3); };
+
+  const long long t_lo = a.tiles * blockIdx.x / gridDim.x, t_hi = a.tiles * (blockIdx.x + 1) / gridDim.x;
+  if (t_lo >= t_hi) return;
+  const float slope = a.act_fn == CDFO_ACT_NONE ? 1.f : (a.act_fn == CDFO_ACT_LRELU ? 0.1f : 0.f);
+
+  int d_px[8], d_part[8];
+#pragma unroll
+  for (int k = 0; k < 8; ++k) {
+    const int s = 64 * k + lane, p = s >> 4;
+    d_px[k] = p;
+    d_part[k] = (s & 15) ^ (p & 15);
+  }
+  auto part_off = [&](int q) { return r * 256 + ((q ^ (r & 15)) << 4); };
+
+  for (int i = tid; i < (128 >> 2) * 64; i += ST_THREADS) {
+    const int rowpos = i % 64, kg = i / 64;
+    const int n = chan_of_row(rowpos);
+    const f32x4 wv = *reinterpret_cast<const f32x4*>(a.w + ((long long)kg * 64 + n) * 4);
+    const int c = kg >> 2, hh = (kg >> 1) & 1, j0 = (kg & 1) * 4;
+    u32x2 hi, lo;
+    hi[0] = st_pack_bf16(wv[0], wv[1]); hi[1] = st_pack_bf16(wv[2], wv[3]);
+    lo[0] = st_pack_bf16(wv[0] - st_bf16_round(wv[0]), wv[1] - st_bf16_round(wv[1]));
+    lo[1] = st_pack_bf16(wv[2] - st_bf16_round(wv[2]), wv[3] - st_bf16_round(wv[3]));
+    const int off = ((c * 2 + hh) * 64 + rowpos) * 16 + j0 * 2;
+    *reinterpret_cast<u32x2*>(sWh + off) = hi;
+    *reinterpret_cast<u32x2*>(sWl + off) = lo;
+  }
+  for (int i = tid; i < 64; i += ST_THREADS) sBias[i] = a.bias ? a.bias[i] : 0.f;
+
+  const int c_part = lane >> 2, c_sub = (lane & 3) * 4, h_part = (lane / CH) * CH / 4;
+
+  for (long long img_t0 = t_lo; img_t0 < t_hi;) {
+    const int b = (int)(img_t0 / a.tiles_per_image);
+    const long long img_end = (long long)(b + 1) * a.tiles_per_image;
+    const long long seg_hi = img_end < t_hi ? img_end : t_hi;
+    __syncthreads();
+
+    const long long n_items = (seg_hi - img_t0) * IPT;
+    long long issued = 0;
+    auto issue = [&](long long it) {
+      const long long tile = img_t0 + it / IPT;
+      const st_item src = a.src[(int)(it % IPT)];
+      const long long p0 = (tile - (long long)b * a.tiles_per_image) * 128 + wave * 32;
+      const long long rows_left = a.P - p0;
+      const float* base = src.base + ((long long)b * a.P + (rows_left > 0 ? p0 : 0)) * src.ld + src.ch0;
+      const unsigned long long pb = reinterpret_cast<unsigned long long>(base);
+      i32x4 rsrc;
+      rsrc[0] = __builtin_amdgcn_readfirstlane((int)(unsigned)pb);
+      rsrc[1] = __builtin_amdgcn_readfirstlane((int)(unsigned)(pb >> 32));
+      const long long bytes = rows_left > 0 ? (rows_left < 32 ? rows_left : 32) * (long long)src.ld * 4 : 0;
+      rsrc[2] = __builtin_amdgcn_readfirstlane((int)bytes);
+      rsrc[3] = 0x00020000;
+      unsigned voff[8];
+#pragma unroll
+      for (int q = 0; q < 8; ++q) voff[q] = (unsigned)(d_px[q] * src.ld * 4 + d_part[q] * 16);
+      st_dma8(voff, rsrc, __builtin_amdgcn_readfirstlane(ring_lds + (unsigned)(it % NS) * ST_STAGE));
+    };
+    for (; issued < NS - 1 && issued < n_items; ++issued) issue(issued);
+
+    f32x16 acc[2];
+    float g[CH], sq = 0.f, sk = 0.f, sx[2] = {0.f, 0.f};
+#pragma unroll
+    for (int j = 0; j < CH; ++j) g[j] = 0.f;
+    for (long long it = 0; it < n_items; ++it) {
+      const int k = (int)(it % IPT);
+      const long long younger = issued - it - 1;
+      if (younger >= 2) asm volatile("s_waitcnt vmcnt(16)" ::: "memory");
+      else if (younger == 1) asm volatile("s_waitcnt vmcnt(8)" ::: "memory");
+      else asm volatile("s_waitcnt vmcnt(0)" ::: "memory");
+      const unsigned char* st = ring + (it % NS) * ST_STAGE;
+      if (k == 0) {
+#pragma unroll
+        for (int ni = 0; ni < 2; ++ni)
+#pragma unroll
+          for (int e = 0; e < 16; ++e) acc[ni][e] = 0.f;
+      }
+      if (k < NKB) {
+#pragma unroll
+        for (int c = 0; c < 4; ++c) {
+          const f32x4 v0 = *reinterpret_cast<const f32x4*>(st + part_off(c * 4 + h * 2));
+          const f32x4 v1 = *reinterpret_cast<const f32x4*>(st + part_off(c * 4 + h * 2 + 1));
+          union { unsigned u[4]; bf16x8_t v; } ph, pl;
+          ph.u[0] = st_pack_bf16(v0[0], v0[1]); ph.u[1] = st_pack_bf16(v0[2], v0[3]);
+          ph.u[2] = st_pack_bf16(v1[0], v1[1]); ph.u[3] = st_pack_bf16(v1[2], v1[3]);
+          pl.u[0] = st_pack_bf16(v0[0] - st_bf16_round(v0[0]), v0[1] - st_bf16_round(v0[1]));
+          pl.u[1] = st_pack_bf16(v0[2] - st_bf16_round(v0[2]), v0[3] - st_bf16_round(v0[3]));
+          pl.u[2] = st_pack_bf16(v1[0] - st_bf16_round(v1[0]), v1[1] - st_bf16_round(v1[1]));
+          pl.u[3] = st_pack_bf16(v1[2] - st_bf16_round(v1[2]), v1[3] - st_bf16_round(v1[3]));
+          const int wrow = ((k * 4 + c) * 2 + h) * 64 + r;
+#pragma unroll
+          for (int ni = 0; ni < 2; ++ni) {
+            const bf16x8_t wh = *reinterpret_cast<const bf16x8_t*>(sWh + (wrow + ni * 32) * 16);
+            const bf16x8_t wl = *reinterpret_cast<const bf16x8_t*>(sWl + (wrow + ni * 32) * 16);
+            acc[ni] = __builtin_amdgcn_mfma_f32_32x32x16_bf16(wh, pl.v, acc[ni], 0, 0, 0);
+            acc[ni] = __builtin_amdgcn_mfma_f32_32x32x16_bf16(wl, ph.v, acc[ni], 0, 0, 0);
+            acc[ni] = __builtin_amdgcn_mfma_f32_32x32x16_bf16(wh, ph.v, acc[ni], 0, 0, 0);
+          }
+        }
+        float t4[4] = {0.f, 0.f, 0.f, 0.f};
+#pragma unroll
+        for (int p = 0; p < 32; ++p)
+          t4[p & 3] += *reinterpret_cast<const float*>(st + p * 256 + ((c_part ^ (p & 15)) << 4) + c_sub);
+        sx[k] += (t4[0] + t4[1]) + (t4[2] + t4[3]);
+        if (k == NKB - 1) {
+          const long long pin = (img_t0 + it / IPT - (long long)b * a.tiles_per_image) * 128 + wave * 32 + r;
+          const bool inside = pin < a.P;
+#pragma unroll
+          for (int ni = 0; ni < 2; ++ni)
+#pragma unroll
+            for (int e = 0; e < 16; ++e) {
+              const float t = acc[ni][e] + sBias[ni * 32 + (e >> 3) * 16 + h * 8 + (e & 7)];
+              acc[ni][e] = inside ? fmaxf(t, 0.f) + slope * fminf(t, 0.f) : 0.f;
+            }
+        }
+      } else {
+        unsigned char* kst = ring + ((it - 1) % NS) * ST_STAGE;
+#pragma unroll
+        for (int ni = 0; ni < 2; ++ni)
+#pragma unroll
+          for (int jj = 0; jj < 2; ++jj) {
+            const int q0 = (ni * 32 + jj * 16 + h * 8) >> 2;
+            const f32x4 v0 = {acc[ni][8 * jj], acc[ni][8 * jj + 1], acc[ni][8 * jj + 2], acc[ni][8 * jj + 3]};
+            const f32x4 v1 = {acc[ni][8 * jj + 4], acc[ni][8 * jj + 5], acc[ni][8 * jj + 6], acc[ni][8 * jj + 7]};
+            *reinterpret_cast<f32x4*>(kst + part_off(q0)) = v0;
+            *reinterpret_cast<f32x4*>(kst + part_off(q0 + 1)) = v1;
+          }
+        float gt[CH], tq = 0.f, tk = 0.f;
+#pragma unroll
+        for (int j = 0; j < CH; ++j) gt[j] = 0.f;
+#pragma unroll
+        for (int p = 0; p < 32; ++p) {
+          const int own = p * 256 + ((c_part ^ (p & 15)) << 4) + c_sub;
+          const float qv = *reinterpret_cast<const float*>(st + own);
+          const float kc = *reinterpret_cast<const float*>(kst + own);
+          tq = fmaf(qv, qv, tq);
+          tk = fmaf(kc, kc, tk);
+#pragma unroll
+          for (int j4 = 0; j4 < CH / 4; ++j4) {
+            const f32x4 kv = *reinterpret_cast<const f32x4*>(kst + p * 256 + (((h_part + j4) ^ (p & 15)) << 4));
+#pragma unroll
+            for (int e = 0; e < 4; ++e) gt[j4 * 4 + e] = fmaf(qv, kv[e], gt[j4 * 4 + e]);
+          }
+        }
+#pragma unroll
+        for (int j = 0; j < CH; ++j) g[j] += gt[j];
+        sq += tq;
+        sk += tk;
+      }
+      if (issued < n_items) { asm volatile("s_waitcnt lgkmcnt(0)" ::: "memory"); issue(issued); ++issued; }
+    }
+
+    {
+      float* red = reinterpret_cast<float*>(ring);
+#pragma unroll
+      for (int j = 0; j < CH; ++j) red[lane * GS + j] = g[j];
+      red[lane * GS + CH] = sq;
+      red[lane * GS + CH + 1] = sk;
+      red[64 * GS + lane] = sx[0];
+      red[64 * GS + 64 + lane] = sx[1];
+      __syncthreads();
+      const int slot = (int)(blockIdx.x - st_owner((long long)b * a.tiles_per_image, a.tiles, gridDim.x));
+      if (slot >= 0 && slot < a.slots) {
+        const float* r0 = reinterpret_cast<const float*>(smem + ring_off);
+        const float* r1 = reinterpret_cast<const float*>(smem + ring_off + 1 * NS * ST_STAGE);
+        const float* r2 = reinterpret_cast<const float*>(smem + ring_off + 2 * NS * ST_STAGE);
+        const float* r3 = reinterpret_cast<const float*>(smem + ring_off + 3 * NS * ST_STAGE);
+        const long long bs = (long long)b * a.slots + slot;
+        for (int i = tid; i < 64 * GS + 128; i += ST_THREADS) {
+          const float v = (r0[i] + r1[i]) + (r2[i] + r3[i]);
+          if (i < 64 * GS) a.gram[bs * (64 * GS) + i] = v;
+          else if (i < 64 * GS + 64) a.sum0[bs * 64 + (i - 64 * GS)] = v;
+          else a.sum1[bs * 64 + (i - 64 * GS - 64)] = v;
+        }
+      }
+    }
+    img_t0 = seg_hi;
+  }
+}
+
+}
+
+extern "C" int cdfo_stream_slots_for_grid(int B, long long P, int grid) {
+  if (B <= 0 || P <= 0 || grid <= 0 || (P + 127) / 128 > 0x7fffffff / 2) return CDFO_EINVAL;
+  const int tpi = (int)((P + 127) / 128);
+  const long long tiles = (long long)B * tpi;
+  return st_slots(B, tpi, (int)(tiles < grid ? tiles : grid));
+}
+extern "C" int cdfo_stream_slot_of(int B, long long P, int grid, int wg, int b) {
+  if (B <= 0 || P <= 0 || grid <= 0 || wg < 0 || b < 0 || b >= B) return CDFO_EINVAL;
+  const int tpi = (int)((P + 127) / 128);
+  const long long tiles = (long long)B * tpi;
+  const int g = (int)(tiles < grid ? tiles : grid);
+  if (wg >= g) return -1;
+  const long long t_lo = tiles * wg / g, t_hi = tiles * (wg + 1) / g;
+  const long long lo = t_lo > (long long)b * tpi ? t_lo : (long long)b * tpi, hi = t_hi < (long long)(b + 1) * tpi ? t_hi : (long long)(b + 1) * tpi;
+  if (lo >= hi) return -1;
+  return (int)(wg - st_owner((long long)b * tpi, tiles, g));
+}
+extern "C" int cdfo_align_stats_slots(int B, long long P) {
+  const int cus = cdfo_num_cus();
+  if (cus <= 0) return CDFO_EINVAL;
+  return cdfo_stream_slots_for_grid(B, P, cus);
+}
+
+extern "C" int cdfo_align_stats(const float* x0, int ld0, const float* x1, int ld1, const float* q, int ldq, const float* w_packed,
+                                const float* bias, int act, int ch_per_head, int B, long long P, int nslots, float* gram_partial,
+                                float* sum0_partial, float* sum1_partial, void* stream) {
+  if (B <= 0 || P <= 0 || nslots <= 0 || !x0 || !x1 || !q || !w_packed || !gram_partial || !sum0_partial || !sum1_partial) return CDFO_EINVAL;
+  if (act != CDFO_ACT_NONE && act != CDFO_ACT_LRELU && act != CDFO_ACT_RELU) return CDFO_EINVAL;
+  if (ch_per_head != 8 && ch_per_head != 16) return CDFO_EINVAL;
+  const int lds_[3] = {ld0, ld1, ldq};
+  for (int i = 0; i < 3; ++i)
+    if (lds_[i] < 64 || lds_[i] % 4 || (long long)lds_[i] * 4 * 32 >= (1ll << 31)) return CDFO_EINVAL;
+  if (!aligned16(x0) || !aligned16(x1) || !aligned16(q) || !aligned16(w_packed) || !aligned16(gram_partial) || !aligned16(sum0_partial) ||
+      !aligned16(sum1_partial))
+    return CDFO_EALIGN;
+  if ((P + 127) / 128 > 0x7fffffff / 2) return CDFO_EINVAL;
+  hipStream_t st = static_cast<hipStream_t>(stream);
+  sg_args s{};
+  s.src[0] = {x0, ld0, 0}; s.src[1] = {x1, ld1, 0}; s.src[2] = {q, ldq, 0};
+  s.w = w_packed; s.bias = bias; s.act_fn = act;
+  s.P = P; s.tiles_per_image = (int)((P + 127) / 128); s.tiles = (long long)B * s.tiles_per_image;
+  s.gram = gram_partial; s.sum0 = sum0_partial; s.sum1 = sum1_partial; s.slots = nslots;
+  const int cus = cdfo_num_cus();
+  if (cus <= 0) return CDFO_EINVAL;
+  const int grid = (int)(s.tiles < cus ? s.tiles : cus);
+  if (nslots < st_slots(B, s.tiles_per_image, grid)) return CDFO_EINVAL;
+  const int lds = 2 * (2 * 4 * 2 * 64 * 16) + 64 * 4 + 4 * SG_NS * ST_STAGE;
+  const double px = (double)B * P;
+  CdfoProfScope prof(st, KID_GRAM, px * (2.0 * 128 * 64 + 2.0 * 64 * 18), 4.0 * 192 * px);
+  if (ch_per_head == 16) {
+    static CdfoAttrOnce once;
+    const hipError_t e = cdfo_set_max_lds(once, reinterpret_cast<const void*>(align_gram_partial_kernel<16>), 160 * 1024 - 256);
+    if (e != hipSuccess) return (int)e;
+    hipLaunchKernelGGL(align_gram_partial_kernel<16>, dim3(grid), dim3(ST_THREADS), lds, st, s);
+  } else {
+    static CdfoAttrOnce once;
+    const hipError_t e = cdfo_set_max_lds(once, reinterpret_cast<const void*>(align_gram_partial_kernel<8>), 160 * 1024 - 256);
+    if (e != hipSuccess) return (int)e;
+    hipLaunchKernelGGL(align_gram_partial_kernel<8>, dim3(grid), dim3(ST_THREADS), lds, st, s);
+  }
+  CDFO_LAUNCH_CHECK();
+  return 0;
 }
 
 int cdfo_conv1x1_stream_try(const cdfo_conv_args& a, hipStream_t st) {
@@ -422,6 +735,7 @@
   }
   if (a.store_mode != CDFO_STORE_PLAIN || (a.ln_gamma && !ln_out) || a.CoutP % 64 || a.CoutP > 128 || a.Cout % 8) return 0;
   if (ln_out && (a.CoutP != 64 || a.Cout != 64)) return 0;
+  if (a.chan_sum_out && (a.CoutP != 64 || a.Cout != 64 || ln_out || a.chan_sum_slots <= 0)) return 0;
   const int ncb = a.CoutP / 64, nkb = a.Cin / 64;
   if (nkb < 1 || nkb > CDFO_MAXSRC * 4) return 0;
   const int w_bytes = 2 * nkb * 4 * 2 * ncb * 64 * 16 + ncb * 64 * 4;
@@ -459,7 +773,14 @@
   const int lds = w_bytes + 4 * ns * ST_STAGE + scale_bytes;
   const double px = (double)a.B * P;
   CdfoProfScope prof(st, KID_CONV1, 2.0 * px * a.Cout * a.Cin, 4.0 * (px * a.Cout * (1 + nr) + px * a.Cin + (double)a.Cin * a.Cout));
-  if (ncb == 1) {
+  if (a.chan_sum_out) {
+    if (a.chan_sum_slots < st_slots(a.B, s.tiles_per_image, grid)) return 0;
+    s.csum = a.chan_sum_out; s.csum_slots = a.chan_sum_slots;
+    static CdfoAttrOnce once;
+    const hipError_t e = cdfo_set_max_lds(once, reinterpret_cast<const void*>(conv1x1_stream_kernel<1, false, true>), 160 * 1024 - 256);
+    if (e != hipSuccess) return (int)e;
+    hipLaunchKernelGGL((conv1x1_stream_kernel<1, false, true>), dim3(grid), dim3(ST_THREADS), lds, st, s);
+  } else if (ncb == 1) {
     static CdfoAttrOnce once;
     const hipError_t e = cdfo_set_max_lds(once, reinterpret_cast<const void*>(conv1x1_stream_kernel<1>), 160 * 1024 - 256);
     if (e != hipSuccess) return (int)e;
diff --git a/cdfo_amd/csrc/conv3x3_bf16.hip b/cdfo_amd/csrc/conv3x3_bf16.hip
--- a/cdfo_amd/csrc/conv3x3_bf16.hip
+++ b/cdfo_amd/csrc/conv3x3_bf16.hip
@@ -362,7 +362,7 @@
   hipStream_t st = static_cast<hipStream_t>(stream);
   if (a.nsrc < 1 || a.nsrc > CDFO_MAXSRC || a.B <= 0 || a.ks != 3 || a.stride != 1 || a.pad != 1) return CDFO_EINVAL;
   if (a.act == CDFO_ACT_SIGMOID) return CDFO_EINVAL;
-  if (a.out2_cp16 || a.res_up2 || a.src_plane_wrap || a.res2_pixscale) return CDFO_EINVAL;
+  if (a.out2_cp16 || a.res_up2 || a.src_plane_wrap || a.res2_pixscale || a.chan_sum_out) return CDFO_EINVAL;
   int csum = 0;
   for (int s = 0; s < a.nsrc; ++s) {
     if (a.cs[s] <= 0 || a.cs[s] % 16 || a.ld[s] % 4 || a.ld[s] < a.cs[s]) return CDFO_EINVAL;
diff --git a/cdfo_amd/csrc/conv3x3_ring.hip b/cdfo_amd/csrc/conv3x3_ring.hip
--- a/cdfo_amd/csrc/conv3x3_ring.hip
+++ b/cdfo_amd/csrc/conv3x3_ring.hip
@@ -1107,7 +1107,7 @@
   if (a.nsrc != 1 || a.B <= 0 || a.ks != 3 || a.stride != 1 || a.pad != 1 || !a.src_f16) return CDFO_EINVAL;
   if (a.act == CDFO_ACT_SIGMOID || a.Cin <= 0 || a.Cin % 16 || a.cs[0] != a.Cin || a.ld[0] != 16) return CDFO_EINVAL;
   if (a.CoutP % 64 || a.CoutP > 1024 || a.CoutP < a.Cout || a.Cout <= 0 || a.Ho != a.H || a.Wo != a.W || a.w_bstride != 0) return CDFO_EINVAL;
-  if (a.store_mode != CDFO_STORE_PLAIN || a.res2_pixscale) return CDFO_EINVAL;
+  if (a.store_mode != CDFO_STORE_PLAIN || a.res2_pixscale || a.chan_sum_out) return CDFO_EINVAL;
   if (a.Cout % 8) return CDFO_EINVAL;
   if (a.out2_cp16 && (a.Cout % 16 || !aligned16(a.out2_cp16))) return CDFO_EINVAL;
   if (a.res_up2 && ((a.H | a.W) & 1 || a.ldru % 4 || a.ldru < a.Cout || !aligned16(a.res_up2))) return CDFO_EINVAL;
diff --git a/cdfo_amd/csrc/conv_igemm.hip b/cdfo_amd/csrc/conv_igemm.hip
--- a/cdfo_amd/csrc/conv_igemm.hip
+++ b/cdfo_amd/csrc/conv_igemm.hip
@@ -195,7 +195,7 @@
   const cdfo_conv_args& a = *pa;
   hipStream_t st = static_cast<hipStream_t>(stream);
   if (a.nsrc < 1 || a.nsrc > CDFO_MAXSRC || a.B <= 0 || a.H <= 0 || a.W <= 0) return CDFO_EINVAL;
-  if (a.act == CDFO_ACT_SIGMOID || a.out2_cp16 || a.res_up2 || a.src_plane_wrap || a.res2_pixscale) return CDFO_EINVAL;
+  if (a.act == CDFO_ACT_SIGMOID || a.out2_cp16 || a.res_up2 || a.src_plane_wrap || a.res2_pixscale || a.chan_sum_out) return CDFO_EINVAL;
   int csum = 0;
   for (int s = 0; s < a.nsrc; ++s) {
     if (a.cs[s] <= 0 || a.cs[s] % 16 || a.ld[s] % 4 || a.ld[s] < a.cs[s]) return CDFO_EINVAL;
diff --git a/cdfo_amd/cvsr_v8.py b/cdfo_amd/cvsr_v8.py
--- a/cdfo_amd/cvsr_v8.py
+++ b/cdfo_amd/cvsr_v8.py
@@ -114,6 +114,7 @@
         self.new_frame_alone = switches.get("CDFO_NEW_ALONE")
         self.trunk_side_stream = switches.get("CDFO_TRUNK_SIDE")
         self.wino_halfsplit = switches.get("CDFO_WINO_HS")
+        self.align_stats = switches.get("CDFO_ALIGN_STATS")
         self.fe_weight_lo = True
         self.fea_r_single_pass = switches.get("CDFO_FEA_R_1PASS")
         for key, shape, fan_in, init in _param_spec():
@@ -331,15 +332,23 @@
         warped = K.empty_act(GB, H, W, NF, xc.device)
         for g, mv in enumerate(mvs):
             K.flow_warp(extra[g * B:(g + 1) * B], mv, mv_bstride, out=warped[g * B:(g + 1) * B])
-        kf = self._conv([warped, pred], w[a + "fusion_out.0"], act=K.ACT_RELU)
-        gp, ng = K.gram_partial(xc, kf, 16)
-        sw, ns = K.chan_sum_partial(warped)
-        sp, _ = K.chan_sum_partial(pred)
+        fused = self.precision != "f32" and self.align_stats
+        if fused:
+            gp, sw, sp, ng = K.align_stats(warped, pred, xc, w[a + "fusion_out.0"], K.ACT_RELU, 16)
+            ns = ng
+        else:
+            kf = self._conv([warped, pred], w[a + "fusion_out.0"], act=K.ACT_RELU)
+            gp, ng = K.gram_partial(xc, kf, 16)
+            sw, ns = K.chan_sum_partial(warped)
+            sp, _ = K.chan_sum_partial(pred)
         fold = K.align_fold(gp, ng, sw, sp, ns, H * W, raw[a + "temperature"], raw[a + "conv_du.0.weight"],
                             raw[a + "conv_du.0.bias"], raw[a + "conv_du.2.weight"], raw[a + "conv_du.2.bias"],
                             raw[a + "project_out.weight"], raw[a + "fusion_out.0.weight"])
-        o = self._conv([warped, pred, xc], fold, act=K.ACT_RELU)
-        part, n = K.chan_sum_partial(o)
+        if fused:
+            o, part, n = self._conv([warped, pred, xc], fold, act=K.ACT_RELU, chan_sum_out=True)
+        else:
+            o = self._conv([warped, pred, xc], fold, act=K.ACT_RELU)
+            part, n = K.chan_sum_partial(o)
         gate = K.vec_mlp(part, n, H * W, raw[a + "CALayer.conv_du.0.weight"], raw[a + "CALayer.conv_du.0.bias"], 64,
                          K.ACT_RELU, raw[a + "CALayer.conv_du.2.weight"], raw[a + "CALayer.conv_du.2.bias"], 64,
                          K.ACT_SIGMOID)
diff --git a/cdfo_amd/kernels.py b/cdfo_amd/kernels.py
--- a/cdfo_amd/kernels.py
+++ b/cdfo_amd/kernels.py
@@ -133,9 +133,17 @@
          res1: Optional[torch.Tensor] = None, res2: Optional[torch.Tensor] = None,
          out: Optional[torch.Tensor] = None, prec: int = PREC_F32,
          ln: Optional[tuple] = None, s2d: bool = False, out_f16: bool = False, ln_out: Optional[tuple] = None,
-         res2_scale: Optional[torch.Tensor] = None, cp16_out: bool = False):
+         res2_scale: Optional[torch.Tensor] = None, cp16_out: bool = False, chan_sum_out: bool = False):
     if isinstance(srcs, torch.Tensor):
         srcs = [srcs]
+    if chan_sum_out:
+        if cp16_out or ln_out is not None or out_f16 or s2d or pc.shuffle2 or pc.Cout != 64:
+            raise ValueError("conv: chan_sum_out needs a plain fp32 64-channel result")
+        if (prec != PREC_F32 and pc.ks == 1 and stride == 1 and pad == 0 and pc.CoutP == 64 and ln is None
+                and all(s.dtype == torch.float32 and s.shape[3] % 64 == 0 for s in srcs)):
+            return _conv1x1_chan_sum(srcs, pc, act, res1, res2, out, res2_scale)
+        o = conv(srcs, pc, stride=stride, pad=pad, act=act, res1=res1, res2=res2, out=out, prec=prec, ln=ln, res2_scale=res2_scale)
+        return (o, *chan_sum_partial(o))
     a = ConvArgs()
     B = H = W = None
     cin = 0
@@ -234,6 +242,45 @@
     return C.c_void_p(None if t is None else t.data_ptr())
 
 
+def _conv1x1_chan_sum(srcs, pc: PackedConv, act, res1, res2, out, res2_scale):
+    a = ConvArgs()
+    B, H, W, _, _ = _chk_act(srcs[0], "src0")
+    cin = 0
+    for i, s in enumerate(srcs):
+        b_, h_, w_, c_, ld_ = _chk_act(s, f"src{i}")
+        if (B, H, W) != (b_, h_, w_):
+            raise ValueError("conv sources disagree on B/H/W")
+        a.src[i], a.ld[i], a.cs[i] = s.data_ptr(), ld_, c_
+        cin += c_
+    if cin != pc.Cin:
+        raise ValueError(f"conv: sources have {cin} channels, weight expects {pc.Cin}")
+    a.nsrc = len(srcs)
+    a.B, a.H, a.W, a.Ho, a.Wo = B, H, W, H, W
+    a.ks, a.stride, a.pad = 1, 1, 0
+    a.Cin, a.Cout, a.CoutP = pc.Cin, pc.Cout, pc.CoutP
+    a.w, a.w_bstride, a.bias, a.act = pc.w.data_ptr(), pc.w_bstride, _p(pc.bias), act
+    if out is None:
+        out = empty_act(B, H, W, 64, srcs[0].device)
+    _, _, _, _, a.ldo = _chk_act(out, "out")
+    a.out = out.data_ptr()
+    for nm, r in (("res1", res1), ("res2", res2)):
+        if r is not None:
+            rb, rh, rw, rc, rld = _chk_act(r, nm)
+            if (rb, rh, rw) != (B, H, W) or rc < 64:
+                raise ValueError(f"{nm} shape {tuple(r.shape)} does not match the conv output")
+            setattr(a, nm, r.data_ptr())
+            setattr(a, "ldr" + nm[-1], rld)
+    if res2_scale is not None:
+        if res2 is None or tuple(res2_scale.shape) != (B, H, W) or not res2_scale.is_contiguous() or res2_scale.dtype != torch.float32:
+            raise ValueError("conv: res2_scale must be a contiguous fp32 [B,H,W] plane next to res2")
+        a.res2_pixscale = res2_scale.data_ptr()
+    n = align_stats_slots(B, H * W)
+    part = torch.zeros((B, n, 64), dtype=torch.float32, device=out.device)
+    a.chan_sum_out, a.chan_sum_slots = part.data_ptr(), n
+    check(_lib.lib().cdfo_conv1x1_bf16x3(C.byref(a), _stream()), "cdfo_conv1x1_bf16x3 (channel sums)")
+    return out, part, n
+
+
 @contextlib.contextmanager
 def cu_limit(n: int):
     prev = _lib.lib().cdfo_set_cu_limit(int(n))
@@ -857,6 +904,32 @@
     return part, n
 
 
+def align_stats_slots(B: int, P: int) -> int:
+    n = _lib.lib().cdfo_align_stats_slots(B, C.c_longlong(P))
+    if n <= 0:
+        raise CdfoError(f"cdfo_align_stats_slots({B}, {P}) failed: {n}")
+    return n
+
+
+def align_stats(x0: torch.Tensor, x1: torch.Tensor, q: torch.Tensor, pc: PackedConv, act: int, ch_per_head: int):
+    B, H, W, c0, ld0 = _chk_act(x0, "x0")
+    b1, h1, w1, c1, ld1 = _chk_act(x1, "x1")
+    bq, hq, wq, cq, ldq = _chk_act(q, "q")
+    if (b1, h1, w1) != (B, H, W) or (bq, hq, wq) != (B, H, W) or (c0, c1, cq) != (64, 64, 64):
+        raise ValueError("align_stats: three [B,H,W,64] operands expected")
+    if pc.ks != 1 or pc.Cin != 128 or pc.Cout != 64 or pc.CoutP != 64 or pc.w_bstride != 0:
+        raise ValueError("align_stats: a packed 128 -> 64 1x1 convolution expected")
+    n = align_stats_slots(B, H * W)
+    gs = 64 * (ch_per_head + 2)
+    buf = torch.zeros((B * n * (gs + 128),), dtype=torch.float32, device=q.device)
+    gram = buf[:B * n * gs].view(B, n, gs)
+    s0 = buf[B * n * gs:B * n * (gs + 64)].view(B, n, 64)
+    s1 = buf[B * n * (gs + 64):].view(B, n, 64)
+    check(_lib.lib().cdfo_align_stats(_vp(x0), ld0, _vp(x1), ld1, _vp(q), ldq, _vp(pc.w), _vp(pc.bias), act, ch_per_head, B,
+                                      C.c_longlong(H * W), n, _vp(gram), _vp(s0), _vp(s1), _stream()), "cdfo_align_stats")
+    return gram, s0, s1, n
+
+
 def mdta_fold(part: torch.Tensor, n: int, temperature: torch.Tensor, proj_w: torch.Tensor) -> PackedConv:
     B = part.shape[0]
     wout = torch.empty((B, 4096), dtype=torch.float32, device=part.device)
diff --git a/cdfo_amd/switches.py b/cdfo_amd/switches.py
--- a/cdfo_amd/switches.py
+++ b/cdfo_amd/switches.py
@@ -35,6 +35,7 @@
     Switch("CDFO_V7_HEAD_1PASS", 1, ONOFF, "python", "0: MVDualAttAlignment's offset head on two-pass activations (head_one_pass)"),
     Switch("CDFO_V7_OFF0_1PASS", 1, ONOFF, "python", "0: MVDualAttAlignment's conv_offset[0] on two-pass activations (off0_one_pass)"),
     Switch("CDFO_V7_WS_HEAD", 1, ONOFF, "python", "0: MVDualAttAlignment's offset head off the weights-stationary kernel (ws_head)"),
+    Switch("CDFO_ALIGN_STATS", 1, ONOFF, "python", "0: DualAttAlignment's statistics on the five launches of round 5: kf written, Gram and channel sums in passes of their own (model.align_stats)"),
     Switch("CDFO_WS_RING", 1, ONOFF, "hip", "0: Block_.body[0] on the private-halo kernel of rounds 1-2 instead of the ring-fed wave-specialised one"),
     Switch("CDFO_WS_MFMA16", 1, ONOFF, "hip", "0: the ring-fed weights-stationary kernel on v_mfma_f32_32x32x16_f16 instead of 16x16x32"),
     Switch("CDFO_WS_WAVES", 12, INT, "hip", "8: two instead of three waves per SIMD in the private-halo weights-stationary kernel", (8, 12)),
diff --git a/include/cdfo_hip.h b/include/cdfo_hip.h
--- a/include/cdfo_hip.h
+++ b/include/cdfo_hip.h
@@ -41,6 +41,8 @@
   float* mask_out; const float* flow; long long flow_bstride; float off_mag; int off_accumulate;
   const float* res2_pixscale;
   int src_halfsplit;
+  float* chan_sum_out;
+  int chan_sum_slots;
 } cdfo_conv_args;
 int cdfo_sizeof_conv_args(void);
 int cdfo_conv_igemm(const cdfo_conv_args* a, void* stream);
@@ -112,6 +114,12 @@
 int cdfo_chan_sum_partial(const float* in, int ldi, int B, long long P, int nchunk, float* partial, void* stream);
 int cdfo_gram_partial(const float* q, int ldq, const float* k, int ldk, int B, long long P, int ch_per_head, int nchunk,
                       float* partial, void* stream);
+int cdfo_align_stats_slots(int B, long long P);
+int cdfo_stream_slots_for_grid(int B, long long P, int grid);
+int cdfo_stream_slot_of(int B, long long P, int grid, int wg, int b);
+int cdfo_align_stats(const float* x0, int ld0, const float* x1, int ld1, const float* q, int ldq, const float* w_packed,
+                     const float* bias, int act, int ch_per_head, int B, long long P, int nslots, float* gram_partial,
+                     float* sum0_partial, float* sum1_partial, void* stream);
 int cdfo_mdta_fold(const float* partial, int nchunk, const float* temperature, const float* proj_w, int B, float* wout,
                    void* stream);
 int cdfo_align_fold(const float* gram_partial, int nchunk_g, const float* sum_warp, const float* sum_pred, int nchunk_s,
```

Result: faster. 78.62 frames/s, median of 6 (+1.2%).
